# MrTornado24/IDE-3D

Hardware: AMD Instinct MI355X
Metric: 512x512 RGB+seg frames/s @96 depth samples (whole job) (higher is better)
Workload: dtype f32 (3x3 convs + MLPs: fp32 operands as 3 bf16 pieces, 6 products, f32 accumulate); 1 GPU; BASELINE config 2: random-init ide3d-ffhq-64-512, G.mapping + G.synthesis (64 render -> 512, 96 samples, RGB + 19-class seg) + uint8 frames, batch 4 seeds per GPU; global_batch=4, parallelism=dp1, conv_arithmetic=bf16x6, conv_arithmetic_is_library_default=True

## Files before the change

### ide-3d_amd/csrc/camera.hip

```cpp
#include "common.h"

namespace ide3d {

#pragma clang fp contract(off)

struct V3 { float x, y, z; };
__device__ __forceinline__ V3 normalized(V3 v) {
    const float n = sqrtf(v.x * v.x + v.y * v.y + v.z * v.z);
    return V3{v.x / n, v.y / n, v.z / n};
}
__device__ __forceinline__ V3 cross(V3 a, V3 b) { return V3{a.y * b.z - a.z * b.y, a.z * b.x - a.x * b.z, a.x * b.y - a.y * b.x}; }

__global__ void __launch_bounds__(64)
sphere_points_kernel(const float* __restrict__ theta, const float* __restrict__ pitch, int n, float r, int pitch_is_v,
                     float* __restrict__ pos, float* __restrict__ phi_out) {
    const int i = blockIdx.x * 64 + threadIdx.x;
    if (i >= n) return;
    const float kPi = 3.14159265358979323846f;
    float p = fminf(fmaxf(pitch[i], 1e-5f), (float)(3.14159265358979323846 - 1e-5));
    if (pitch[i] != pitch[i]) p = pitch[i];
    if (pitch_is_v) p = acosf(1.f - 2.f * (p * (1.f / kPi)));
    const float t = theta[i], sp = r * sinf(p);
    pos[3 * i + 0] = sp * cosf(t);
    pos[3 * i + 2] = sp * sinf(t);
    pos[3 * i + 1] = r * cosf(p);
    if (phi_out) phi_out[i] = p;
}

__global__ void __launch_bounds__(64)
cam2world_kernel(const float* __restrict__ forward, const float* __restrict__ origin, const float* __restrict__ lookat, int lookat_stride,
                 int n, float* __restrict__ out) {
    const int i = blockIdx.x * 64 + threadIdx.x;
    if (i >= n) return;
    const V3 o{origin[3 * i], origin[3 * i + 1], origin[3 * i + 2]};
    V3 f;
    if (lookat) {
        const float* l = lookat + (int64_t)i * lookat_stride;
        f = normalized(V3{l[0] - o.x, l[1] - o.y, l[2] - o.z});
    } else {
        f = V3{forward[3 * i], forward[3 * i + 1], forward[3 * i + 2]};
    }
    f = normalized(f);
    const V3 left = normalized(cross(V3{0.f, 1.f, 0.f}, f));
    const V3 up = normalized(cross(f, left));
    float* m = out + (int64_t)i * 16;
    m[0] = -left.x; m[1] = up.x; m[2]  = -f.x; m[3]  = o.x;
    m[4] = -left.y; m[5] = up.y; m[6]  = -f.y; m[7]  = o.y;
    m[8] = -left.z; m[9] = up.z; m[10] = -f.z; m[11] = o.z;
    m[12] = 0.f;    m[13] = 0.f; m[14] = 0.f;  m[15] = 1.f;
}

}

extern "C" int ide3d_sphere_points(const float* theta, const float* pitch, int32_t n, float r, int32_t pitch_is_v,
                                   float* pos, float* phi_out, void* stream) {
    using namespace ide3d;
    IDE3D_CHECK_ARG(theta && pitch && pos, "sphere_points: null pointer");
    IDE3D_CHECK_ARG(n > 0, "sphere_points: bad shape");
    hipLaunchKernelGGL(sphere_points_kernel, dim3(cdiv(n, 64)), dim3(64), 0, (hipStream_t)stream, theta, pitch, n, r, pitch_is_v, pos, phi_out);
    IDE3D_CHECK_LAUNCH("sphere_points");
    return IDE3D_OK;
}

extern "C" int ide3d_cam2world(const float* forward, const float* origin, const float* lookat, int32_t lookat_stride, int32_t n,
                               float* out, void* stream) {
    using namespace ide3d;
    IDE3D_CHECK_ARG(origin && out && (forward || lookat), "cam2world: null pointer");
    IDE3D_CHECK_ARG(n > 0 && (lookat_stride == 0 || lookat_stride == 3), "cam2world: bad shape");
    hipLaunchKernelGGL(cam2world_kernel, dim3(cdiv(n, 64)), dim3(64), 0, (hipStream_t)stream, forward, origin, lookat, lookat_stride, n, out);
    IDE3D_CHECK_LAUNCH("cam2world");
    return IDE3D_OK;
}
```

### ide-3d_amd/csrc/common.h

```cpp
#pragma once

#include <hip/hip_runtime.h>
#include <hip/hip_fp16.h>
#include <hip/hip_bf16.h>
#include <stdint.h>
#include <stdarg.h>
#include <stdio.h>

#include "../../include/ide3d_hip.h"

namespace ide3d {

constexpr int kWave = 64;
constexpr int kNumCU = 256;
constexpr int kNumXCD = 8;


void set_error(const char* fmt, ...);

const char* modconv_build_flags();
const char* triplane_tile_build_flags();
const char* raymarch_build_flags();

void note_exclusive_violation(const char* kernel, int blocks_per_cu);
// ... 10 lines not shown
}
#define IDE3D_EXCL_LAUNCH(KERNEL, GRID, THREADS, DYN_LDS, ST, ...) \
    do { if (ide3d::exclusive_on_this_device(KERNEL, (THREADS), (DYN_LDS), #KERNEL)) hipLaunchKernelGGL(KERNEL, GRID, dim3(THREADS), DYN_LDS, ST, __VA_ARGS__); } while (0)
#define IDE3D_STR_(x) #x
#define IDE3D_STR(x) IDE3D_STR_(x)

#define IDE3D_CHECK_ARG(cond, ...)                                   \
    do { if (!(cond)) { ide3d::set_error(__VA_ARGS__); return IDE3D_EINVAL; } } while (0)

#define IDE3D_CHECK_LAUNCH(what)                                     \
    do { hipError_t e_ = hipGetLastError();                          \
         if (e_ != hipSuccess) { ide3d::set_error("%s: %s", what, hipGetErrorString(e_)); \
                                 return IDE3D_ELAUNCH; }                \
         if (ide3d::take_refused()) return IDE3D_ELAUNCH; } while (0)


template <class T> struct Elem;
template <> struct Elem<float> {
    using math_t = float;
    static __device__ __forceinline__ float  ld(const float* p) { return *p; }
    static __device__ __forceinline__ void   st(float* p, float v) { *p = v; }
};
template <> struct Elem<double> {
    using math_t = double;
    static __device__ __forceinline__ double ld(const double* p) { return *p; }
    static __device__ __forceinline__ void   st(double* p, double v) { *p = v; }
};
template <> struct Elem<__half> {
    using math_t = float;
    static __device__ __forceinline__ float  ld(const __half* p) { return __half2float(*p); }
    static __device__ __forceinline__ void   st(__half* p, float v) { *p = __float2half(v); }
};
template <> struct Elem<__hip_bfloat16> {
    using math_t = float;
    static __device__ __forceinline__ float  ld(const __hip_bfloat16* p) { return __bfloat162float(*p); }
    static __device__ __forceinline__ void   st(__hip_bfloat16* p, float v) { *p = __float2bfloat16(v); }
};


__device__ __forceinline__ int lane_id() { return threadIdx.x & (kWave - 1); }

__host__ __device__ __forceinline__ int floordiv(int a, int b) {
    int q = a / b;
    return (a % b != 0 && ((a < 0) != (b < 0))) ? q - 1 : q;
}

__device__ __forceinline__ void amax_raise(float* amax, int n, float v) {
    unsigned* const slot = reinterpret_cast<unsigned*>(amax) + (size_t)n * IDE3D_AMAX_FLOATS + (blockIdx.x % IDE3D_AMAX_SLOTS) * IDE3D_AMAX_STRIDE;
    __hip_atomic_fetch_max(slot, __float_as_uint(v), __ATOMIC_RELAXED, __HIP_MEMORY_SCOPE_AGENT);
}
__device__ __forceinline__ void amax_raise_block(float* amax, int n, float v, float* scratch) {
#pragma unroll
    for (int off = 32; off > 0; off >>= 1) v = fmaxf(v, __shfl_xor(v, off));
    __syncthreads();
    if ((threadIdx.x & 63) == 0) scratch[threadIdx.x >> 6] = v;
    __syncthreads();
    if (threadIdx.x == 0) {
        float m = scratch[0];
        for (int i = 1; i < (int)(blockDim.x >> 6); ++i) m = fmaxf(m, scratch[i]);
        if (m > 0.f) amax_raise(amax, n, m);
    }
}
__device__ __forceinline__ void amax_lds_flush(unsigned* s_am, int n, float v) { if (v > 0.f) atomicMax(&s_am[n & 63], __float_as_uint(v)); }
__device__ __forceinline__ void amax_lds_commit(float* amax, const unsigned* s_am, int p_n) {
    __syncthreads();
    if ((int)threadIdx.x < p_n && threadIdx.x < 64 && s_am[threadIdx.x] != 0u) amax_raise(amax, (int)threadIdx.x, __uint_as_float(s_am[threadIdx.x]));
}

__host__ __device__ __forceinline__ int64_t cdiv64(int64_t a, int64_t b) { return (a + b - 1) / b; }
__host__ __device__ __forceinline__ int     cdiv(int a, int b) { return (a + b - 1) / b; }

__device__ __forceinline__ bool pool_gt(float v, float m) { return v > m || v != v; }

inline bool ptr_aligned(const void* p, uintptr_t bytes) { return (reinterpret_cast<uintptr_t>(p) & (bytes - 1)) == 0; }

inline int stream_grid(int64_t work_items, int per_block) {
    int64_t g = cdiv64(work_items, per_block);
    const int64_t cap = (int64_t)kNumCU * 8;
    if (g > cap) g = cap;
    if (g < 1) g = 1;
    return (int)g;
}

__device__ __forceinline__ int xcd_remap(int bid, int nblocks) {
    const int xcd = bid % kNumXCD;
    const int idx = bid / kNumXCD;
    const int q = nblocks / kNumXCD, r = nblocks % kNumXCD;
    const int base = (xcd < r) ? xcd * (q + 1) : r * (q + 1) + (xcd - r) * q;
    return base + idx;
}

}
```

### ide-3d_amd/csrc/core.hip

```cpp
#include "common.h"
#include <string.h>
#include <stdio.h>
#include <map>
#include <mutex>
#include <tuple>

namespace ide3d {

static thread_local char g_err[512] = "";

void set_error(const char* fmt, ...) {
    va_list ap;
    va_start(ap, fmt);
    vsnprintf(g_err, sizeof(g_err), fmt, ap);
    va_end(ap);
}

static int g_excl_violations = 0;
static char g_excl_text[384] = "";
void note_exclusive_violation(const char* kernel, int blocks_per_cu) {
    ++g_excl_violations;
    snprintf(g_excl_text, sizeof(g_excl_text), "%d workgroups of %.200s fit one CU of this device: exclusive residency (DESIGN.md 4.2) does not hold", blocks_per_cu, kernel);
    fprintf(stderr, "[libide3d_hip] %s; the launch is refused (select IDE3D_CONV_ARITH=fp32)\n", g_excl_text);
}
int exclusive_violations() { return g_excl_violations; }
static thread_local bool g_refused = false;
void refuse_launch(const char* kernel) {
    g_refused = true;
    set_error("%.200s: more than one workgroup fits a CU of this device, exclusive residency (DESIGN.md 4.2) does not hold; launch refused "
              "(IDE3D_CONV_ARITH=fp32 selects the arithmetic that needs none)", kernel);
}
bool take_refused() { const bool r = g_refused; g_refused = false; return r; }

bool exclusive_checked(const void* kernel, int threads, size_t dyn_lds, const char* name) {
    static std::mutex mu;
    static std::map<std::tuple<const void*, int, int, size_t>, int> table;
    int dev = 0;
    if (hipGetDevice(&dev) != hipSuccess) return true;
    int occ;
    {
        std::lock_guard<std::mutex> lock(mu);
        const auto key = std::make_tuple(kernel, dev, threads, dyn_lds);
        auto it = table.find(key);
        if (it == table.end()) {
            int n = 0;
            occ = (hipOccupancyMaxActiveBlocksPerMultiprocessor(&n, kernel, threads, dyn_lds) == hipSuccess && n > 0) ? n : -1;
            table.emplace(key, occ);
            if (occ > 1) note_exclusive_violation(name, occ);
        } else occ = it->second;
    }
    if (occ > 1) refuse_launch(name);
    return occ <= 1;
}

}

extern "C" int ide3d_exclusive_violations(void) { return ide3d::g_excl_violations; }
extern "C" const char* ide3d_exclusive_violation_text(void) { return ide3d::g_excl_text; }
extern "C" const char* ide3d_last_error(void) { return ide3d::g_err; }
extern "C" int ide3d_abi_version(void) { return 8; }
extern "C" const char* ide3d_build_arch(void) { return "gfx950"; }
extern "C" const char* ide3d_build_flags(void) {
    static char buf[512] = "";
    static bool done = false;
    if (!done) {
        snprintf(buf, sizeof(buf), "%s%s%s", ide3d::modconv_build_flags(), ide3d::triplane_tile_build_flags(), ide3d::raymarch_build_flags());
        const size_t n = strlen(buf);
        if (n && buf[n - 1] == ' ') buf[n - 1] = 0;
        done = true;
    }
    return buf;
}
```

### ide-3d_amd/csrc/modconv.hip

```cpp
#include "common.h"
#include "knobs.h"
#include <stdlib.h>
#include <string.h>
#include <type_traits>

namespace ide3d {

typedef float f32x16 __attribute__((ext_vector_type(16)));

#ifdef IDE3D_MC_TRACE
__device__ unsigned long long g_mc_dbg[256];
#define IDE3D_MC_TS(k) { const unsigned long long now_ = __builtin_readcyclecounter(); mc_acc[k] += now_ - mc_last; mc_last = now_; }
#else
#define IDE3D_MC_TS(k)
#endif

enum { MODE_CONV3 = 0, MODE_CONV1 = 1, MODE_TCONV3 = 2, MODE_TCONV3A = 3, MODE_CONV3S2 = 4 };

template <int MODE> struct ModeCfg;
template <> struct ModeCfg<MODE_CONV3>  { static constexpr int KC = 4, WTAPS = 9, MAXT = 9; };
template <> struct ModeCfg<MODE_CONV1>  { static constexpr int KC = 16, WTAPS = 1, MAXT = 1; };
template <> struct ModeCfg<MODE_CONV3S2> { static constexpr int KC = 4, WTAPS = 9, MAXT = 9; };
template <> struct ModeCfg<MODE_TCONV3> { static constexpr int KC = 4, WTAPS = 9, MAXT = 4; };
template <> struct ModeCfg<MODE_TCONV3A> { static constexpr int KC = 4, WTAPS = 9, MAXT = 9; };
// ... 495 lines not shown
    for (int q = 0; q < PARTS; ++q) {
        const unsigned pk = pk_bf16(a, b);
        out[q] = pk;
        if (q + 1 < PARTS) { a -= __uint_as_float(pk << 16); b -= __uint_as_float(pk & 0xffff0000u); }
    }
    }
}
template <int F16>
__device__ __forceinline__ f32x16 sp_mfma(const u32x4& a, const u32x4& b, const f32x16& c) {
    if constexpr (F16) return __builtin_amdgcn_mfma_f32_32x32x16_f16(__builtin_bit_cast(f16x8, a), __builtin_bit_cast(f16x8, b), c, 0, 0, 0);
    else return __builtin_amdgcn_mfma_f32_32x32x16_bf16(__builtin_bit_cast(bf16x8, a), __builtin_bit_cast(bf16x8, b), c, 0, 0, 0);
}
__device__ __forceinline__ void f16_scale(float bound, float& scale, float& unscale) {
    scale = 1.f; unscale = 1.f;
    if (bound > 0.f && bound < __builtin_inff()) {
        int e;
        frexpf(bound, &e);
        e = min(max(15 - e, -126), 126);
        scale = ldexpf(1.f, e); unscale = ldexpf(1.f, -e);
    }
}

__global__ void __launch_bounds__(256)
modconv_row_scale_kernel(const float* __restrict__ w, int cout, int rowlen, int rows_padded, float* __restrict__ scale, float* __restrict__ unscale) {
    const int row = blockIdx.x * 4 + (threadIdx.x >> 6), lane = threadIdx.x & 63;
    if (row >= rows_padded) return;
    float m = 0.f;
    if (row < cout) for (int i = lane; i < rowlen; i += 64) m = fmaxf(m, fabsf(w[(int64_t)row * rowlen + i]));
#pragma unroll
    for (int off = 32; off > 0; off >>= 1) m = fmaxf(m, __shfl_xor(m, off));
    if (lane == 0) { float sc, us; f16_scale(m, sc, us); scale[row] = sc; unscale[row] = us; }
}

template <int PARTS, int F16 = 0>
__global__ void __launch_bounds__(256)
modconv_pack_split_kernel(const float* __restrict__ w, int cout, int cin, int bm, int mblocks, int cchunks, u32x4* __restrict__ out,
                          const float* __restrict__ row_scale = nullptr) {
    const int64_t total = (int64_t)mblocks * cchunks * 9 * 2 * bm;
    const int64_t stride = (int64_t)gridDim.x * blockDim.x;
    for (int64_t i = (int64_t)blockIdx.x * blockDim.x + threadIdx.x; i < total; i += stride) {
        int64_t r = i;
        const int co_l = (int)(r % bm); r /= bm;
        const int kg = (int)(r % 2); r /= 2;
        const int tap = (int)(r % 9); r /= 9;
        const int cc = (int)(r % cchunks); r /= cchunks;
        const int mb = (int)r;
        const int co = mb * bm + co_l;
        const float rs = F16 ? row_scale[co] : 1.f;
        unsigned pk[4][PARTS];
#pragma unroll
        for (int e = 0; e < 4; ++e) {
            const int ci = cc * 16 + kg * 8 + e * 2;
            const float a = (co < cout && ci < cin) ? w[((int64_t)co * cin + ci) * 9 + tap] * rs : 0.f;
            const float b = (co < cout && ci + 1 < cin) ? w[((int64_t)co * cin + ci + 1) * 9 + tap] * rs : 0.f;
            split_pair<PARTS, F16>(a, b, pk[e]);
        }
        const int64_t base = (((int64_t)(mb * cchunks + cc) * 9 + tap) * PARTS * 2 + kg) * bm + co_l;
#pragma unroll
        for (int q = 0; q < PARTS; ++q) {
            const u32x4 v = {pk[0][q], pk[1][q], pk[2][q], pk[3][q]};
            out[base + (int64_t)q * 2 * bm] = v;
        }
    }
}

template <int OFF_BYTES>
__device__ __forceinline__ u32x4 lds_read128_async(unsigned addr) {
    u32x4 v;
    asm volatile("ds_read_b128 %0, %1 offset:%2" : "=v"(v) : "v"(addr), "n"(OFF_BYTES));
    return v;
}
template <int PENDING>
__device__ __forceinline__ void lds_wait128(u32x4& first) { asm volatile("s_waitcnt lgkmcnt(%1)" : "+v"(first) : "n"(PENDING)); }
__device__ __forceinline__ void lds_pin128(u32x4& v) { asm volatile("" : "+v"(v)); }

struct HeadEpi {
    const u32x4* w;
    const float* bias;
    float* y;
    int rows;
    float clamp;
    int store_x;
    int bias_first;
};
template <int PH, int PW, int NWV, int MTW, int NTW, int BM, int MT, int PARTS, int SCRATCH>
__device__ __forceinline__ void split_heads_finish(const ide3d_modconv_params& p, const HeadEpi& he, f32x16 (&acc)[1][MTW][NTW], float* smem,
                                                   int n0, int y0, int x0, int wm, int wn, int lp) {
    constexpr int NT = 64 * NWV, BN = PH * PW, TP = BN + 4, ROWS = MT * 32, CCH = BM / 16, A_UNITS = PARTS * 2 * ROWS;
    static_assert(BM * TP + 2 * BM + ROWS <= SCRATCH, "activation tile + coefficients must fit the loop's LDS");
    const int tid = threadIdx.x, lane = tid & 63, half = lane >> 5, l32 = lane & 31;
    const int wid = __builtin_amdgcn_readfirstlane(tid >> 6);
    const int hw = p.h * p.w_;
    float* const s_t = smem;
    float* const s_dm = smem + BM * TP;
    float* const s_bi = s_dm + BM;
    float* const s_hb = s_bi + BM;
    for (int e = tid; e < BM; e += NT) {
        s_dm[e] = (p.dcoefs && e < p.cout) ? p.dcoefs[(int64_t)n0 * p.cout + e] : 1.f;
        s_bi[e] = (p.bias && e < p.cout) ? p.bias[e] : 0.f;
    }
    for (int e = tid; e < ROWS; e += NT) s_hb[e] = (he.bias && e < he.rows) ? he.bias[e] : 0.f;
    __syncthreads();
    const float e_alpha = (p.act == 3) ? p.alpha : 1.f, e_gain = p.gain;
    const float e_clamp = (p.clamp >= 0.f) ? p.clamp : __builtin_inff();
    const float e_nstr = p.noise ? p.noise_strength : 0.f;
    auto finish = [&](float v, float d, float nz, float bb) {
        v *= d; v += nz; v += bb;
        v = (v > 0.f) ? v : v * e_alpha;
        v *= e_gain;
        return fminf(fmaxf(v, -e_clamp), e_clamp);
    };
#pragma unroll
    for (int j = 0; j < NTW; ++j) {
        const int pix = (wn * NTW + j) * 32 + lp;
        const int gy = y0 + pix / PW, gx = x0 + pix % PW;
        const float nz = (e_nstr != 0.f) ? p.noise[gy * p.w_ + gx] * e_nstr : 0.f;
#pragma unroll
        for (int i = 0; i < MTW; ++i)
#pragma unroll
            for (int r = 0; r < 16; ++r) {
                const int rl = (wm * MTW + i) * 32 + (r & 3) + 8 * (r >> 2) + 4 * half;
                s_t[rl * TP + pix] = finish(acc[0][i][j][r], s_dm[rl], nz, s_bi[rl]);
            }
    }
    __syncthreads();
    typedef float f32x4a __attribute__((ext_vector_type(4)));
    typedef float f32x4u __attribute__((ext_vector_type(4), aligned(4)));
    if (he.store_x) {
        float* const yimg = p.y + (int64_t)n0 * p.cout * hw;
#pragma unroll 4
        for (int e = tid; e < BM * BN / 4; e += NT) {
            const int rl = e / (BN / 4), pix = (e % (BN / 4)) * 4;
            const int gy = y0 + pix / PW, gx = x0 + pix % PW;
            *reinterpret_cast<f32x4u*>(yimg + (int64_t)rl * hw + gy * p.w_ + gx) = *reinterpret_cast<const f32x4a*>(s_t + rl * TP + pix);
        }
    }
    constexpr int NPT = BN / 32;
    constexpr int RG = (MT % 2 == 0 && NPT / NWV < 2) ? 2 : 1, MTH = MT / RG, PG = NWV / RG, NTH = NPT / PG;
    static_assert(MTH * RG == MT && NTH * PG == NPT && NTH >= 1, "head work must split evenly over the waves");
    const int rg = wid / PG, pg = wid % PG;
    const u32x4* __restrict__ wsrc = he.w + (int64_t)n0 * CCH * A_UNITS + half * ROWS + rg * MTH * 32 + l32;
    f32x16 hacc[MTH][NTH];
#pragma unroll
    for (int m = 0; m < MTH; ++m)
#pragma unroll
        for (int g = 0; g < 4; ++g) {
            const f32x4a b4 = *reinterpret_cast<const f32x4a*>(s_hb + (rg * MTH + m) * 32 + 8 * g + 4 * half);
#pragma unroll
            for (int t = 0; t < NTH; ++t)
#pragma unroll
                for (int k = 0; k < 4; ++k) hacc[m][t][4 * g + k] = he.bias_first ? b4[k] : 0.f;
        }
    u32x4 af[2][MTH][PARTS];
    auto fetch_a = [&](int c, int buf) {
#pragma unroll
        for (int m = 0; m < MTH; ++m)
#pragma unroll
            for (int q = 0; q < PARTS; ++q) af[buf][m][q] = wsrc[(int64_t)c * A_UNITS + q * 2 * ROWS + m * 32];
    };
    fetch_a(0, 0);
#pragma unroll
    for (int c = 0; c < CCH; ++c) {
        const int ab = c & 1;
        if (c + 1 < CCH) fetch_a(c + 1, ab ^ 1);
#pragma unroll
        for (int t = 0; t < NTH; ++t) {
// ... 661 lines not shown
                for (int j = 0; j < STRIP_CO; ++j) acc[j] = fmaf(va, w1[j], acc[j]);
            } else {
                const float vb = ok_b ? xb[k] * scv[k] : 0.f;
                const float4 a0 = wv[0], a1 = wv[1], c0v = wv[4], c1v = wv[5];
                const float w0[STRIP_CO] = {a0.x, a0.y, a0.z, a0.w, a1.x, a1.y, a1.z, a1.w};
                const float w2[STRIP_CO] = {c0v.x, c0v.y, c0v.z, c0v.w, c1v.x, c1v.y, c1v.z, c1v.w};
#pragma unroll
                for (int j = 0; j < STRIP_CO; ++j) { acc[j] = fmaf(va, w0[j], acc[j]); acc[j] = fmaf(vb, w2[j], acc[j]); }
            }
        }
    }
#pragma unroll
    for (int j = 0; j < STRIP_CO; ++j) s_red[q][j][lane] = acc[j];
    __syncthreads();
    float am = 0.f;
    {
        static_assert(STRIP_CO <= STRIP_WAVES, "wave q < STRIP_CO finishes output channel co0 + q");
        float v = 0.f;
        const int qc = min(q, STRIP_CO - 1);
#pragma unroll
        for (int k = 0; k < STRIP_WAVES; ++k) v += s_red[k][qc][lane];
        const int co = co0 + q;
        if (live && q < STRIP_CO && co < p.cout) {
            v *= p.dcoefs ? p.dcoefs[(int64_t)n * p.cout + co] : 1.f;
            const int oy = is_row ? oh - 1 : t, ox = is_row ? t : ow - 1;
            p.y[((int64_t)n * p.cout + co) * ((int64_t)oh * pitch) + (int64_t)oy * pitch + ox] = v;
            amax_acc(am, v);
        }
    }
    if (p.y_amax) amax_raise_block(p.y_amax, n, am, s_am);
}

struct BlockId { int mb, tile, grp, split; };
__device__ __forceinline__ BlockId decode_block(const ConvGeom& g) {
    int bid = xcd_remap(blockIdx.x, gridDim.x);
    BlockId b;
    b.mb = bid % g.mblocks; bid /= g.mblocks;
    b.tile = bid % g.tile_base[4]; bid /= g.tile_base[4];
    b.grp = bid % g.img_groups; bid /= g.img_groups;
    b.split = bid;
    return b;
}

template <int MODE, int BIG, int TI, int PH, int PW>
__global__ void __launch_bounds__(256, (McCfg<MODE, BIG, TI, PH, PW>::NCLS * McCfg<MODE, BIG, TI, PH, PW>::MTW * McCfg<MODE, BIG, TI, PH, PW>::NTW > 8) ? 1
                                       : (TI * PH * PW <= 128 && MODE != MODE_CONV3S2) ? 3 : 2)
modconv_kernel(ide3d_modconv_params p, const float* __restrict__ wp, float* __restrict__ partial, ConvGeom g) {
    using K = McCfg<MODE, BIG, TI, PH, PW>;
    __shared__ __attribute__((aligned(16))) float s_w[2 * K::LDS_W];
    __shared__ __attribute__((aligned(16))) float s_x[2 * K::LDS_X];
    const BlockId b = decode_block(g);
    int cls = 0;
    if (MODE == MODE_TCONV3) { cls = (b.tile >= g.tile_base[1]) + (b.tile >= g.tile_base[2]) + (b.tile >= g.tile_base[3]); }
    modconv_tile<MODE, BIG, TI, PH, PW>(p, wp, partial, g, s_w, s_x, b.mb, b.tile - g.tile_base[cls], b.grp, b.split, cls, g.tiles_x[cls]);
}


#ifdef IDE3D_SP_SHARED_SIMD
constexpr bool kSpExclusive = false;
#else
constexpr bool kSpExclusive = true;
#endif
template <int MODE, int BIG, int PH, int PARTS, int WBUF, int NWV>
constexpr int sp_waves_per_simd() {
    using K = SpCfg<MODE, BIG, PH, PARTS, WBUF, NWV>;
    return (NWV == 8) ? 2 : (!kSpExclusive && K::LDS_BYTES <= 80 * 1024 && (WBUF == 1 || K::NCLS * K::MTW * K::NTW <= 8)) ? 2 : 1;
}
template <int MODE, int BIG, int PH, int PARTS, int WBUF = 2, int NWV = 4, int F16 = 0>
__global__ void __launch_bounds__(64 * NWV, (sp_waves_per_simd<MODE, BIG, PH, PARTS, WBUF, NWV>()))
modconv_split_kernel(ide3d_modconv_params p, const u32x4* __restrict__ wp, float* __restrict__ partial, ConvGeom g, const float* __restrict__ row_unscale) {
    using K = SpCfg<MODE, BIG, PH, PARTS, WBUF, NWV>;
    if constexpr (kSpExclusive) { if constexpr (NWV == 8) asm volatile("" ::: "v255"); else asm volatile("" ::: "v255", "a255"); }
    __shared__ __attribute__((aligned(16))) unsigned char sp_smem[K::LDS_BYTES];
    const BlockId b = decode_block(g);
    modconv_split_tile<MODE, BIG, PH, PARTS, WBUF, NWV, F16>(p, wp, partial, g, sp_smem, b.mb, b.tile, b.grp, b.split, g.tiles_x[0], row_unscale);
}

template <int BIG, int PH, int HEAD_MT>
__global__ void __launch_bounds__(512, 2)
modconv_split_heads_kernel(ide3d_modconv_params p, const u32x4* __restrict__ wp, ConvGeom g, HeadEpi he) {
    using K = SpCfg<MODE_CONV3, BIG, PH, 3, 2, 8>;
    if constexpr (kSpExclusive) asm volatile("" ::: "v255");
    __shared__ __attribute__((aligned(16))) unsigned char sp_smem[K::LDS_BYTES];
    const BlockId b = decode_block(g);
    modconv_split_tile<MODE_CONV3, BIG, PH, 3, 2, 8, 0, 1, -1, HEAD_MT>(p, wp, nullptr, g, sp_smem, b.mb, b.tile, b.grp, b.split, g.tiles_x[0], nullptr, nullptr, &he);
}

template <int BIG, int PH, int PARTS, int F16 = 0>
__global__ void __launch_bounds__(512, 2)
modconv_split_pair_kernel(ide3d_modconv_params p, const u32x4* __restrict__ wp, float* __restrict__ partial, ConvGeom g, const float* __restrict__ row_unscale) {
    using K = SpCfg<MODE_TCONV3A, BIG, PH, PARTS, 2, 8, 1>;
    if constexpr (kSpExclusive) asm volatile("" ::: "v255");
    __shared__ __attribute__((aligned(16))) unsigned char sp_smem[K::LDS_BYTES];
    const int half_grid = (int)(gridDim.x >> 1);
    const int par = __builtin_amdgcn_readfirstlane((int)blockIdx.x >= half_grid ? 1 : 0);
    int bid = xcd_remap((int)blockIdx.x - par * half_grid, half_grid);
    BlockId b;
    b.mb = bid % g.mblocks; bid /= g.mblocks;
    b.tile = bid % g.tile_base[4]; bid /= g.tile_base[4];
    b.grp = bid % g.img_groups; bid /= g.img_groups;
    b.split = bid;
    if (par == 0) modconv_split_tile<MODE_TCONV3A, BIG, PH, PARTS, 2, 8, F16, 1, 0>(p, wp, partial, g, sp_smem, b.mb, b.tile, b.grp, b.split, g.tiles_x[0], row_unscale);
    else          modconv_split_tile<MODE_TCONV3A, BIG, PH, PARTS, 2, 8, F16, 1, 1>(p, wp, partial, g, sp_smem, b.mb, b.tile, b.grp, b.split, g.tiles_x[0], row_unscale);
}

template <int MODE, int BIG, int PH, int PARTS, int WBUF, int F16>
__global__ void __launch_bounds__(512, 2)
modconv_split_teams_kernel(ide3d_modconv_params p, const u32x4* __restrict__ wp, float* __restrict__ partial, ConvGeom g, const float* __restrict__ row_unscale) {
    using K = SpCfg<MODE, BIG, PH, PARTS, WBUF, 4>;
    static_assert(2 * K::LDS_BYTES <= 160 * 1024, "both teams' LDS must fit");
    asm volatile("" ::: "v255");
    __shared__ __attribute__((aligned(16))) unsigned char sp_smem[2 * K::LDS_BYTES];
    const int team = (int)(threadIdx.x >> 8);
    int bid = xcd_remap(blockIdx.x, gridDim.x);
    const int mpairs = g.mblocks >> 1;
    BlockId b;
    b.mb = 2 * (bid % mpairs) + team; bid /= mpairs;
    b.tile = bid % g.tile_base[4]; bid /= g.tile_base[4];
    b.grp = bid % g.img_groups; bid /= g.img_groups;
    b.split = bid;
    modconv_split_tile<MODE, BIG, PH, PARTS, WBUF, 4, F16, 2>(p, wp, partial, g, sp_smem + team * K::LDS_BYTES, b.mb, b.tile, b.grp, b.split, g.tiles_x[0], row_unscale,
                                                              reinterpret_cast<float*>(sp_smem));
}

__global__ void __launch_bounds__(256)
modconv_epilogue_kernel(ide3d_modconv_params p, const float* __restrict__ partial, int split_k, int oh, int ow) {
    const int64_t per = (int64_t)p.n * p.cout * oh * ow;
    const int64_t stride = (int64_t)gridDim.x * blockDim.x;
    int am_n = -1; float am = 0.f;
    __shared__ unsigned s_am[64];
    const bool am_lds = p.y_amax && p.n <= 64;
    if (p.y_amax) { if (threadIdx.x < 64) s_am[threadIdx.x] = 0u; __syncthreads(); }
    const int hw = oh * ow;
    if (p.y_pitch <= 0 && (hw & 3) == 0) {
        typedef float f32x4v __attribute__((ext_vector_type(4)));
        const int64_t per4 = per >> 2;
        for (int64_t q = (int64_t)blockIdx.x * blockDim.x + threadIdx.x; q < per4; q += stride) {
            const int64_t i = q << 2;
            f32x4v v = {0.f, 0.f, 0.f, 0.f};
            int s = 0;
            for (; s + 4 <= split_k; s += 4) {
                f32x4v t[4];
#pragma unroll
                for (int k = 0; k < 4; ++k) t[k] = *reinterpret_cast<const f32x4v*>(partial + (int64_t)(s + k) * per + i);
#pragma unroll
                for (int k = 0; k < 4; ++k) v += t[k];
            }
            for (; s < split_k; ++s) v += *reinterpret_cast<const f32x4v*>(partial + (int64_t)s * per + i);
            const int pix = (int)(i % hw);
            const int co = (int)((i / hw) % p.cout);
            const int n = (int)(i / ((int64_t)hw * p.cout));
            const float d = p.dcoefs ? p.dcoefs[(int64_t)n * p.cout + co] : 1.f, bb = p.bias ? p.bias[co] : 0.f;
#pragma unroll
            for (int e = 0; e < 4; ++e) {
                float x = v[e];
                if (p.dcoefs) x *= d;
                if (p.noise) x += p.noise[pix + e] * p.noise_strength;
                if (p.bias) x += bb;
                if (p.act == 3) x = (x > 0.f) ? x : x * p.alpha;
                x *= p.gain;
                if (p.clamp >= 0.f) x = fminf(fmaxf(x, -p.clamp), p.clamp);
                v[e] = x;
            }
            *reinterpret_cast<f32x4v*>(p.y + i) = v;
            if (p.y_amax) {
                if (n != am_n) { if (am_n >= 0) { if (am_lds) amax_lds_flush(s_am, am_n, am); else amax_commit(p.y_amax, am_n, am, false); } am_n = n; am = 0.f; }
                amax_acc(am, v[0]); amax_acc(am, v[1]); amax_acc(am, v[2]); amax_acc(am, v[3]);
// ... 363 lines not shown
    IDE3D_CHECK_ARG(p.y_pitch == 0 || (p.mode == 2 && p.y_pitch >= 2 * p.w_ + 1), "modconv2d: y_pitch is the row pitch of a transposed convolution's output (>= 2 w + 1), or 0");
    hipStream_t st_head = (hipStream_t)stream;
    {
        const int64_t hw = (int64_t)p.h * p.w_;
        if (head_small_applies(p)) {
            if (hw <= 64) hipLaunchKernelGGL((head_small_kernel<64, 32>), dim3(cdiv(p.cout, HS_RB), 1, p.n), dim3(HS_THREADS), 0, st_head, p, (int)hw);
            else          hipLaunchKernelGGL((head_small_kernel<256, 8>), dim3(cdiv(p.cout, HS_RB), cdiv((int)hw, 256), p.n), dim3(HS_THREADS), 0, st_head, p, (int)hw);
            IDE3D_CHECK_LAUNCH("modconv2d (small-map heads)");
            return IDE3D_OK;
        }
    }
    if (head_split_applies(p, resolve_arith(p.arith))) {
        const int parts = resolve_arith(p.arith) == 3 ? 2 : 3, mt = p.cout <= 32 ? 1 : 6, cchunks = cdiv(p.cin, 16);
        IDE3D_CHECK_ARG(p.workspace_bytes >= head_packed_units(p.n, cchunks, parts, mt) * 16, "modconv2d: workspace too small for the packed head weights");
        u32x4* wu = reinterpret_cast<u32x4*>(p.workspace);
        const int64_t items = (int64_t)p.n * cchunks * 2 * mt * 32;
        const int tiles = cdiv(p.h * p.w_, 32 * head_waves(mt));
        const int hw_h = p.h * p.w_, wgs_img = kNumCU / p.n, tiles32 = hw_h / 32;
        const bool resident = head_resident_applies(p);
#define IDE3D_HEAD_RES(P, M, C) IDE3D_EXCL_LAUNCH((head_resident_kernel<P, M, C>), dim3(p.n * wgs_img), 512, 0, st_head, p, wu, wgs_img, tiles32)
#define IDE3D_HEAD(P, M) do { \
            hipLaunchKernelGGL(head_pack_split_kernel<P>, dim3(stream_grid(items, 256)), dim3(256), 0, st_head, p.w, p.w_batch_stride, p.n, p.cout, p.cin, M * 32, cchunks, wu); \
            if (resident) { if (M == 6) IDE3D_HEAD_RES(P, 6, 8); else if (cchunks == 4) IDE3D_HEAD_RES(P, 1, 4); else IDE3D_HEAD_RES(P, 1, 8); } \
            else IDE3D_EXCL_LAUNCH((head_split_kernel<P, M>), dim3(p.n * tiles), 64 * head_waves(M), 0, st_head, p, wu, cchunks, tiles); } while (0)
        if (parts == 2) { if (mt == 1) IDE3D_HEAD(2, 1); else IDE3D_HEAD(2, 6); }
        else            { if (mt == 1) IDE3D_HEAD(3, 1); else IDE3D_HEAD(3, 6); }
#undef IDE3D_HEAD
#undef IDE3D_HEAD_RES
        IDE3D_CHECK_LAUNCH("modconv2d (split-bf16 heads)");
        return IDE3D_OK;
    }
    int arith_eff = resolve_arith(p.arith);
    if (arith_eff == 16 && !p.x_amax) arith_eff = 6;
    ConvPlan pl; plan_conv(p, pl, arith_eff);
    IDE3D_CHECK_ARG(p.workspace_bytes >= (pl.packed_floats + pl.aux_floats + pl.partial_floats) * (int64_t)sizeof(float),
                    "modconv2d: workspace too small (need %lld bytes)", (long long)((pl.packed_floats + pl.aux_floats + pl.partial_floats) * sizeof(float)));
    hipStream_t st = (hipStream_t)stream;
    float* wp = p.workspace;
    float* partial = p.workspace + pl.packed_floats + pl.aux_floats;
    if (pl.parts) {
        if (!p.weights_packed) pack_split_weights(p, pl, wp, st);
#define IDE3D_SP_DISPATCH(M) \
        do { if (pl.big == 1) { if (pl.f16) launch_split<M, 1, 2, 1>(p, pl, wp, partial, st); else if (pl.parts == 2) launch_split<M, 1, 2>(p, pl, wp, partial, st); else launch_split<M, 1, 3>(p, pl, wp, partial, st); } \
             else             { if (pl.f16) launch_split<M, 2, 2, 1>(p, pl, wp, partial, st); else if (pl.parts == 2) launch_split<M, 2, 2>(p, pl, wp, partial, st); else launch_split<M, 2, 3>(p, pl, wp, partial, st); } } while (0)
        if (pl.mode == MODE_CONV3) IDE3D_SP_DISPATCH(MODE_CONV3); else IDE3D_SP_DISPATCH(MODE_TCONV3A);
#undef IDE3D_SP_DISPATCH
    } else {
    if (!p.weights_packed) {
        hipLaunchKernelGGL(modconv_pack_kernel, dim3(stream_grid(pl.packed_floats, 256)), dim3(256), 0, st,
                           p.w, p.w_batch_stride, p.w_batch_stride ? p.n : 1, p.cout, p.cin, pl.taps, pl.bm, pl.kc, pl.mblocks, pl.cchunks, wp);
    }
#define IDE3D_MC_DISPATCH(M) \
    do { if (pl.big == 1) launch_tiles<M, 1>(p, pl, wp, partial, st); else if (pl.big == 2) launch_tiles<M, 2>(p, pl, wp, partial, st); \
         else launch_tiles<M, 0>(p, pl, wp, partial, st); } while (0)
    if (pl.mode == MODE_CONV3)       IDE3D_MC_DISPATCH(MODE_CONV3);
    else if (pl.mode == MODE_CONV1)  IDE3D_MC_DISPATCH(MODE_CONV1);
    else if (pl.mode == MODE_CONV3S2) IDE3D_MC_DISPATCH(MODE_CONV3S2);
    else if (pl.mode == MODE_TCONV3A) IDE3D_MC_DISPATCH(MODE_TCONV3A);
    else                             IDE3D_MC_DISPATCH(MODE_TCONV3);
#undef IDE3D_MC_DISPATCH
    }
    if (pl.g.split_k > 1) {
        const int64_t per = (int64_t)p.n * p.cout * pl.oh * pl.ow;
        hipLaunchKernelGGL(modconv_epilogue_kernel, dim3(stream_grid((p.y_pitch <= 0 && ((pl.oh * pl.ow) & 3) == 0) ? per / 4 : per, 256)), dim3(256), 0, st, p, partial, pl.g.split_k, pl.oh, pl.ow);
    }
    if (pl.mode == MODE_TCONV3A && !p.weights_packed) {
        hipLaunchKernelGGL(tconv_strip_pack_kernel, dim3(stream_grid(pl.strip_floats, 256)), dim3(256), 0, st, p.w, p.cout, p.cin, cdiv(p.cout, STRIP_CO) * STRIP_CO,
                           wp + pl.packed_floats + pl.strip_off);
    }
    if (pl.strip) {
        const int cout_pad = cdiv(p.cout, STRIP_CO) * STRIP_CO;
        float* const wstrip = wp + pl.packed_floats + pl.strip_off;
        const int nb_re = cdiv(p.w_ + 1, 64), nb_ro = cdiv(p.w_, 64), nb_ce = cdiv(p.h, 64), nb_co = cdiv(p.h, 64);
        float* const xs = wstrip + pl.strip_floats;
        hipLaunchKernelGGL(tconv_strip_gather_kernel, dim3(stream_grid((int64_t)p.n * p.cin * (p.h + p.w_), 256)), dim3(256), 0, st, p.x, p.n * p.cin, p.h, p.w_, xs);
        hipLaunchKernelGGL(tconv_strip_kernel, dim3(nb_re + nb_ro + nb_ce + nb_co, cout_pad / STRIP_CO, p.n), dim3(64 * STRIP_WAVES), 0, st, p, wstrip, xs, cout_pad,
                           pl.oh, pl.ow, (int64_t)(p.y_pitch > 0 ? p.y_pitch : pl.ow), nb_re, nb_ro, nb_ce);
    }
    IDE3D_CHECK_LAUNCH("modconv2d");
    return IDE3D_OK;
}

extern "C" int ide3d_modconv2d_heads(const ide3d_modconv_params* pp, const ide3d_modconv_head_epilogue* hp, void* stream) {
    using namespace ide3d;
    IDE3D_CHECK_ARG(pp != nullptr && hp != nullptr, "modconv2d_heads: null params");
    const ide3d_modconv_params& p = *pp;
    const ide3d_modconv_head_epilogue& h = *hp;
    IDE3D_CHECK_ARG(p.x && p.w && p.workspace && (p.y || h.no_activation_output) && h.w && h.y && h.workspace, "modconv2d_heads: null tensor / workspace pointer");
    int rc = check_modconv(p);
    if (rc) return rc;
    IDE3D_CHECK_ARG(p.act == 1 || p.act == 3, "modconv2d_heads: act must be linear (1) or lrelu (3)");
    IDE3D_CHECK_ARG(h.rows > 0, "modconv2d_heads: bad head rows");
    auto no_kernel = [](const char* why) { set_error("modconv2d_heads: %s", why); return IDE3D_ENOKERNEL; };
    if (knob_live("IDE3D_MODCONV_NO_HEAD_FUSION")) return no_kernel("IDE3D_MODCONV_NO_HEAD_FUSION is set");
    if (p.k != 3 || p.mode != 0 || p.w_batch_stride != 0 || p.y_amax || p.y_pitch != 0) return no_kernel("not a shared-weight 3x3 layer without side outputs");
    int arith = resolve_arith(p.arith);
    if (arith == 16 && !p.x_amax) arith = 6;
    if (arith != 6) return no_kernel("the fused form exists for bf16x6 only");
    ConvPlan pl; plan_conv(p, pl, arith);
    if (pl.parts != 3 || pl.f16 || pl.mode != MODE_CONV3 || pl.pair || pl.g.split_k != 1 || pl.g.mblocks != 1 || pl.bm != p.cout || kTiles[pl.tile].images != 1)
        return no_kernel("the layer's plan does not hold all channels of a tile in one workgroup");
    const bool tile16 = pl.big == 1 && p.cout == 128 && pl.tile == T16x16 && sp_form(pl).waves == 8;
    const bool tile32 = pl.big == 2 && p.cout == 64 && pl.tile == T32x16;
    const int ph = tile32 ? 32 : 16;
    if (!(tile16 || tile32) || p.h % ph != 0 || p.w_ % 16 != 0) return no_kernel("no fused instance for this tile");
    ide3d_modconv_params q{};
    q.x = p.y; q.w = h.w; q.bias = h.bias; q.y = h.y;
    q.n = p.n; q.cin = p.cout; q.cout = h.rows; q.h = p.h; q.w_ = p.w_; q.k = 1; q.mode = 0;
    q.act = 1; q.alpha = 0.f; q.gain = 1.f; q.clamp = h.clamp; q.w_batch_stride = (int64_t)h.rows * p.cout; q.arith = p.arith;
    const int mt = h.rows <= 32 ? 1 : 6, hcc = p.cout / 16;
    if (head_small_applies(q) || !head_split_applies(q, resolve_arith(q.arith)) || resolve_arith(q.arith) == 3 || (mt == 6 && !tile16))
        return no_kernel("the heads do not take the split-bf16 path");
    IDE3D_CHECK_ARG(p.workspace_bytes >= (pl.packed_floats + pl.aux_floats) * (int64_t)sizeof(float), "modconv2d_heads: workspace too small");
    IDE3D_CHECK_ARG(h.workspace_bytes >= head_packed_units(p.n, hcc, 3, mt) * 16, "modconv2d_heads: head workspace too small");
    hipStream_t st = (hipStream_t)stream;
    if (!p.weights_packed) pack_split_weights(p, pl, p.workspace, st);
    u32x4* const hw_packed = reinterpret_cast<u32x4*>(h.workspace);
    const int64_t items = (int64_t)p.n * hcc * 2 * mt * 32;
    hipLaunchKernelGGL(head_pack_split_kernel<3>, dim3(stream_grid(items, 256)), dim3(256), 0, st, h.w, q.w_batch_stride, p.n, h.rows, p.cout, mt * 32, hcc, hw_packed);
    HeadEpi e;
    e.w = hw_packed; e.bias = h.bias; e.y = h.y; e.rows = h.rows; e.clamp = h.clamp; e.store_x = !h.no_activation_output;
    e.bias_first = head_resident_applies(q) ? 1 : 0;
    const ConvGeom& g = pl.g;
    const unsigned nblocks = (unsigned)((int64_t)g.mblocks * g.tile_base[4] * g.img_groups * g.split_k);
    const u32x4* wu = reinterpret_cast<const u32x4*>(p.workspace);
    if (tile32) IDE3D_EXCL_LAUNCH((modconv_split_heads_kernel<2, 32, 1>), dim3(nblocks), 512, 0, st, p, wu, g, e);
    else if (mt == 1) IDE3D_EXCL_LAUNCH((modconv_split_heads_kernel<1, 16, 1>), dim3(nblocks), 512, 0, st, p, wu, g, e);
    else IDE3D_EXCL_LAUNCH((modconv_split_heads_kernel<1, 16, 6>), dim3(nblocks), 512, 0, st, p, wu, g, e);
    IDE3D_CHECK_LAUNCH("modconv2d_heads");
    return IDE3D_OK;
}

extern "C" int ide3d_modconv_plan(const ide3d_modconv_params* pp, ide3d_modconv_plan_info* out) {
    using namespace ide3d;
    IDE3D_CHECK_ARG(pp != nullptr && out != nullptr, "modconv_plan: null argument");
    const ide3d_modconv_params p = flatten_pointwise(*pp);
    int rc = check_modconv(p);
    if (rc) return rc;
    *out = ide3d_modconv_plan_info{};
    const int arith = resolve_arith(p.arith);
    if (head_small_applies(p)) {
        const int hw = p.h * p.w_;
        out->kind = IDE3D_PLAN_HEAD_SMALL; out->tile_h = 1; out->tile_w = hw <= 64 ? 64 : 256; out->rows = HS_RB; out->waves = HS_THREADS / 64; out->split_k = 1;
        out->workgroups = (int64_t)cdiv(p.cout, HS_RB) * (hw <= 64 ? 1 : cdiv(hw, 256)) * p.n;
        return IDE3D_OK;
    }
    if (head_split_applies(p, arith)) {
        const int mt = p.cout <= 32 ? 1 : 6;
        out->rows = mt * 32; out->parts = arith == 3 ? 2 : 3; out->split_k = 1; out->tile_h = 1;
        if (head_resident_applies(p)) { out->kind = IDE3D_PLAN_HEAD_RESIDENT; out->tile_w = 32; out->waves = 8; out->workgroups = (int64_t)p.n * (kNumCU / p.n); }
        else { out->kind = IDE3D_PLAN_HEAD_SPLIT; out->waves = head_waves(mt); out->tile_w = 32 * out->waves; out->workgroups = (int64_t)p.n * cdiv(p.h * p.w_, out->tile_w); }
        return IDE3D_OK;
    }
    int arith_eff = arith;
    if (arith_eff == 16 && !p.x_amax) arith_eff = 6;
    ConvPlan pl; plan_conv(p, pl, arith_eff);
    const int64_t blocks = (int64_t)pl.g.mblocks * pl.g.tile_base[4] * pl.g.img_groups * pl.g.split_k * (pl.pair ? 2 : 1);
    out->tile_h = kTiles[pl.tile].rows; out->tile_w = kTiles[pl.tile].cols; out->images_per_tile = kTiles[pl.tile].images;
    out->rows = pl.bm; out->parts = pl.parts; out->f16 = pl.f16; out->split_k = pl.g.split_k; out->strip = pl.strip;
    out->transposed_all_class = (pl.mode == MODE_TCONV3A);
    if (pl.parts) {
        const SpForm f = sp_form(pl);
        out->kind = f.teams ? IDE3D_PLAN_SPLIT_TEAMS : IDE3D_PLAN_SPLIT; out->waves = f.teams ? 8 : f.waves; out->workgroups = f.teams ? blocks / 2 : blocks;
    } else {
        out->kind = IDE3D_PLAN_FP32; out->waves = 4; out->workgroups = blocks;
    }
    return IDE3D_OK;
}

extern "C" int ide3d_set_conv_arithmetic(int32_t arith) {
    IDE3D_CHECK_ARG(arith == 0 || arith == 1 || arith == 3 || arith == 6 || arith == 16,
                    "set_conv_arithmetic: 0 (environment default), 1 (fp32), 3 (bf16x3), 6 (bf16x6) or 16 (f16x3)");
    ide3d::g_conv_arith = arith;
    return IDE3D_OK;
}
extern "C" int32_t ide3d_get_conv_arithmetic(void) { return ide3d::conv_arith_default(); }

#ifdef IDE3D_MC_TRACE
extern "C" int ide3d_debug_mc(unsigned long long* host) {
    return (int)hipMemcpyFromSymbol(host, HIP_SYMBOL(ide3d::g_mc_dbg), sizeof(unsigned long long) * 256);
}
#endif

namespace ide3d {
const char* modconv_build_flags() {
    return ""
#ifdef IDE3D_SP_SHARED_SIMD
        "!IDE3D_SP_SHARED_SIMD "
#endif
#ifdef IDE3D_MC_TRACE
        "IDE3D_MC_TRACE "
#endif
        ;
}
}
```

### ide-3d_amd/csrc/resample.hip

```cpp
#include "common.h"

namespace ide3d {
namespace {

constexpr int SK_ROWS = 8, SK_COLS = 32, SK_CH = 32;
constexpr int SK_LR = SK_ROWS / 2 + 2, SK_LC = SK_COLS / 2 + 2;
constexpr int SK_TP = SK_CH + 1;

struct SkipArgs {
    const float* lo; const float* add; float* out;
    int64_t lo_s[4], add_s[4];
    int n, c, h, w;
    int tiles_x, tiles_y, cgroups;
};

__global__ void __launch_bounds__(256)
skip_upsample_add_cl_kernel(const SkipArgs p) {
    __shared__ float s_lo[SK_CH][SK_LR][SK_LC + 1];
    __shared__ float s_t[SK_ROWS * SK_COLS][SK_TP];
    const int tid = threadIdx.x;
    int b = xcd_remap(blockIdx.x, gridDim.x);
    const int cg = b % p.cgroups; b /= p.cgroups;
    const int tx = b % p.tiles_x; b /= p.tiles_x;
    const int ty = b % p.tiles_y; b /= p.tiles_y;
    const int n = b;
    const int c0 = cg * SK_CH, Y0 = ty * SK_ROWS, X0 = tx * SK_COLS;
    const int H = 2 * p.h, W = 2 * p.w;
    const int m0 = Y0 / 2 - 1, q0 = X0 / 2 - 1;
    constexpr int NLO = (SK_CH * SK_LR * SK_LC + 255) / 256;
    float lo_v[NLO];
#pragma unroll
    for (int i = 0; i < NLO; ++i) {
        const int e = tid + i * 256;
        const int c = e / (SK_LR * SK_LC), r = e % (SK_LR * SK_LC), ry = r / SK_LC, rx = r % SK_LC;
        const int yy = m0 + ry, xx = q0 + rx;
        const bool ok = e < SK_CH * SK_LR * SK_LC && c0 + c < p.c && yy >= 0 && yy < p.h && xx >= 0 && xx < p.w;
        const int64_t off = n * p.lo_s[0] + (int64_t)min(c0 + c, p.c - 1) * p.lo_s[1] + (int64_t)min(max(yy, 0), p.h - 1) * p.lo_s[2]
                          + (int64_t)min(max(xx, 0), p.w - 1) * p.lo_s[3];
        const float v = p.lo[off];
        lo_v[i] = ok ? v : 0.f;
    }
    const int row = tid >> 5, x = tid & 31;
    const int Y = Y0 + row, X = X0 + x;
    const bool ok = Y < H && X < W;
    float add_v[SK_CH];
    {
        const float* ap = p.add + n * p.add_s[0] + (int64_t)min(Y, H - 1) * p.add_s[2] + (int64_t)min(X, W - 1) * p.add_s[3];
#pragma unroll
        for (int c = 0; c < SK_CH; ++c) add_v[c] = ap[(int64_t)min(c0 + c, p.c - 1) * p.add_s[1]];
    }
#pragma unroll
    for (int i = 0; i < NLO; ++i) {
        const int e = tid + i * 256;
        if (e < SK_CH * SK_LR * SK_LC) {
            const int c = e / (SK_LR * SK_LC), r = e % (SK_LR * SK_LC);
            s_lo[c][r / SK_LC][r % SK_LC] = lo_v[i];
        }
    }
    __syncthreads();
    {
        const int ly = (Y >> 1) - m0 - 1 + (Y & 1), lx = (X >> 1) - q0 - 1 + (X & 1);
        const float wy0 = (Y & 1) ? 0.75f : 0.25f, wy1 = 1.0f - wy0;
        const float wx0 = (X & 1) ? 0.75f : 0.25f, wx1 = 1.0f - wx0;
#pragma unroll
        for (int c = 0; c < SK_CH; ++c) {
            const float a = s_lo[c][ly][lx], bq = s_lo[c][ly][lx + 1], cq = s_lo[c][ly + 1][lx], d = s_lo[c][ly + 1][lx + 1];
            float v = wy0 * (wx0 * a + wx1 * bq) + wy1 * (wx0 * cq + wx1 * d);
            if (ok && c0 + c < p.c) v += add_v[c];
            s_t[tid][c] = v;
        }
    }
    __syncthreads();
    {
        const int j = tid & 7;
#pragma unroll
        for (int k = 0; k < 8; ++k) {
            const int px = (tid >> 3) + 32 * k, row = px >> 5, x = px & 31;
            const int Y = Y0 + row, X = X0 + x;
            if (Y >= H || X >= W) continue;
            float* o = p.out + (((int64_t)n * H + Y) * W + X) * p.c + c0 + 4 * j;
            const float* t = &s_t[px][4 * j];
            if (c0 + 4 * j + 3 < p.c) {
                typedef float f32x4_t __attribute__((ext_vector_type(4)));
                const f32x4_t v = {t[0], t[1], t[2], t[3]};
                __builtin_nontemporal_store(v, reinterpret_cast<f32x4_t*>(o));
            } else {
                for (int e = 0; e < 4; ++e) if (c0 + 4 * j + e < p.c) o[e] = t[e];
            }
        }
    }
}

struct BilinArgs {
    const float* x; int n, c, h, w;
    float* dst[3]; int c_begin[3], c_count[3];
    int64_t bs[3];
};

__global__ void __launch_bounds__(256)
bilinear_up2_split_kernel(const BilinArgs p) {
    const int H = 2 * p.h, W = 2 * p.w, W4 = W / 4;
    const int ctot = p.c_count[0] + p.c_count[1] + p.c_count[2];
    const int64_t total = (int64_t)p.n * ctot * H * W4;
    const int64_t stride = (int64_t)gridDim.x * blockDim.x;
    for (int64_t i = (int64_t)blockIdx.x * blockDim.x + threadIdx.x; i < total; i += stride) {
        int64_t r = i;
        const int X = (int)(r % W4) * 4; r /= W4;
        const int Y = (int)(r % H); r /= H;
        int cc = (int)(r % ctot);
        const int n = (int)(r / ctot);
        int k = 0;
        if (cc >= p.c_count[0]) { cc -= p.c_count[0]; k = 1; if (cc >= p.c_count[1]) { cc -= p.c_count[1]; k = 2; } }
        const int ci = p.c_begin[k] + cc;
        const float sy = fmaxf(0.5f * ((float)Y + 0.5f) - 0.5f, 0.f);
        const int y0 = (int)sy, y1 = y0 + (y0 < p.h - 1);
        const float ly1 = sy - (float)y0, ly0 = 1.f - ly1;
        const float* r0 = p.x + ((int64_t)n * p.c + ci) * ((int64_t)p.h * p.w) + (int64_t)y0 * p.w;
        const float* r1 = r0 + (int64_t)(y1 - y0) * p.w;
        float o[4];
#pragma unroll
        for (int e = 0; e < 4; ++e) {
            const float sx = fmaxf(0.5f * ((float)(X + e) + 0.5f) - 0.5f, 0.f);
            const int x0 = (int)sx, x1 = x0 + (x0 < p.w - 1);
            const float lx1 = sx - (float)x0, lx0 = 1.f - lx1;
            o[e] = ly0 * (lx0 * r0[x0] + lx1 * r0[x1]) + ly1 * (lx0 * r1[x0] + lx1 * r1[x1]);
        }
        *reinterpret_cast<float4*>(p.dst[k] + (int64_t)n * p.bs[k] + ((int64_t)cc * H + Y) * W + X) = make_float4(o[0], o[1], o[2], o[3]);
    }
}

}
}

extern "C" int ide3d_skip_upsample_add_cl(const float* lo, const int64_t lo_stride[4], const float* add, const int64_t add_stride[4],
                                          int32_t n, int32_t c, int32_t h, int32_t w, float* out, void* stream) {
    using namespace ide3d;
    IDE3D_CHECK_ARG(lo && add && out && lo_stride && add_stride, "skip_upsample_add_cl: null pointer");
    IDE3D_CHECK_ARG(n > 0 && c > 0 && h > 0 && w > 0, "skip_upsample_add_cl: bad shape");
    IDE3D_CHECK_ARG(c % 4 == 0 && (reinterpret_cast<uintptr_t>(out) & 15) == 0, "skip_upsample_add_cl: channels must be a multiple of 4 and out 16-byte aligned");
    SkipArgs a;
    a.lo = lo; a.add = add; a.out = out;
    for (int i = 0; i < 4; ++i) { a.lo_s[i] = lo_stride[i]; a.add_s[i] = add_stride[i]; }
    a.n = n; a.c = c; a.h = h; a.w = w;
    a.tiles_x = cdiv(2 * w, SK_COLS); a.tiles_y = cdiv(2 * h, SK_ROWS); a.cgroups = cdiv(c, SK_CH);
    const int64_t blocks = (int64_t)n * a.tiles_x * a.tiles_y * a.cgroups;
    IDE3D_CHECK_ARG(blocks < 0x7fffffffLL, "skip_upsample_add_cl: too many tiles");
    hipLaunchKernelGGL(skip_upsample_add_cl_kernel, dim3((unsigned)blocks), dim3(256), 0, (hipStream_t)stream, a);
    IDE3D_CHECK_LAUNCH("skip_upsample_add_cl");
    return IDE3D_OK;
}

extern "C" int ide3d_bilinear_up2_split(const float* x, int32_t n, int32_t c, int32_t h, int32_t w,
                                        float* const dst[3], const int32_t c_begin[3], const int32_t c_count[3], const int64_t* dst_batch_floats, void* stream) {
    using namespace ide3d;
    IDE3D_CHECK_ARG(x && dst && c_begin && c_count, "bilinear_up2_split: null pointer");
    IDE3D_CHECK_ARG(n > 0 && c > 0 && h > 0 && w > 0, "bilinear_up2_split: bad shape");
    IDE3D_CHECK_ARG(w % 2 == 0, "bilinear_up2_split: input width must be even (16-byte output stores)");
    BilinArgs a;
    a.x = x; a.n = n; a.c = c; a.h = h; a.w = w;
    int64_t total = 0;
    for (int k = 0; k < 3; ++k) {
        a.dst[k] = dst[k]; a.c_begin[k] = c_begin[k]; a.c_count[k] = c_count[k];
        const int64_t dense = (int64_t)c_count[k] * 4 * h * w;
        a.bs[k] = (dst_batch_floats && dst_batch_floats[k]) ? dst_batch_floats[k] : dense;
        IDE3D_CHECK_ARG(a.bs[k] >= dense && a.bs[k] % 4 == 0, "bilinear_up2_split: batch stride of output %d is smaller than an image or not a multiple of 4 floats", k);
        IDE3D_CHECK_ARG(c_count[k] >= 0 && c_begin[k] >= 0 && c_begin[k] + c_count[k] <= c && (c_count[k] == 0 || dst[k]),
                        "bilinear_up2_split: channel range %d outside the input", k);
        IDE3D_CHECK_ARG(c_count[k] == 0 || (reinterpret_cast<uintptr_t>(dst[k]) & 15) == 0, "bilinear_up2_split: output %d is not 16-byte aligned", k);
        total += (int64_t)n * c_count[k] * 2 * h * (w / 2);
    }
    if (total == 0) return IDE3D_OK;
    hipLaunchKernelGGL(bilinear_up2_split_kernel, dim3(stream_grid(total, 256)), dim3(256), 0, (hipStream_t)stream, a);
    IDE3D_CHECK_LAUNCH("bilinear_up2_split");
    return IDE3D_OK;
}
```

### ide-3d_amd/torch_utils/hip_plugin.py

```python

import ctypes
import math
import os
import threading
import weakref

import torch

_LIB_ENV = 'IDE3D_HIP_LIB'
_ABI_VERSION = 8
AMAX_SLOTS, AMAX_STRIDE = 32, 64
AMAX_FLOATS = AMAX_SLOTS * AMAX_STRIDE

_DTYPE_CODE = {torch.float32: 0, torch.float16: 1, torch.bfloat16: 2, torch.float64: 3}

_lock = threading.Lock()
_lib = None

CALLS = {}


def lib_path():
    env = os.environ.get(_LIB_ENV)
    if env:
# ... 270 lines not shown
                    paths.add(line.split()[-1])
    except OSError:
        pass
    return paths


def load():
    global _lib
    if _lib is not None:
        return _lib
    with _lock:
        if _lib is not None:
            return _lib
        path = lib_path()
        if not os.path.isfile(path):
            raise RuntimeError(
                f'libide3d_hip.so not found at {path}. Build it with `python -c "import __graft_entry__ as g; g.build()"` '
                f'or `make -C ide-3d_amd/csrc`, or point ${_LIB_ENV} at it. There is no CPU/eager fallback for CUDA tensors.')
        torch.cuda.is_available()
        try:
            lib = ctypes.CDLL(path, mode=ctypes.RTLD_LOCAL)
        except OSError as e:
            raise RuntimeError(f'failed to load {path}: {e}') from e
        rts = _hip_runtimes_mapped()
        if len(rts) > 1:
            raise RuntimeError(f'two HIP runtimes mapped in one process ({sorted(rts)}); import torch before loading the plugin')
        vp, i32, i64, f32 = ctypes.c_void_p, ctypes.c_int32, ctypes.c_int64, ctypes.c_float
        lib.ide3d_last_error.restype = ctypes.c_char_p
        lib.ide3d_last_error.argtypes = []
        lib.ide3d_abi_version.restype = ctypes.c_int
        lib.ide3d_build_arch.restype = ctypes.c_char_p
        if lib.ide3d_abi_version() != _ABI_VERSION:
            raise RuntimeError(f'{path}: ABI version {lib.ide3d_abi_version()} != expected {_ABI_VERSION}; rebuild')
        lib.ide3d_build_flags.restype = ctypes.c_char_p
        lib.ide3d_build_flags.argtypes = []
        flags = lib.ide3d_build_flags().decode('ascii', 'replace').split()
        unsafe = [f for f in flags if f.startswith('!')]
        if unsafe and os.environ.get('IDE3D_ALLOW_EXPERIMENT_BUILD') != '1':
            raise RuntimeError(f'{path} was built with experiment knobs that change results or drop a safety property ({" ".join(unsafe)}); '
                               'rebuild without EXTRA=..., or set IDE3D_ALLOW_EXPERIMENT_BUILD=1 for timing experiments')
        protos = {
            'ide3d_bias_act': [vp, vp, vp, vp, vp, vp, ctypes.c_int, ctypes.c_int, ctypes.c_int, f32, f32, f32, i64, i64, i64, vp],
            'ide3d_upfirdn2d': [ctypes.POINTER(_UpfirdnParams), vp],
            'ide3d_upfirdn2d_ex': [ctypes.POINTER(_UpfirdnParams), ctypes.POINTER(_UpfirdnEpilogue), vp],
            'ide3d_upfirdn2d_plan': [ctypes.POINTER(_UpfirdnParams), ctypes.POINTER(_UpfirdnEpilogue), ctypes.POINTER(_UpfirdnPlanInfo)],
            'ide3d_filtered_lrelu': [ctypes.POINTER(_FlreluParams), vp],
            'ide3d_filtered_lrelu_act': [vp, vp, ctypes.c_int, i32, i32, i32, i32, ctypes.POINTER(i64 * 4),
                                         i32, i32, i32, i32, f32, f32, f32, ctypes.c_int, vp],
            'ide3d_triplane_sample': [vp, ctypes.POINTER(i64 * 4), i32, i32, i32, i32, vp, i64, vp, vp],
            'ide3d_triplane_sample_rays': [vp, ctypes.POINTER(i64 * 4), i32, i32, i32, i32, vp, i64, vp, i32, i32, i32, vp],
            'ide3d_triplane_taps': [i32, i32, vp, i64, vp, vp],
            'ide3d_triplane_tile_masks': [i32, i32, vp, i32, i32, i32, i32, vp, vp],
            'ide3d_triplane_sample_backward': [vp, vp, ctypes.POINTER(i64 * 4), i32, i32, i32, i32, vp, i64,
                                               vp, ctypes.POINTER(i64 * 4), vp, vp],
            'ide3d_composite': [vp, vp, vp, vp, i64, i32, i32, ctypes.c_int, ctypes.c_int, ctypes.c_int, f32,
                                ctypes.c_int, vp, vp, vp, vp],
            'ide3d_composite_plan': [vp, i64, i32, i32, ctypes.POINTER(_CompositePlanInfo)],
            'ide3d_sample_pdf': [vp, vp, vp, i64, i64, i32, i32, f32, vp, vp],
            'ide3d_render_rays': [ctypes.POINTER(_RenderParams), vp],
            'ide3d_render_ray_weights': [ctypes.POINTER(_RenderParams), vp, vp, vp, vp, vp],
            'ide3d_merge_depths': [vp, vp, i64, i32, i32, vp, vp, vp],
            'ide3d_render_rays_merged': [ctypes.POINTER(_RenderParams), vp, vp, vp, i32, vp],
            'ide3d_render_rays_backward': [ctypes.POINTER(_RenderParams), ctypes.POINTER(_RenderGrads), vp],
            'ide3d_render_param_grad_workspace_bytes': [ctypes.POINTER(_RenderParams)],
            'ide3d_render_rays_backward_params': [ctypes.POINTER(_RenderParams), ctypes.POINTER(_RenderGrads), ctypes.POINTER(_RenderParamGrads), vp],
            'ide3d_render_camera_grad_workspace_bytes': [ctypes.POINTER(_RenderParams)],
            'ide3d_render_rays_backward_camera': [ctypes.POINTER(_RenderParams), ctypes.POINTER(_RenderGrads), ctypes.POINTER(_RenderParamGrads),
                                                  ctypes.POINTER(_RenderCameraGrads), vp],
            'ide3d_render_merged_param_grad_workspace_bytes': [ctypes.POINTER(_RenderParams)],
            'ide3d_render_rays_merged_backward': [ctypes.POINTER(_RenderParams), vp, vp, vp, i32, ctypes.POINTER(_RenderGrads),
                                                  ctypes.POINTER(_RenderParamGrads), vp],
            'ide3d_sample_voxel': [ctypes.POINTER(_RenderParams), vp, i64, vp, vp, ctypes.c_int, vp],
            'ide3d_lattice_points': [ctypes.POINTER(_Lattice), i64, i64, vp, vp],
            'ide3d_density_lattice': [ctypes.POINTER(_RenderParams), ctypes.POINTER(_Lattice), i64, i64, vp, vp],
            'ide3d_mesh_workspace_bytes': [i32, i32, i32],
            'ide3d_mesh_count': [vp, i32, i32, i32, f32, vp, vp, i64, vp],
            'ide3d_mesh_emit': [vp, i32, i32, i32, f32, vp, ctypes.POINTER(_Lattice), i32, vp, i64, i64, i64, vp, vp, vp, vp],
            'ide3d_raster_workspace_bytes': [i32, i64, i32, i32],
            'ide3d_raster_project': [vp, i64, vp, i32, i32, i32, f32, f32, f32, f32, f32, f32, f32, vp, i64, vp],
            'ide3d_raster_depth': [vp, i64, i64, i32, i32, i32, i32, i32, vp, i64, vp],
            'ide3d_raster_shade': [vp, vp, i64, i32, i32, i32, vp, vp, vp, vp, i32, f32, f32, ctypes.POINTER(ctypes.c_float * 3), f32, vp, i64, vp, vp, vp, vp, vp],
            'ide3d_modconv2d': [ctypes.POINTER(_ModconvParams), vp],
            'ide3d_modconv2d_heads': [ctypes.POINTER(_ModconvParams), ctypes.POINTER(_ModconvHeadEpilogue), vp],
            'ide3d_modconv_plan': [ctypes.POINTER(_ModconvParams), ctypes.POINTER(_ModconvPlanInfo)],
            'ide3d_modconv_workspace_bytes': [i32, i32, i32, i32, i32, i32, i32, i32],
            'ide3d_act_bwd_workspace_bytes': [i32, i32, i32, i32],
            'ide3d_modconv_act_backward': [ctypes.POINTER(_ActBwdParams), vp],
            'ide3d_modconv_scale_dot': [vp, vp, vp, vp, vp, i32, i32, i32, i32, vp, i64, vp],
            'ide3d_head_wgrad_workspace_bytes': [i32, i32, i32, i32, i32],
            'ide3d_head_weight_grad': [vp, vp, vp, i32, i32, i32, i32, i32, vp, i64, vp],
            'ide3d_wgrad_workspace_bytes': [i32, i32, i32, i32, i32],
            'ide3d_modconv_weight_grad': [ctypes.POINTER(_WgradParams), vp],
            'ide3d_bias_noise_workspace_bytes': [i32, i32, i32, i32],
            'ide3d_bias_noise_grad': [vp, vp, vp, i32, i32, i32, i32, vp, i64, vp],
            'ide3d_noise_reg_workspace_bytes': [ctypes.POINTER(i32), i32],
            'ide3d_noise_reg_levels': [ctypes.POINTER(i32), i32],
            'ide3d_noise_reg': [vp, ctypes.POINTER(i32), i32, vp, i64, vp, vp, vp],
            'ide3d_noise_reg_backward': [vp, ctypes.POINTER(i32), i32, vp, i64, vp, vp, vp, vp],
            'ide3d_noise_normalize_workspace_bytes': [ctypes.POINTER(i32), i32],
            'ide3d_noise_normalize': [vp, ctypes.POINTER(i32), i32, vp, i64, vp],
            'ide3d_lpips_prep': [vp, vp, vp, vp, i32, i32, i32, i32, f32, f32, vp],
            'ide3d_lpips_prep_backward': [vp, vp, vp, i32, i32, i32, i32, f32, vp],
            'ide3d_maxpool2': [vp, vp, i64, i32, i32, vp],
            'ide3d_lpips_stage_backward': [vp, vp, vp, vp, i64, i32, i32, vp],
            'ide3d_lpips_head_workspace_bytes': [ctypes.POINTER(_LpipsTap), i32, i32],
            'ide3d_lpips_head': [ctypes.POINTER(_LpipsTap), i32, i32, vp, i64, vp, vp],
            'ide3d_lpips_head_backward': [ctypes.POINTER(_LpipsTap), i32, i32, vp, vp],
            'ide3d_unfold2d': [vp, vp, i32, i32, i32, i32, i32, i32, i32, vp],
            'ide3d_fold2d': [vp, vp, i32, i32, i32, i32, i32, i32, i32, vp],
            'ide3d_maxpool3s2p0': [vp, vp, vp, i64, i32, i32, vp],
            'ide3d_lpips_tap_backward': [vp, vp, vp, vp, vp, i64, i32, i32, i32, vp],
            'ide3d_feat_l1_workspace_bytes': [ctypes.POINTER(_FeatL1Tap), i32, i32],
            'ide3d_feat_l1': [ctypes.POINTER(_FeatL1Tap), i32, i32, vp, i64, vp, vp],
            'ide3d_feat_l1_tap_backward': [vp, vp, vp, vp, vp, f32, i64, i32, i32, i64, vp],
            'ide3d_maxpool2_relu_backward': [vp, vp, vp, i64, i32, i32, vp],
            'ide3d_resize_bilinear': [vp, vp, i64, i32, i32, i32, i32, vp],
            'ide3d_resize_bilinear_backward': [vp, vp, i64, i32, i32, i32, i32, vp],
            'ide3d_parse_ce_workspace_bytes': [i32, i32, i32, i32, i32, i32],
            'ide3d_parse_ce': [vp, vp, i32, i32, i32, i32, i32, i32, vp, vp, i64, vp, vp],
            'ide3d_parse_ce_backward': [vp, vp, vp, vp, vp, i32, i32, i32, i32, i32, i32, vp],
            'ide3d_maxpool3s2': [vp, vp, vp, i64, i32, i32, vp],
            'ide3d_maxpool3s2_backward': [vp, vp, vp, vp, i64, i32, i32, vp],
            'ide3d_parse_join': [ctypes.POINTER(_ParseJoinParams), vp],
            'ide3d_plane_sums': [vp, vp, vp, i64, i64, f32, vp],
            'ide3d_parse_stem_backward': [vp, vp, vp, i32, i32, i32, i32, vp],
            'ide3d_id_prep': [vp, vp, i32, i32, vp],
            'ide3d_id_prep_backward': [vp, vp, i32, i32, vp],
            'ide3d_prelu': [vp, vp, vp, i32, i32, i32, i32, vp],
            'ide3d_prelu_backward': [vp, i64, i64, i32, vp, vp, vp, i32, i32, i32, i32, vp],
            'ide3d_se_gate': [vp, vp, vp, vp, i32, i32, i32, vp],
            'ide3d_se_gate_backward': [vp, vp, vp, vp, vp, vp, i32, i32, i32, vp],
            'ide3d_linear_workspace_bytes': [i32, i32, i32],
            'ide3d_linear_backward_input_workspace_bytes': [i32, i32, i32],
            'ide3d_linear': [vp, vp, vp, vp, i32, i32, i32, vp, i64, vp],
            'ide3d_linear_backward_input': [vp, vp, vp, i32, i32, i32, vp, i64, vp],
            'ide3d_linear_weight_grad': [vp, vp, vp, i32, i32, i32, vp],
            'ide3d_residual_join': [vp, vp, vp, i64, f32, vp],
            'ide3d_id_head': [vp, vp, vp, vp, vp, i32, i32, vp],
            'ide3d_id_head_backward': [vp, vp, vp, vp, vp, i32, i32, vp],
            'ide3d_set_conv_arithmetic': [i32],
            'ide3d_get_conv_arithmetic': [],
            'ide3d_frame_u8': [vp, vp, vp, i32, i32, i32, i32, vp, vp],
            'ide3d_sphere_points': [vp, vp, i32, ctypes.c_float, i32, vp, vp, vp],
            'ide3d_cam2world': [vp, vp, vp, i32, i32, vp, vp],
            'ide3d_style_demod': [vp, i64, vp, vp, vp, i32, i32, i32, i32, f32, f32, vp, vp, vp],
            'ide3d_fold_heads': [vp, i64, i32, i32, i32, f32, vp, vp, vp, i32, f32, vp, vp, vp, i32, f32, vp, vp],
            'ide3d_style_demod_batch': [ctypes.POINTER(_StyleJob), i32, i32, i32, vp],
            'ide3d_fold_heads_batch': [ctypes.POINTER(_FoldJob), i32, i32, i32, vp],
            'ide3d_mapping': [ctypes.POINTER(_MappingParams), vp],
            'ide3d_mapping_workspace_bytes': [],
            'ide3d_mapping_supported': [],
            'ide3d_skip_upsample_add_cl': [vp, ctypes.POINTER(i64 * 4), vp, ctypes.POINTER(i64 * 4), i32, i32, i32, i32, vp, vp],
            'ide3d_bilinear_up2_split': [vp, i32, i32, i32, i32, ctypes.POINTER(vp * 3), ctypes.POINTER(i32 * 3), ctypes.POINTER(i32 * 3), ctypes.POINTER(ctypes.c_int64 * 3), vp],
            'ide3d_lowres_layers_supported': [i32, i32, i32, ctypes.POINTER(i32), i32, i32],
            'ide3d_lowres_workspace_bytes': [ctypes.POINTER(_LowresParams)],
            'ide3d_lowres_group': [ctypes.POINTER(_LowresParams), vp],
        }
        for name, argtypes in protos.items():
            fn = getattr(lib, name)
            fn.restype = ctypes.c_int64 if name.endswith('_bytes') else ctypes.c_int
            fn.argtypes = argtypes
        _lib = lib
        return _lib


EXPORTED_SYMBOLS = (
    'ide3d_last_error', 'ide3d_abi_version', 'ide3d_build_arch', 'ide3d_build_flags', 'ide3d_exclusive_violations', 'ide3d_exclusive_violation_text', 'ide3d_bias_act', 'ide3d_upfirdn2d', 'ide3d_upfirdn2d_ex', 'ide3d_upfirdn2d_plan',
    'ide3d_filtered_lrelu', 'ide3d_filtered_lrelu_act', 'ide3d_triplane_sample', 'ide3d_triplane_sample_rays', 'ide3d_triplane_taps', 'ide3d_triplane_tile_masks',
    'ide3d_triplane_sample_backward', 'ide3d_composite', 'ide3d_composite_plan', 'ide3d_sample_pdf', 'ide3d_render_rays', 'ide3d_render_rays_backward', 'ide3d_sample_voxel',
    'ide3d_lattice_points', 'ide3d_density_lattice',
    'ide3d_modconv2d', 'ide3d_modconv2d_heads', 'ide3d_modconv_workspace_bytes', 'ide3d_modconv_plan', 'ide3d_set_conv_arithmetic', 'ide3d_get_conv_arithmetic', 'ide3d_frame_u8', 'ide3d_sphere_points', 'ide3d_cam2world', 'ide3d_style_demod', 'ide3d_fold_heads',
    'ide3d_style_demod_batch', 'ide3d_fold_heads_batch',
    'ide3d_skip_upsample_add_cl', 'ide3d_bilinear_up2_split', 'ide3d_mapping', 'ide3d_mapping_workspace_bytes', 'ide3d_mapping_supported',
    'ide3d_lowres_layers_supported', 'ide3d_lowres_phase_r_plan', 'ide3d_lowres_workspace_bytes', 'ide3d_lowres_group',
    'ide3d_act_bwd_workspace_bytes', 'ide3d_modconv_act_backward', 'ide3d_modconv_scale_dot', 'ide3d_head_wgrad_workspace_bytes',
    'ide3d_head_weight_grad', 'ide3d_wgrad_workspace_bytes', 'ide3d_modconv_weight_grad', 'ide3d_bias_noise_workspace_bytes',
    'ide3d_bias_noise_grad', 'ide3d_render_param_grad_workspace_bytes', 'ide3d_render_rays_backward_params',
    'ide3d_noise_reg_workspace_bytes', 'ide3d_noise_reg_levels', 'ide3d_noise_reg', 'ide3d_noise_reg_backward',
    'ide3d_noise_normalize_workspace_bytes', 'ide3d_noise_normalize',
    'ide3d_render_camera_grad_workspace_bytes', 'ide3d_render_rays_backward_camera',
    'ide3d_lpips_prep', 'ide3d_lpips_prep_backward', 'ide3d_maxpool2', 'ide3d_lpips_stage_backward', 'ide3d_lpips_head_workspace_bytes',
    'ide3d_lpips_head', 'ide3d_lpips_head_backward',
    'ide3d_unfold2d', 'ide3d_fold2d', 'ide3d_maxpool3s2p0', 'ide3d_lpips_tap_backward',
    'ide3d_feat_l1_workspace_bytes', 'ide3d_feat_l1', 'ide3d_feat_l1_tap_backward', 'ide3d_maxpool2_relu_backward',
    'ide3d_resize_bilinear', 'ide3d_resize_bilinear_backward', 'ide3d_parse_ce_workspace_bytes', 'ide3d_parse_ce', 'ide3d_parse_ce_backward',
    'ide3d_maxpool3s2', 'ide3d_maxpool3s2_backward', 'ide3d_parse_join', 'ide3d_plane_sums', 'ide3d_parse_stem_backward',
    'ide3d_id_prep', 'ide3d_id_prep_backward', 'ide3d_prelu', 'ide3d_prelu_backward', 'ide3d_se_gate', 'ide3d_se_gate_backward',
    'ide3d_linear_workspace_bytes', 'ide3d_linear_backward_input_workspace_bytes', 'ide3d_linear', 'ide3d_linear_backward_input',
    'ide3d_linear_weight_grad', 'ide3d_residual_join', 'ide3d_id_head', 'ide3d_id_head_backward',
    'ide3d_mesh_workspace_bytes', 'ide3d_mesh_count', 'ide3d_mesh_emit',
    'ide3d_render_ray_weights', 'ide3d_merge_depths', 'ide3d_render_rays_merged',
    'ide3d_render_merged_param_grad_workspace_bytes', 'ide3d_render_rays_merged_backward',
    'ide3d_raster_workspace_bytes', 'ide3d_raster_project', 'ide3d_raster_depth', 'ide3d_raster_shade',
)


def exclusive_violations():
    lib = load()
    lib.ide3d_exclusive_violations.restype = ctypes.c_int
    lib.ide3d_exclusive_violation_text.restype = ctypes.c_char_p
    return int(lib.ide3d_exclusive_violations()), lib.ide3d_exclusive_violation_text().decode('utf-8', 'replace')


def _check(rc, what):
    if rc == 0:
        CALLS[what] = CALLS.get(what, 0) + 1
    if rc != 0:
        msg = load().ide3d_last_error().decode('utf-8', 'replace')
        raise RuntimeError(f'{what} failed (code {rc}): {msg}')


_raw_stream = getattr(torch._C, '_cuda_getCurrentRawStream', None)


def _stream_handle(device):
    if _raw_stream is not None:
        return _raw_stream(device.index if device.index is not None else torch.cuda.current_device())
    return torch.cuda.current_stream(device).cuda_stream


def _stream(t):
    return ctypes.c_void_p(_stream_handle(t.device))


_private_streams = {}


def _hip_runtime():
    paths = _hip_runtimes_mapped()
    if len(paths) != 1:
        raise RuntimeError(f'expected exactly one HIP runtime mapped in this process, found {sorted(paths)}')
    rt = ctypes.CDLL(next(iter(paths)))
    rt.hipStreamCreateWithFlags.argtypes = [ctypes.POINTER(ctypes.c_void_p), ctypes.c_uint]
    rt.hipStreamCreateWithFlags.restype = ctypes.c_int
    return rt


def private_stream(device, purpose):
    device = torch.device(device)
    idx = device.index if device.index is not None else torch.cuda.current_device()
    key = (idx, purpose)
    st = _private_streams.get(key)
    if st is None:
        with _lock:
            st = _private_streams.get(key)
            if st is None:
                torch.cuda.init()
                h = ctypes.c_void_p()
                with torch.cuda.device(idx):
                    rc = _hip_runtime().hipStreamCreateWithFlags(ctypes.byref(h), 1)
                if rc != 0 or not h.value:
                    raise RuntimeError(f'hipStreamCreateWithFlags failed ({rc})')
                st = _private_streams[key] = torch.cuda.ExternalStream(h.value, device=torch.device('cuda', idx))
    return st


capture_lock = threading.RLock()


class _NoGuard:
    def __enter__(self):
        return self

    def __exit__(self, *exc):
        return False


_NO_GUARD = _NoGuard()


def _dev_guard(device):
    if device is None:
        return _NO_GUARD
    idx = device.index if isinstance(device, torch.device) else device
    if idx is None or idx == torch.cuda.current_device():
        return _NO_GUARD
# ... 679 lines not shown
        sig = torch.empty([p.n * int(count)], dtype=torch.float32, device=tex_planes.device)
        if count:
            with _dev_guard(tex_planes.device):
                rc = load().ide3d_density_lattice(ctypes.byref(p), ctypes.byref(lat), int(first), int(count), _ptr(sig), _stream(tex_planes))
            if rc == -2:
                return None
            _check(rc, 'density_lattice')
        return sig


class ModconvPlugin:
    _ws = _Workspaces(limit=1024)
    _heads_declined = set()

    @staticmethod
    def _workspace(lib, x, w, n, cin, cout, h, wd, k, mode, per_image, arith):
        key = (0 if per_image else w.data_ptr(), tuple(w.shape), n, h, wd, mode, x.device.index, _ws_domain(x.device), arith)
        def alloc():
            nbytes = lib.ide3d_modconv_workspace_bytes(n, cin, cout, h, wd, k, mode, int(per_image))
            _require(nbytes >= 0, 'modconv2d: unsupported configuration')
            return torch.empty([max(nbytes // 4, 1)], dtype=torch.float32, device=x.device)
        return ModconvPlugin._ws.entry(key, alloc)

    @staticmethod
    def _params(lib, x, w, y, styles, dcoefs, noise, noise_strength, bias, act, alpha, gain, clamp, mode, arith, x_amax, y_amax):
        n, cin, h, wd = x.shape
        per_image = (w.ndim == 5)
        cout, _, k, _ = w.shape[-4:]
        ent = ModconvPlugin._workspace(lib, x, w, n, cin, cout, h, wd, k, mode, per_image, arith)
        p = _ModconvParams()
        p.x, p.w, p.y = x.data_ptr(), w.data_ptr(), (y.data_ptr() if y is not None else None)
        keep = []
        for name, t in (('styles', styles), ('dcoefs', dcoefs), ('noise', noise), ('bias', bias)):
            if t is not None:
                t = t.contiguous(); keep.append(t)
                _require(t.is_cuda and t.dtype == torch.float32, f'modconv2d: {name} must be float32 on GPU')
                _require(t.device == x.device, f'modconv2d: {name} must reside on the same device as x')
                setattr(p, name, t.data_ptr())
        p.n, p.cin, p.cout, p.h, p.w_, p.k = n, cin, cout, h, wd, k
        p.noise_strength = float(noise_strength)
        p.act, p.alpha, p.gain, p.clamp = int(act), float(alpha), float(gain), float(clamp)
        p.mode = mode
        p.weights_packed = int((not per_image) and ModconvPlugin._ws.packed(ent, (w,))[0])
        p.w_batch_stride = (cout * cin * k * k) if per_image else 0
        p.arith = arith
        for name, t in (('x_amax', x_amax), ('y_amax', y_amax)):
            if t is not None:
                _require(t.is_cuda and t.device == x.device and t.dtype == torch.float32 and tuple(t.shape) == (n, AMAX_FLOATS) and t.is_contiguous(),
                         f'modconv2d: {name} must be a contiguous float32 [n, AMAX_FLOATS] tensor on the device of x')
                setattr(p, name, t.data_ptr())
        p.workspace, p.workspace_bytes = ent[0].data_ptr(), ent[0].numel() * 4
        return p, ent, keep

    @staticmethod
    def modconv2d(x, w, styles, dcoefs, noise, noise_strength, bias, act, alpha, gain, clamp, mode=0, arith=0, x_amax=None, y_amax=None, pad_rows=False):
        for t in (x, w):
            _require(t.is_cuda and t.dtype == torch.float32 and t.is_contiguous(), 'modconv2d: contiguous float32 CUDA tensors required')
        _require(w.device == x.device, 'modconv2d: w must reside on the same device as x')
        n, cin, h, wd = x.shape
        per_image = (w.ndim == 5)
        if per_image:
            _require(w.shape[0] == n and styles is None, 'modconv2d: per-image weights need w.shape[0] == batch and styles=None')
        cout, cin2, k, k2 = w.shape[-4:]
        _require(cin == cin2 and k == k2 and k in (1, 3), 'modconv2d: weight must be [cout, cin, k, k] with k in {1, 3}')
        _require(mode in (0, 1, 2), 'modconv2d: mode must be 0, 1 or 2')
        _require(mode != 1 or (k == 3 and h >= 3 and wd >= 3), 'modconv2d: mode 1 is a 3x3 stride-2 convolution on an input of at least 3x3')
        oh, ow = (2 * h + 1, 2 * wd + 1) if mode == 2 else (((h - 3) // 2 + 1, (wd - 3) // 2 + 1) if mode == 1 else (h, wd))
        pitch = (ow + 3) // 4 * 4 if (pad_rows and mode == 2) else ow
        y = torch.empty([n, cout, oh, pitch], dtype=torch.float32, device=x.device)
        lib = load()
        arith = int(arith) or int(lib.ide3d_get_conv_arithmetic())
        if arith == 16 and x_amax is None:
            arith = 6
        p, ent, keep = ModconvPlugin._params(lib, x, w, y, styles, dcoefs, noise, noise_strength, bias, act, alpha, gain, clamp, mode, arith, x_amax, y_amax)
        p.y_pitch = pitch if pitch != ow else 0
        with _dev_guard(x.device):
            rc = lib.ide3d_modconv2d(ctypes.byref(p), _stream(x))
        _check(rc, 'modconv2d')
        ModconvPlugin._ws.mark_packed(ent, () if per_image else (w,))
        return y if pitch == ow else y[..., :ow]

    @staticmethod
    def modconv2d_heads(x, w, styles, dcoefs, noise, noise_strength, bias, act, alpha, gain, clamp, head_w, head_bias, head_clamp,
                        want_x=True, arith=0):
        for t in (x, w, head_w):
            _require(t.is_cuda and t.dtype == torch.float32 and t.is_contiguous(), 'modconv2d_heads: contiguous float32 CUDA tensors required')
        n, cin, h, wd = x.shape
        cout = w.shape[0]
        _require(w.ndim == 4 and tuple(w.shape[1:]) == (cin, 3, 3), 'modconv2d_heads: w must be [cout, cin, 3, 3]')
        _require(head_w.ndim == 5 and head_w.shape[0] == n and head_w.shape[2] == cout and tuple(head_w.shape[3:]) == (1, 1),
                 'modconv2d_heads: head_w must be [n, rows, cout, 1, 1]')
        lib = load()
        arith = int(arith) or int(lib.ide3d_get_conv_arithmetic())
        if arith == 16:
            arith = 6
        rows = head_w.shape[1]
        shape_key = (n, cin, cout, h, wd, rows, arith)
        knob_off = 'IDE3D_MODCONV_NO_HEAD_FUSION' in os.environ
        if knob_off or shape_key in ModconvPlugin._heads_declined:
            return None
        y = torch.empty([n, cout, h, wd], dtype=torch.float32, device=x.device) if want_x else None
        heads = torch.empty([n, rows, h, wd], dtype=torch.float32, device=x.device)
        p, ent, keep = ModconvPlugin._params(lib, x, w, y, styles, dcoefs, noise, noise_strength, bias, act, alpha, gain, clamp, 0, arith, None, None)
        hent = ModconvPlugin._workspace(lib, heads, head_w, n, cout, rows, h, wd, 1, 0, True, arith)
        e = _ModconvHeadEpilogue()
        e.w, e.y, e.rows, e.clamp, e.no_activation_output = head_w.data_ptr(), heads.data_ptr(), rows, float(head_clamp), int(not want_x)
        if head_bias is not None:
            head_bias = head_bias.contiguous()
            _require(head_bias.is_cuda and head_bias.dtype == torch.float32 and head_bias.numel() == rows, 'modconv2d_heads: head_bias must be float32 [rows] on GPU')
            e.bias = head_bias.data_ptr()
        e.workspace, e.workspace_bytes = hent[0].data_ptr(), hent[0].numel() * 4
        with _dev_guard(x.device):
            rc = lib.ide3d_modconv2d_heads(ctypes.byref(p), ctypes.byref(e), _stream(x))
        if rc == -2:
            ModconvPlugin._heads_declined.add(shape_key)
            return None
        _check(rc, 'modconv2d_heads')
        ModconvPlugin._ws.mark_packed(ent, (w,))
        return y, heads


class ModconvGradPlugin:

    @staticmethod
    def _f32(t, name, dev, shape=None):
        _require(t.is_cuda and t.dtype == torch.float32 and t.device == dev, f'{name} must be float32 on the device of the gradient')
        if shape is not None:
            _require(tuple(t.shape) == tuple(shape), f'{name} must be {list(shape)}, got {list(t.shape)}')
        return t

    @staticmethod
    def act_backward(dy, y, act, alpha, gain, clamp, noise=None, noise_strength=1.0, bias=None, dcoefs=None):
        dev = dy.device
        ModconvGradPlugin._f32(dy, 'dy', dev)
        _require(dy.ndim == 4 and dy.is_contiguous(), 'act_backward: dy must be a contiguous [n, c, h, w] tensor')
        n, c, h, w = dy.shape
        ModconvGradPlugin._f32(y, 'y', dev, dy.shape)
        _require(y.stride(3) == 1 and y.stride(2) >= w and y.stride(1) == h * y.stride(2) and y.stride(0) == c * y.stride(1),
                 'act_backward: y must be dense apart from padded rows')
        _require(act in (0, 1, 3), 'act_backward: act must be 0 (dot only), 1 (linear) or 3 (lrelu)')
        _require(act != 0 or dcoefs is not None, 'act_backward: the dot-only form needs dcoefs')
        lib = load()
        p = _ActBwdParams()
        keep = []
        p.dy, p.y = dy.data_ptr(), y.data_ptr()
        p.y_pitch = y.stride(2) if y.stride(2) != w else 0
        dz = torch.empty_like(dy) if act != 0 else None
        if dz is not None:
            p.dz = dz.data_ptr()
        if noise is not None:
            noise = ModconvGradPlugin._f32(noise, 'noise', dev).contiguous(); keep.append(noise)
            _require(noise.numel() == h * w, 'act_backward: noise must be [h, w]')
            p.noise = noise.data_ptr()
        p.noise_strength = float(noise_strength)
        if bias is not None:
            bias = ModconvGradPlugin._f32(bias, 'bias', dev, (c,)).contiguous(); keep.append(bias)
            p.bias = bias.data_ptr()
        dd = ws = None
        if dcoefs is not None:
            dcoefs = ModconvGradPlugin._f32(dcoefs, 'dcoefs', dev, (n, c)).contiguous(); keep.append(dcoefs)
            dd = torch.empty([n, c], dtype=torch.float32, device=dev)
            nbytes = lib.ide3d_act_bwd_workspace_bytes(n, c, h, w)
            _require(nbytes > 0, 'act_backward: unsupported shape')
            ws = torch.empty([nbytes // 4], dtype=torch.float32, device=dev)
            p.dcoefs, p.ddcoefs, p.workspace, p.workspace_bytes = dcoefs.data_ptr(), dd.data_ptr(), ws.data_ptr(), nbytes
        p.n, p.c, p.h, p.w = n, c, h, w
        p.act, p.alpha, p.gain, p.clamp = int(act), float(alpha), float(gain), float(clamp)
        with _dev_guard(dev):
            rc = lib.ide3d_modconv_act_backward(ctypes.byref(p), _stream(dy))
        _check(rc, 'modconv_act_backward')
        return dz, dd

    @staticmethod
    def scale_dot(x, t, styles):
        dev = t.device
        ModconvGradPlugin._f32(t, 't', dev)
        _require(t.ndim == 4 and t.is_contiguous(), 'scale_dot: t must be a contiguous [n, c, h, w] tensor')
        n, c, h, w = t.shape
        x = ModconvGradPlugin._f32(x, 'x', dev, t.shape).contiguous()
        styles = ModconvGradPlugin._f32(styles, 'styles', dev, (n, c)).contiguous()
        lib = load()
        dx = torch.empty_like(t)
        ds = torch.empty([n, c], dtype=torch.float32, device=dev)
        nbytes = lib.ide3d_act_bwd_workspace_bytes(n, c, h, w)
        _require(nbytes > 0, 'scale_dot: unsupported shape')
        ws = torch.empty([nbytes // 4], dtype=torch.float32, device=dev)
        with _dev_guard(dev):
            rc = lib.ide3d_modconv_scale_dot(_ptr(x), _ptr(t), _ptr(styles), _ptr(dx), _ptr(ds), n, c, h, w, _ptr(ws), nbytes, _stream(t))
        _check(rc, 'modconv_scale_dot')
        return dx, ds

    @staticmethod
    def head_weight_grad(dy, x):
        dev = dy.device
        ModconvGradPlugin._f32(dy, 'dy', dev)
        _require(dy.ndim == 4 and x.ndim == 4 and x.shape[0] == dy.shape[0] and x.shape[2:] == dy.shape[2:], 'head_weight_grad: dy [n, rows, h, w], x [n, cin, h, w]')
# ... 1116 lines not shown
    def cam2world(forward, origin, lookat=None):
        _require(origin.is_cuda and origin.dtype == torch.float32 and origin.ndim == 2 and origin.shape[1] == 3, 'cam2world: origin must be float32 [n, 3] on a CUDA device')
        origin = origin.contiguous()
        n = origin.shape[0]
        stride = 0
        if lookat is not None:
            _require(lookat.dtype == torch.float32 and lookat.device == origin.device and lookat.numel() in (3, 3 * n), 'cam2world: lookat must hold 3 or 3 n float32 values on the same device')
            lookat = lookat.contiguous()
            stride = 3 if (lookat.numel() == 3 * n and n > 1) else 0
        else:
            _require(forward is not None and forward.dtype == torch.float32 and forward.device == origin.device and tuple(forward.shape) == (n, 3),
                     'cam2world: forward must be float32 [n, 3] on the same device')
            forward = forward.contiguous()
        out = torch.empty([n, 4, 4], dtype=torch.float32, device=origin.device)
        with _dev_guard(origin.device):
            rc = load().ide3d_cam2world(_ptr(forward if lookat is None else None), _ptr(origin), _ptr(lookat), stride, n, _ptr(out), _stream(origin))
        _check(rc, 'cam2world')
        return out


class MappingPlugin:
    MAX_N, MAX_WIDTH, MAX_LAYERS = 8, 1024, 16
    _ws = _Workspaces()

    @staticmethod
    def supports(n, z_dim, embed, widths, device=None):
        k0 = z_dim + embed
        if not (1 <= n <= MappingPlugin.MAX_N and 0 < k0 <= MappingPlugin.MAX_WIDTH and k0 % 4 == 0 and 1 <= len(widths) <= MappingPlugin.MAX_LAYERS
                and all(0 < w <= MappingPlugin.MAX_WIDTH and w % 4 == 0 for w in widths)):
            return False
        with _dev_guard(device):
            return bool(load().ide3d_mapping_supported())

    @staticmethod
    def mapping(z, c, embed_w, embed_b, embed_wgain, embed_bgain, fc_ws, fc_bs, lr_multiplier, alpha, act_gain, num_ws, w_avg, psi, cutoff, trusted=False):
        dev = z.device
        if trusted:
            _require(z.is_cuda and z.dtype == torch.float32 and z.is_contiguous() and (c is None or (c.device == dev and c.dtype == torch.float32 and c.is_contiguous()
                                                                                                 and tuple(c.shape) == (z.shape[0], embed_w.shape[1]))),
                     'mapping: z / c must be contiguous float32 tensors on one CUDA device, c [n, c_dim]')
            return MappingPlugin._launch(z, c, embed_w, embed_b, embed_wgain, embed_bgain, fc_ws, fc_bs, lr_multiplier, alpha, act_gain, num_ws, w_avg, psi, cutoff)
        f32c = lambda t: t is None or (t.is_cuda and t.device == dev and t.dtype == torch.float32 and t.is_contiguous())
        _require(all(f32c(t) for t in (z, c, embed_w, embed_b, w_avg, *fc_ws, *fc_bs)), 'mapping: contiguous float32 tensors on one CUDA device required')
        n, z_dim = z.shape
        embed = 0 if embed_w is None else embed_w.shape[0]
        _require(MappingPlugin.supports(n, z_dim, embed, [w.shape[0] for w in fc_ws], device=dev), 'mapping: unsupported shape')
        _require((embed_w is None) or (c is not None and embed_w.ndim == 2 and tuple(c.shape) == (n, embed_w.shape[1])),
                 f'mapping: c must be [{n}, {None if embed_w is None else embed_w.shape[1]}] (got {None if c is None else tuple(c.shape)})')
        _require(embed_b is None or (embed_w is not None and tuple(embed_b.shape) == (embed,)), 'mapping: embed bias must be [embed]')
        _require(w_avg is None or w_avg.numel() == fc_ws[-1].shape[0], 'mapping: w_avg must have w_dim elements')
        _require(num_ws >= 1, 'mapping: num_ws must be positive')
        k = z_dim + embed
        for w, b in zip(fc_ws, fc_bs):
            _require(w.ndim == 2 and w.shape[1] == k and (b is None or tuple(b.shape) == (w.shape[0],)), 'mapping: layer widths do not chain')
            k = w.shape[0]
        return MappingPlugin._launch(z, c, embed_w, embed_b, embed_wgain, embed_bgain, fc_ws, fc_bs, lr_multiplier, alpha, act_gain, num_ws, w_avg, psi, cutoff)

    @staticmethod
    def _launch(z, c, embed_w, embed_b, embed_wgain, embed_bgain, fc_ws, fc_bs, lr_multiplier, alpha, act_gain, num_ws, w_avg, psi, cutoff):
        dev = z.device
        n, z_dim = z.shape
        embed = 0 if embed_w is None else embed_w.shape[0]
        k = fc_ws[-1].shape[0]
        lib = load()
        wsp = MappingPlugin._ws.entry((dev.index, _ws_domain(dev)), lambda: torch.zeros([lib.ide3d_mapping_workspace_bytes() // 4 + 4], dtype=torch.float32, device=dev))[0]
        out = torch.empty([n, num_ws, k], dtype=torch.float32, device=dev)
        p = _MappingParams()
        p.z, p.c = z.data_ptr(), (c.data_ptr() if c is not None else 0)
        p.embed_w, p.embed_b = (embed_w.data_ptr() if embed_w is not None else 0), (embed_b.data_ptr() if embed_b is not None else 0)
        for i, (w, b) in enumerate(zip(fc_ws, fc_bs)):
            p.fc_w[i], p.fc_b[i], p.fc_out[i] = w.data_ptr(), (b.data_ptr() if b is not None else 0), w.shape[0]
        p.w_avg = w_avg.data_ptr() if w_avg is not None else 0
        p.ws, p.workspace, p.workspace_bytes = out.data_ptr(), wsp.data_ptr(), wsp.numel() * 4
        p.n, p.z_dim, p.c_dim, p.embed, p.layers, p.num_ws = n, z_dim, (c.shape[1] if c is not None else 0), embed, len(fc_ws), num_ws
        p.embed_weight_gain, p.embed_bias_gain, p.lr_multiplier = float(embed_wgain), float(embed_bgain), float(lr_multiplier)
        p.alpha, p.act_gain, p.truncation_psi = float(alpha), float(act_gain), float(psi)
        p.truncation_cutoff = -1 if cutoff is None else int(cutoff)
        with _dev_guard(dev):
            rc = lib.ide3d_mapping(ctypes.byref(p), _stream(z))
        _check(rc, 'mapping')
        return out


class ResamplePlugin:
    @staticmethod
    def skip_upsample_add_cl(lo, add):
        _require(lo.is_cuda and lo.dtype == torch.float32 and add.dtype == torch.float32 and add.device == lo.device,
                 'skip_upsample_add_cl: float32 CUDA tensors on one device required')
        n, c, h, w = lo.shape
        _require(tuple(add.shape) == (n, c, 2 * h, 2 * w), 'skip_upsample_add_cl: add must be [n, c, 2h, 2w]')
        _require(c % 4 == 0, 'skip_upsample_add_cl: channel count must be a multiple of 4')
        out = torch.empty([n, c, 2 * h, 2 * w], dtype=torch.float32, device=lo.device, memory_format=torch.channels_last)
        with _dev_guard(lo.device):
            rc = load().ide3d_skip_upsample_add_cl(_ptr(lo), ctypes.byref(_i64x4(lo.stride())), _ptr(add), ctypes.byref(_i64x4(add.stride())),
                                                   n, c, h, w, _ptr(out), _stream(lo))
        _check(rc, 'skip_upsample_add_cl')
        return out

    @staticmethod
    def bilinear_up2_split(x, ranges, adjacent=None):
        _require(x.is_cuda and x.dtype == torch.float32, 'bilinear_up2_split: float32 CUDA tensor required')
        _require(1 <= len(ranges) <= 3, 'bilinear_up2_split: one to three channel ranges')
        x = x.contiguous()
        n, c, h, w = x.shape
        outs = [None if (adjacent and k in adjacent) else torch.empty([n, cnt, 2 * h, 2 * w], dtype=torch.float32, device=x.device) for k, (_b, cnt) in enumerate(ranges)]
        bs = [0, 0, 0]
        if adjacent:
            i, j = adjacent
            _require(j == i + 1 and 0 <= i and j < len(ranges), 'bilinear_up2_split: adjacent outputs must be consecutive')
            ci, cj = ranges[i][1], ranges[j][1]
            both = torch.empty([n, ci + cj, 2 * h, 2 * w], dtype=torch.float32, device=x.device)
            outs[i], outs[j] = both[:, :ci], both[:, ci:]
            bs[i] = bs[j] = (ci + cj) * 4 * h * w
        dst = (ctypes.c_void_p * 3)(*([o.data_ptr() for o in outs] + [0] * (3 - len(outs))))
        bsa = (ctypes.c_int64 * 3)(*bs)
        beg = (ctypes.c_int32 * 3)(*([int(b) for b, _c in ranges] + [0] * (3 - len(outs))))
        cnt = (ctypes.c_int32 * 3)(*([int(c_) for _b, c_ in ranges] + [0] * (3 - len(outs))))
        with _dev_guard(x.device):
            rc = load().ide3d_bilinear_up2_split(_ptr(x), n, c, h, w, ctypes.byref(dst), ctypes.byref(beg), ctypes.byref(cnt), ctypes.byref(bsa), _stream(x))
        _check(rc, 'bilinear_up2_split')
        return outs


class LowresPlugin:
    _ws = _Workspaces(limit=64)

    @staticmethod
    def layers_supported(n, C, res0, ups, arith=0):
        arr = (ctypes.c_int32 * len(ups))(*[int(u) for u in ups])
        return int(load().ide3d_lowres_layers_supported(int(n), int(C), int(res0), arr, len(ups), int(arith)))

    @staticmethod
    def phase_r_plan(n, C, res0, ups, arith=0):
        arr = (ctypes.c_int32 * len(ups))(*[int(u) for u in ups])
        bands, scratch = (ctypes.c_int32 * len(ups))(), (ctypes.c_int64 * len(ups))()
        fit = int(load().ide3d_lowres_phase_r_plan(int(n), int(C), int(res0), arr, len(ups), int(arith), bands, scratch))
        return [(int(bands[l]), int(scratch[l])) for l in range(fit)]

    @staticmethod
    def group(x0, layers, heads, fir, arith=0):
        lib = load()
        n, C = layers[0]['styles'].shape
        dev = x0.device
        _require(1 <= len(layers) <= LOWRES_MAX_LAYERS and len(heads) <= LOWRES_MAX_HEADS, 'lowres_group: too many layers / heads')
        _require(x0.is_cuda and x0.dtype == torch.float32 and x0.is_contiguous() and x0.shape[-3] == C and x0.shape[-1] == x0.shape[-2], 'lowres_group: x0 must be contiguous float32 [C, r, r] or [n, C, r, r]')
        _require(fir.is_cuda and fir.dtype == torch.float32 and fir.is_contiguous() and tuple(fir.shape) == (4, 4) and fir.device == dev, 'lowres_group: fir must be a float32 [4, 4] filter on the device of x0')
        arith = int(arith) or int(lib.ide3d_get_conv_arithmetic())
        p = _LowresParams()
        p.x0, p.x0_batch_stride = x0.data_ptr(), (x0.stride(0) if x0.ndim == 4 else 0)
        p.fir = fir.data_ptr()
        p.n, p.C, p.res0, p.nlayers, p.nheads, p.arith = n, C, x0.shape[-1], len(layers), len(heads), arith
        keep, res, head_res = [], x0.shape[-1], {}
        for l, L in enumerate(layers):
            q = p.layers[l]
            w = L['weight']
            _require(w.is_cuda and w.dtype == torch.float32 and w.is_contiguous() and tuple(w.shape) == (C, C, 3, 3) and w.device == dev, f'lowres_group: layer {l}: weight must be contiguous float32 [C, C, 3, 3]')
            q.weight = w.data_ptr()
            res = res * 2 if int(L['up']) == 2 else res
            for name, shape in (('styles', (n, C)), ('dcoefs', (n, C)), ('noise', (res, res)), ('bias', (C,))):
                t = L.get(name)
                if t is None:
                    _require(name in ('noise', 'bias'), f'lowres_group: layer {l}: {name} is required')
                    continue
                t = t.contiguous(); keep.append(t)
                _require(t.is_cuda and t.dtype == torch.float32 and tuple(t.shape) == shape and t.device == dev, f'lowres_group: layer {l}: {name} must be float32 {shape} on the device of x0')
                setattr(q, name, t.data_ptr())
            q.act_gain, q.clamp, q.up, q.head = float(L['act_gain']), float(L['clamp']), int(L['up']), int(L.get('head', -1))
            if q.head >= 0:
                head_res[q.head] = res
        key = (tuple(L['weight'].data_ptr() for L in layers), n, C, x0.shape[-1], tuple(int(L['up']) for L in layers), dev.index, _ws_domain(dev), arith)
        def alloc():
            nbytes = lib.ide3d_lowres_workspace_bytes(ctypes.byref(p))
            _require(nbytes > 0, 'lowres_group: unsupported configuration')
            return torch.zeros([nbytes // 4 + 1], dtype=torch.float32, device=dev)
        ent = LowresPlugin._ws.entry(key, alloc)
        weights = [L['weight'] for L in layers]
        for l, packed in enumerate(LowresPlugin._ws.packed(ent, weights)):
            p.layers[l].weights_packed = int(packed)
# ... 50 lines not shown
```

### ide-3d_amd/training/graph_cache.py

```python

import collections
import contextlib
import os
import threading
import warnings
import weakref

import torch

_tls = threading.local()
_caches = weakref.WeakKeyDictionary()
_pools = {}

STATS = collections.Counter()


_PASS_ENV = ('IDE3D_NO_SKIP_MERGE', 'IDE3D_NO_STYLE_PREFETCH', 'IDE3D_NO_STYLE_BATCH', 'IDE3D_NO_LOWRES_GROUP')


def _env_int(name, default):
    try:
        return int(os.environ.get(name, default))
    except ValueError:
        return default


def enabled():
    return os.environ.get('IDE3D_AUTO_GRAPH', '1') != '0' and not getattr(_tls, 'off', 0)


@contextlib.contextmanager
def disabled():
    _tls.off = getattr(_tls, 'off', 0) + 1
    try:
        yield
    finally:
        _tls.off -= 1


def reset(module=None):
    if module is None:
        for c in list(_caches.values()):
            c.clear()
    elif module in _caches:
        _caches[module].clear()


def stats(module):
    c = _caches.get(module)
    return {'graphs': 0 if c is None else len(c.entries), 'seen': 0 if c is None else len(c.seen)}


def tree_stamp(root):
    acc = []
    push = acc.append
    requires_grad = False
    hooked = False
    stack = [root]
    while stack:
        m = stack.pop()
        if m._forward_hooks or m._forward_pre_hooks:
            hooked = True
        for p in m._parameters.values():
            if p is not None:
                push(p._version); push(p.data_ptr())
                if p.requires_grad:
                    requires_grad = True
        for b in m._buffers.values():
            if b is not None:
                push(b._version); push(b.data_ptr())
        for sub in m._modules.values():
            if sub is not None:
                stack.append(sub)
    return hash(tuple(acc)), requires_grad, hooked


def _global_hooks():
    mod = torch.nn.modules.module
    return bool(getattr(mod, '_global_forward_hooks', None)) or bool(getattr(mod, '_global_forward_pre_hooks', None))


class _Captured:
    __slots__ = ('graph', 'ws', 'c', 'jitter', 'jitter_given', 'out', 'planes', 'tensors', 'aliases', 'versions', '__weakref__')

    def untouched(self):
        v = 0
        for t in self.tensors:
            v += t._version
        return v == self.versions


class _ModuleGraphs:
    def __init__(self):
        self.entries = collections.OrderedDict()
        self.seen = {}
        self.stamp = None
        self.evictions = 0
        self.lock = threading.RLock()

    def clear(self):
# ... 224 lines not shown
```

### ide-3d_amd/training/networks.py

```python

import math

import numpy as np
import torch

from dnnlib import util
from torch_utils import custom_ops
from torch_utils import misc
from torch_utils import persistence
from torch_utils.ops import bias_act
from torch_utils.ops import conv2d_resample
from torch_utils.ops import fma
from torch_utils.ops import upfirdn2d

_modconv_plugin = None

use_hip_modconv = True


def _upfirdn_plugin():
    upfirdn2d._init()
    return upfirdn2d._plugin


# ... 448 lines not shown
    if not (lay.weight.shape[2:] == (3, 3) and lay.padding == 1 and lay.up in (1, 2) and lay.activation in ('linear', 'lrelu') and x.ndim == 4
            and styles.shape[0] == x.shape[0]):
        return None
    oh, ow = lay.up * x.shape[2], lay.up * x.shape[3]
    noise_const = getattr(lay, 'noise_const', None)
    map_grad = noise_const is not None and noise_const.requires_grad
    map_used = map_grad and noise is not None and noise.ndim == 2 and tuple(noise_const.shape) == (oh, ow)
    if (map_grad and not (hip_noise_grad and map_used)) or not _conv_grad_ok(x, styles, *_layer_params(lay), noise_map=(noise_const if map_used else None)):
        return None
    gh, gw = (oh + 1, ow + 1) if lay.up == 2 else (oh, ow)
    if x.shape[0] * lay.weight.shape[0] * gh * gw >= 2 ** 31 or x.numel() >= 2 ** 31:
        return None
    if noise is not None and not (noise.ndim == 2 and tuple(noise.shape) == (oh, ow) and (hip_param_grad or map_used or not noise.requires_grad)):
        return None
    if lay.resample_filter.requires_grad:
        return None
    if dcoefs is None:
        dcoefs = _demod_coefs(lay.weight, styles)
    bias = lay.bias.to(x.dtype)
    if lay.up == 1:
        return _ModconvActGrad.apply(x, styles, dcoefs, lay.weight, noise, bias, lay.activation, act_gain, act_clamp)
    return _ModconvUpGrad.apply(x, styles, dcoefs, lay.weight, lay.resample_filter, noise, bias, lay.activation, act_gain, act_clamp)


def _folded_head_weights(torgb, toseg, w):
    if not (w.ndim == 2 and w.stride(1) == 1 and torgb.weight.shape[2] == 1
            and _inference_on_gpu(w, torgb.weight, toseg.weight, torgb.affine.weight, torgb.affine.bias, toseg.affine.weight, toseg.affine.bias)
            and _style_init()):
        return None
    return _style_plugin.fold_heads(w, torgb.affine.weight_gain,
                                    torgb.affine.weight, torgb.affine.bias, torgb.weight.reshape(torgb.weight.shape[0], -1), torgb.weight_gain,
                                    toseg.affine.weight, toseg.affine.bias, toseg.weight.reshape(toseg.weight.shape[0], -1), toseg.weight_gain)


def _adjacent_views(a, b):
    if a is None or b is None or a._base is None or a._base is not b._base:
        return None
    t = a._base
    if (t.ndim != 4 or a.ndim != 4 or b.ndim != 4 or not t.is_contiguous() or t.shape[1] != a.shape[1] + b.shape[1]
            or a.shape[0] != t.shape[0] or a.shape[2:] != t.shape[2:] or b.shape[0] != t.shape[0] or b.shape[2:] != t.shape[2:]
            or a.stride() != t.stride() or b.stride() != t.stride()
            or a.data_ptr() != t.data_ptr() or b.data_ptr() != t.data_ptr() + a.shape[1] * t.stride(1) * t.element_size()):
        return None
    return t


def _dual_head_weights(torgb, toseg, w):
    wcat = _take_prefetched(torgb, w) if _prefetch_table() else None
    if wcat is None:
        wcat = _folded_head_weights(torgb, toseg, w)
    if wcat is None:
        s_rgb = torgb.affine(w) * torgb.weight_gain
        s_seg = toseg.affine(w) * toseg.weight_gain
        wr = torgb.weight[None, :, :, 0, 0] * s_rgb[:, None, :]
        ws = toseg.weight[None, :, :, 0, 0] * s_seg[:, None, :]
        wcat = torch.cat([wr, ws], dim=1)[:, :, :, None, None].contiguous()
    return wcat


def _dual_head(x, torgb, toseg, w, wcat=None):
    if (hip_conv_grad and torch.is_grad_enabled() and torgb.weight.shape[2] == 1 and torgb.conv_clamp == toseg.conv_clamp and x.ndim == 4
            and w.ndim == 2 and w.shape[0] == x.shape[0] and x.numel() < 2 ** 31
            and x.shape[0] * (torgb.weight.shape[0] + toseg.weight.shape[0]) * x.shape[2] * x.shape[3] < 2 ** 31
            and _conv_grad_ok(x, w, *_head_params(torgb, toseg))):
        y = _DualHeadGrad.apply(x, _dual_head_weights(torgb, toseg, w), _cat_cached(torgb.bias, toseg.bias),
                                -1.0 if torgb.conv_clamp is None else torgb.conv_clamp)
        co = torgb.weight.shape[0]
        return y[:, :co], y[:, co:]
    if not (use_hip_modconv and torgb.weight.shape[2] == 1 and torgb.conv_clamp == toseg.conv_clamp
            and _inference_on_gpu(x, w, *_head_params(torgb, toseg)) and _modconv_init()):
        return None
    n = x.shape[0]
    if w.shape[0] != n:
        return None
    if wcat is None:
        wcat = _dual_head_weights(torgb, toseg, w)
    bias = _cat_cached(torgb.bias, toseg.bias)
    clamp = -1.0 if torgb.conv_clamp is None else torgb.conv_clamp
    y = _modconv_plugin.modconv2d(x.contiguous(), wcat, None, None, None, 0.0, bias, 1, 0.0, 1.0, clamp)
    co = torgb.weight.shape[0]
    return y[:, :co], y[:, co:]


def _conv1_dual_head(block, x, w1, w_shared, want_x, noise_mode='random', gain=1, input_noise=None, **unused):
    c1, tr, ts = block.conv1, block.torgb, block.toseg
    if not (use_hip_modconv and type(c1) is SynthesisLayer and c1.up == 1 and c1.padding == 1 and c1.weight.shape[2:] == (3, 3)
            and c1.activation in ('linear', 'lrelu') and tr.weight.shape[2] == 1 and tr.conv_clamp == ts.conv_clamp
            and x.ndim == 4 and x.shape[0] == w1.shape[0] == w_shared.shape[0]
            and _inference_on_gpu(x, w1, w_shared, *_layer_params(c1), *_head_params(tr, ts))
            and not _hooked(block, c1, tr, ts) and _modconv_init()):
        return None
    from torch_utils import hip_plugin
    if hip_plugin.conv_arithmetic() != 'bf16x6':
        return None
    noise = None
    if c1.use_noise and noise_mode != 'none':
        if input_noise is not None or noise_mode != 'const' or tuple(c1.noise_const.shape) != tuple(x.shape[2:]):
            return None
        noise = _scaled_const_noise(c1.noise_const, c1.noise_strength)
    styles, dcoefs = _styles_and_dcoefs(c1.affine, w1, c1.weight, True)
    if dcoefs is None:
        dcoefs = _demod_coefs(c1.weight, styles)
    spec = bias_act.activation_funcs[c1.activation]
    act_gain = c1.act_gain * gain
    act_clamp = c1.conv_clamp * gain if c1.conv_clamp is not None else None
    bias = c1.bias.to(x.dtype)
    wcat = _dual_head_weights(tr, ts, w_shared)
    hbias = _cat_cached(tr.bias, ts.bias)
    hclamp = -1.0 if tr.conv_clamp is None else tr.conv_clamp
    xc = x.contiguous()
    out = _modconv_plugin.modconv2d_heads(xc, c1.weight.contiguous(), styles.contiguous(), dcoefs, noise, 1.0, bias,
                                          spec.cuda_idx, spec.def_alpha, act_gain, -1.0 if act_clamp is None else act_clamp,
                                          wcat, hbias, hclamp, want_x=want_x)
    if out is None:
        x = _modconv_bias_act(x, c1.weight, styles, True, noise, 1.0, bias, c1.activation, act_gain, act_clamp, dcoefs=dcoefs)
        return x, _dual_head(x, tr, ts, w_shared, wcat=wcat)
    x, y = out
    co = tr.weight.shape[0]
    return x, (y[:, :co], y[:, co:])


_lowres_plugin = None


def _lowres_init():
    global _lowres_plugin
    if _lowres_plugin is None:
        _lowres_plugin = custom_ops.get_plugin(module_name='lowres_plugin', sources=['lowres.hip'])
    return True


def _hooked(*modules):
    from torch.nn.modules import module as _m
    if _m._global_forward_hooks or _m._global_forward_pre_hooks:
        return True
    return any(m._forward_hooks or m._forward_pre_hooks for m in modules)


def lowres_group_forward(blocks, ws_per_block, noise_mode='const', force_fp32=False, **other_kwargs):
    if os.environ.get('IDE3D_NO_LOWRES_GROUP') or not use_hip_modconv or other_kwargs or noise_mode not in ('const', 'none'):
        return None
    if not blocks or len(blocks) != len(ws_per_block):
        return None
    b0 = blocks[0]
    ws0 = ws_per_block[0]
    if not (torch.is_tensor(ws0) and ws0.is_cuda and ws0.dtype == torch.float32) or (torch.is_grad_enabled() and ws0.requires_grad):
        return None
    if b0.in_channels != 0 or b0.use_single_layer or not hasattr(b0, 'const') or not _inference_on_gpu(b0.const, b0.conv1.weight):
        return None
    from torch_utils import hip_plugin
    if hip_plugin.conv_arithmetic() not in ('bf16x6', 'bf16x3'):
        return None
    C, n = b0.out_channels, ws0.shape[0]
    if C % 32 != 0 or n > 8:
        return None
    cand = []
    for bi, blk in enumerate(blocks):
        ok = (blk.architecture == 'skip' and not blk.use_single_layer and blk.out_channels == C and (bi == 0 or blk.in_channels == C)
              and not (blk.use_fp16 and not force_fp32) and not getattr(blk, 'skip_channels_last', False)
              and blk.torgb.conv_clamp == blk.toseg.conv_clamp and blk.torgb.weight.shape[2] == 1 and blk._filter_is_1331()
              and blk.resolution == b0.resolution << bi
              and not _hooked(blk, blk.conv1, blk.torgb, blk.toseg, *([blk.conv0] if bi else [])))
        if ok and torch.is_grad_enabled():
            ok = _inference_on_gpu(ws_per_block[bi], *([blk.const] if bi == 0 else _layer_params(blk.conv0)), *_layer_params(blk.conv1),
                                   *_head_params(blk.torgb, blk.toseg))
        if not ok:
            break
        for name in (('conv1',) if bi == 0 else ('conv0', 'conv1')):
            lay = getattr(blk, name)
            if not (lay.activation == 'lrelu' and lay.weight.shape == (C, C, 3, 3) and lay.padding == 1 and lay.up == (2 if name == 'conv0' else 1)
                    and _inference_on_gpu(ws0, lay.weight, lay.bias) and lay.weight.is_contiguous()
                    and (not lay.use_noise or noise_mode == 'none' or lay.noise_const.shape[-1] == blk.resolution)):
                ok = False
                break
            cand.append((bi, name, lay))
        if not ok:
            cand = [c for c in cand if c[0] < bi]
            break
    if not cand or not _lowres_init():
        return None
    ups = [lay.up for _, _, lay in cand]
    fit = _lowres_plugin.layers_supported(n, C, b0.resolution, ups)
    if fit < 1:
        return None
    cand = cand[:fit]
    last_bi, last_name, _ = cand[-1]
    resume = last_name == 'conv0'
    nheads = last_bi if resume else last_bi + 1
    if nheads > hip_plugin.LOWRES_MAX_HEADS or (nheads == 0):
        return None
    layers, heads = [], []
    for bi, name, lay in cand:
        blk, wsb = blocks[bi], ws_per_block[bi]
        w = wsb[:, (0 if (bi == 0 or name == 'conv0') else 1)]
        styles, dcoefs = _styles_and_dcoefs(lay.affine, w, lay.weight, True)
        noise = None
# ... 383 lines not shown
        if self.up == 1:
            if noise is None or (const_noise and input_noise is None and noise.shape == x.shape[2:]):
                y = _modconv_bias_act(x, self.weight, styles, True, noise, 1.0,
                                      self.bias.to(x.dtype), self.activation, act_gain, act_clamp, dcoefs=dcoefs_pre)
                if y is not None:
                    return y
        x = modulated_conv2d(x=x, weight=self.weight, styles=styles, noise=noise, up=self.up, padding=self.padding,
                             resample_filter=(self.resample_filter if self.up > 1 else None), flip_weight=(self.up == 1),
                             fused_modconv=(fused_modconv and not _inference_on_gpu(x, self.weight, styles)))
        return bias_act.bias_act(x, self.bias.to(x.dtype), act=self.activation, gain=act_gain, clamp=act_clamp)


@persistence.persistent_class
class ToRGBLayer(torch.nn.Module):

    def __init__(self, in_channels, out_channels, w_dim, kernel_size=1, conv_clamp=None, channels_last=False, **unused):
        super().__init__()
        self.conv_clamp = conv_clamp
        self.affine = FullyConnectedLayer(w_dim, in_channels, bias_init=1)
        memory_format = torch.channels_last if channels_last else torch.contiguous_format
        self.weight = torch.nn.Parameter(torch.randn([out_channels, in_channels, kernel_size, kernel_size]).to(memory_format=memory_format))
        self.bias = torch.nn.Parameter(torch.zeros([out_channels]))
        self.weight_gain = 1 / np.sqrt(in_channels * (kernel_size ** 2))

    def forward(self, x, w, fused_modconv=True):
        styles = self.affine(w) * self.weight_gain
        if x.size(0) > styles.size(0):
            assert x.size(0) % styles.size(0) == 0
            styles = styles.repeat_interleave(x.size(0) // styles.size(0), dim=0)
        y = _modconv_bias_act(x, self.weight, styles, False, None, 0.0, self.bias.to(x.dtype), 'linear', 1.0, self.conv_clamp)
        if y is not None:
            return y
        x = modulated_conv2d(x=x, weight=self.weight, styles=styles, demodulate=False, fused_modconv=fused_modconv)
        return bias_act.bias_act(x, self.bias.to(x.dtype), clamp=self.conv_clamp)


@persistence.persistent_class
class SegSynthesisBlock(torch.nn.Module):

    def __init__(self, in_channels, out_channels, w_dim, resolution, img_channels, seg_channels, is_last,
                 architecture='skip', resample_filter=[1, 3, 3, 1], conv_clamp=None, use_fp16=False,
                 fp16_channels_last=False, use_single_layer=False, disable_upsample=False, **layer_kwargs):
        assert architecture in ['orig', 'skip']
        super().__init__()
        self.in_channels, self.out_channels = in_channels, out_channels
        self.w_dim, self.resolution = w_dim, resolution
        self.img_channels, self.seg_channels = img_channels, seg_channels
        self.is_last, self.architecture = is_last, architecture
        self.use_fp16 = use_fp16
        self.channels_last = (use_fp16 and fp16_channels_last)
        self.use_single_layer = use_single_layer
        self.register_buffer('resample_filter', upfirdn2d.setup_filter(resample_filter))
        self.num_conv = self.num_torgb = self.num_toseg = 0
        layer_name = layer_kwargs.pop('layer_name', 'training.networks.SynthesisLayer')

        if in_channels == 0:
            self.const = torch.nn.Parameter(torch.randn([out_channels, resolution, resolution]))
        else:
            self.conv0 = util.construct_class_by_name(
                class_name=layer_name, in_channels=in_channels, out_channels=out_channels, w_dim=w_dim,
                resolution=resolution, up=(1 if disable_upsample else 2), resample_filter=resample_filter,
                conv_clamp=conv_clamp, channels_last=self.channels_last, **layer_kwargs)
            self.num_conv += 1
        if not use_single_layer:
            self.conv1 = util.construct_class_by_name(
                class_name=layer_name, in_channels=out_channels, out_channels=out_channels, w_dim=w_dim,
                resolution=resolution, conv_clamp=conv_clamp, channels_last=self.channels_last, **layer_kwargs)
            self.num_conv += 1
        if is_last or architecture == 'skip':
            self.torgb = ToRGBLayer(out_channels, img_channels, w_dim=w_dim, conv_clamp=conv_clamp, channels_last=self.channels_last)
            self.num_torgb += 1
            self.toseg = ToRGBLayer(out_channels, seg_channels, w_dim=w_dim, conv_clamp=conv_clamp, channels_last=self.channels_last)
            self.num_toseg += 1

    def _merge_skip(self, skip, x):
        if skip is None:
            return None
        if skip.size(-1) * 2 == x.size(-1):
            return upfirdn2d.upsample2d(skip, self.resample_filter)
        if skip.size(-1) == x.size(-1):
            return skip
        raise NotImplementedError

    def _accumulate(self, lo, cur, y):
        if lo is not None:
            if (getattr(self, 'skip_channels_last', False) and lo.shape[1] % 4 == 0 and self.resample_filter.shape == (4, 4)
                    and _inference_on_gpu(lo, y) and self._filter_is_1331() and _resample_init()):
                return _resample_plugin.skip_upsample_add_cl(lo, y)
            f = self.resample_filter
            return _upfirdn_plugin().upfirdn2d_ex(lo, f, 2, 2, 1, 1, 2, 1, 2, 1, False, 4.0, add=y)
        return cur.add_(y) if cur is not None else y

    def _filter_is_1331(self):
        ok = getattr(self, '_f1331', None)
        if ok is None:
            ref = upfirdn2d.setup_filter([1, 3, 3, 1])
            ok = self._f1331 = bool(torch.equal(self.resample_filter.detach().cpu(), ref))
        return ok

    def forward(self, x, img, seg, ws, force_fp32=False, fused_modconv=None, block_noise=None, disable_rgb=False, **layer_kwargs):
        misc.assert_shape(ws, [None, self.num_conv + self.num_torgb, self.w_dim])
        resume_after_conv0 = bool(layer_kwargs.pop('_resume_after_conv0', False))
        x_unused = bool(layer_kwargs.pop('_x_unused', False))
        ws_list = ws.unbind(dim=1)
        w_iter = iter(ws_list)
        dtype = torch.float16 if self.use_fp16 and not force_fp32 else torch.float32
        memory_format = torch.channels_last if self.channels_last and not force_fp32 else torch.contiguous_format
        out_dtype = dtype
        if dtype == torch.float16 and ws.is_cuda and not torch.is_grad_enabled() and use_hip_modconv:
            dtype, memory_format = torch.float32, torch.contiguous_format
        if fused_modconv is None:
            with misc.suppress_tracer_warnings():
                fused_modconv = (not self.training) and (dtype == torch.float32 or int(ws.shape[0]) == 1)

        fused = fused_heads = None
        if self.in_channels == 0:
            x = self.const.to(dtype=dtype, memory_format=memory_format)
            x = x.unsqueeze(0).expand(ws.shape[0], *x.size())
            if not self.use_single_layer:
                layer_kwargs['input_noise'] = block_noise[:, 1:2] if block_noise is not None else None
                x = self.conv1(x, next(w_iter), fused_modconv=fused_modconv, **layer_kwargs)
        else:
            x = x.to(dtype=dtype, memory_format=memory_format)
            layer_kwargs['input_noise'] = block_noise[:, 0:1] if block_noise is not None else None
            if resume_after_conv0:
                next(w_iter)
            else:
                x = self.conv0(x, next(w_iter), fused_modconv=fused_modconv, **layer_kwargs)
            if not self.use_single_layer:
                layer_kwargs['input_noise'] = block_noise[:, 1:2] if block_noise is not None else None
                w1 = next(w_iter)
                if (self.is_last or self.architecture == 'skip') and not disable_rgb and dtype == torch.float32:
                    fused = _conv1_dual_head(self, x, w1, ws_list[self.num_conv], not x_unused, **layer_kwargs)
                if fused is not None:
                    x, fused_heads = fused
                else:
                    x = self.conv1(x, w1, fused_modconv=fused_modconv, **layer_kwargs)

        w_shared = next(w_iter) if (self.is_last or self.architecture == 'skip') else None
        ref = x if x is not None else fused_heads[0]
        img_lo = seg_lo = None
        heads_follow = (self.is_last or self.architecture == 'skip') and not disable_rgb
        if (heads_follow and _inference_on_gpu(ref, img, seg, w_shared, *_head_params(self.torgb, self.toseg)) and img is not None and seg is not None
                and img.size(-1) * 2 == ref.size(-1)):
            img_lo, seg_lo, img, seg = img, seg, None, None
        else:
            img = self._merge_skip(img, ref)
            seg = self._merge_skip(seg, ref)
        if self.is_last or self.architecture == 'skip':
            if disable_rgb:
                img = seg = None
            else:
                heads = fused_heads if fused_heads is not None else _dual_head(x, self.torgb, self.toseg, w_shared)
                if heads is not None:
                    y, y_seg = heads
                else:
                    y = self.torgb(x, w_shared, fused_modconv=fused_modconv).to(dtype=torch.float32, memory_format=torch.contiguous_format)
                    y_seg = self.toseg(x, w_shared, fused_modconv=fused_modconv).to(dtype=torch.float32, memory_format=torch.contiguous_format)
                lo_both, y_both = _adjacent_views(img_lo, seg_lo), _adjacent_views(y, y_seg)
                if (lo_both is not None and y_both is not None and img is None and seg is None and not getattr(self, 'skip_channels_last', False)
                        and not self.is_last and not os.environ.get('IDE3D_NO_SKIP_MERGE')):
                    both = self._accumulate(lo_both, None, y_both)
                    img, seg = both[:, :y.shape[1]], both[:, y.shape[1]:]
                else:
                    img = self._accumulate(img_lo, img, y)
                    seg = self._accumulate(seg_lo, seg, y_seg)
        assert x is None or x.dtype == dtype
        if x is not None and out_dtype != dtype:
            x = x.to(out_dtype)
        assert img is None or img.dtype == torch.float32
        assert seg is None or seg.dtype == torch.float32
        return x, img, seg
```

### ide-3d_amd/training/triplane.py

```python

import contextlib
import dataclasses
import math
import os
from typing import Dict, List, Optional

import numpy as np
import torch

from dnnlib import util
from torch_utils import misc
from torch_utils import persistence
from torch_utils.ops import bias_act
from training import graph_cache
from training import networks
from training import volumetric_rendering as vr

fused_render_grad = True

fused_render_param_grad = False

fused_render_camera_grad = False

fused_hierarchical = False
# ... 80 lines not shown
        for name, layer in (('geo_w0', self.geo0), ('geo_w1', self.geo1), ('tex_w0', self.tex0), ('tex_w1', self.tex1)):
            if layer.weight.is_cuda and layer.weight.dtype == torch.float32 and not (torch.is_grad_enabled() and layer.weight.requires_grad):
                w = networks._scaled_weight(layer.weight, layer.weight_gain)
                b = layer.bias if layer.bias_gain == 1 else networks._scaled_weight(layer.bias, layer.bias_gain)
            else:
                w, b = layer.effective(torch.float32)
            out[name] = w.contiguous()
            out[name.replace('_w', '_b')] = b.contiguous()
        return out


@persistence.persistent_class
class TriplaneRenderer(torch.nn.Module):

    def __init__(self, spec: GeneratorSpec):
        super().__init__()
        self.spec = spec
        self.decoder = TriplaneDecoder(spec.plane_channels, spec.decoder_hidden, spec.feature_channels, spec.seg_channels)

    def sample_voxel(self, img_v, seg_v, pts, sigma_only=False, ray_grid=None):
        if self._hip_ok(img_v, seg_v, pts):
            vr._init()
            tex, geo = _as_channels_last(img_v), _as_channels_last(seg_v)
            out = vr._plugin.sample_voxel(tex, geo, self.decoder.kernel_weights(), pts.float(), sigma_only=sigma_only)
            if out is not None:
                return out
        geo_feat = util.sample_from_triplane(pts, seg_v, ray_grid=ray_grid)
        tex_feat = util.sample_from_triplane(pts, img_v, ray_grid=ray_grid)
        out = self.decoder(tex_feat, geo_feat)
        return out[:, -1] if sigma_only else out

    def density_lattice(self, img_v, seg_v, n, voxel_size, corner, scale, first, count):
        if self._hip_ok(img_v, seg_v):
            vr._init()
            out = vr._plugin.density_lattice(_as_channels_last(img_v), _as_channels_last(seg_v), self.decoder.kernel_weights(),
                                             n, voxel_size, corner, scale, first, count)
            if out is not None:
                return out
        from training import shape_extraction
        pts = shape_extraction.lattice_points(n, voxel_size, corner, scale, first, count, img_v.device)
        return self.sample_voxel(img_v, seg_v, pts.unsqueeze(0).expand(img_v.shape[0], -1, -1), sigma_only=True)

    def _hip_ok(self, *tensors):
        if any(t.device.type != 'cuda' or t.dtype != torch.float32 for t in tensors):
            return False
        if not torch.is_grad_enabled():
            return True
        return not (any(t.requires_grad for t in tensors) or any(p.requires_grad for p in self.decoder.parameters()))

    def _fused_grad_ok(self, img_v, seg_v, cam2world, jitter, sigma_noise):
        if fused_render_param_grad:
            return self._fused_param_grad_ok(img_v, seg_v, cam2world, jitter, sigma_noise)
        cam_grad = fused_render_camera_grad and cam2world.requires_grad
        if not torch.is_grad_enabled() or not (img_v.requires_grad or seg_v.requires_grad or cam_grad):
            return False
        if any(t.device.type != 'cuda' or t.dtype != torch.float32 for t in (img_v, seg_v, cam2world)):
            return False
        if (cam2world.requires_grad and not cam_grad) or any(p.requires_grad for p in self.decoder.parameters()):
            return False
        return not any(t is not None and t.requires_grad for t in (jitter, sigma_noise))

    def _fused_param_grad_ok(self, img_v, seg_v, cam2world, jitter, sigma_noise):
        params = list(self.decoder.parameters())
        cam_grad = fused_render_camera_grad and cam2world.requires_grad
        if not torch.is_grad_enabled() or not (img_v.requires_grad or seg_v.requires_grad or cam_grad or any(p.requires_grad for p in params)):
            return False
        if any(t.device.type != 'cuda' or t.dtype != torch.float32 for t in (img_v, seg_v, cam2world, *params)):
            return False
        if cam2world.requires_grad and not cam_grad:
            return False
        return not any(t is not None and t.requires_grad for t in (jitter, sigma_noise))

    def _fused_hier_grad_ok(self, img_v, seg_v, cam2world, jitter, sigma_noise, importance_u):
        params = list(self.decoder.parameters())
        param_grad = any(p.requires_grad for p in params)
        if not torch.is_grad_enabled() or not (img_v.requires_grad or seg_v.requires_grad or (fused_render_param_grad and param_grad)):
            return False
        if not _all_fp32_cuda(img_v, seg_v, cam2world, *(params if fused_render_param_grad else ())):
            return False
        if param_grad and not fused_render_param_grad:
            return False
        return not any(t is not None and t.requires_grad for t in (cam2world, jitter, sigma_noise, importance_u))

    def forward(self, img_v, seg_v, cam2world, fov=None, num_steps=None, ray_start=None, ray_end=None, img_size=None,
                nerf_noise=0.0, jitter=None, sigma_noise=None, white_back=False, clamp_mode=None,
                hierarchical=None, importance_u=None, sigma_noise_fine=None, **unused):
        sp = self.spec
        fov = sp.fov if fov is None else fov
        steps = sp.num_steps if num_steps is None else num_steps
        t0 = sp.ray_start if ray_start is None else ray_start
        t1 = sp.ray_end if ray_end is None else ray_end
        size = sp.render_size if img_size is None else img_size
        clamp_mode = sp.clamp_mode if clamp_mode is None else clamp_mode
        n, device = img_v.shape[0], img_v.device
        rays = size * size
        if jitter is None:
            jitter = torch.rand([n, rays, steps], device=device)
        elif jitter is False:
            jitter = None
        if sigma_noise is None and nerf_noise:
            sigma_noise = torch.randn([n, rays, steps], device=device) * nerf_noise
        for name, t in (('jitter', jitter), ('sigma_noise', sigma_noise)):
            if t is not None and tuple(t.shape) != (n, rays, steps):
                raise ValueError(f'TriplaneRenderer: {name} must be [images, rays, steps] = [{n}, {rays}, {steps}] for this call, got {list(t.shape)}')

        hierarchical = sp.hierarchical if hierarchical is None else hierarchical
        if not hierarchical and self._hip_ok(img_v, seg_v, cam2world):
            res = vr.render_triplane_fused(_as_channels_last(img_v), _as_channels_last(seg_v), self.decoder.kernel_weights(),
                                           cam2world.float(), fov, (size, size), steps, t0, t1, jitter=jitter,
                                           sigma_noise=sigma_noise, clamp_mode=clamp_mode, white_back=white_back)
            if res is not None:
                return res
        elif not hierarchical and fused_render_grad and self._fused_grad_ok(img_v, seg_v, cam2world, jitter, sigma_noise):
            res = vr.render_triplane_fused(_as_channels_last(img_v), _as_channels_last(seg_v), self.decoder.kernel_weights(),
                                           cam2world.float(), fov, (size, size), steps, t0, t1, jitter=jitter,
                                           sigma_noise=sigma_noise, clamp_mode=clamp_mode, white_back=white_back)
            if res is not None:
                return res
        elif hierarchical and fused_hierarchical and sigma_noise_fine is None \
                and self._hip_ok(img_v, seg_v, cam2world, *(() if importance_u is None else (importance_u,))):
            res = vr.render_triplane_hierarchical(_as_channels_last(img_v), _as_channels_last(seg_v), self.decoder.kernel_weights(),
                                                  cam2world.float(), fov, (size, size), steps, t0, t1, jitter=jitter,
                                                  sigma_noise=sigma_noise, importance_u=importance_u, clamp_mode=clamp_mode,
                                                  white_back=white_back)
            if res is not None:
                return res
        elif hierarchical and fused_hierarchical_grad and sigma_noise_fine is None \
                and self._fused_hier_grad_ok(img_v, seg_v, cam2world, jitter, sigma_noise, importance_u):
            res = vr.render_triplane_hierarchical(_as_channels_last(img_v), _as_channels_last(seg_v), self.decoder.kernel_weights(),
                                                  cam2world.float(), fov, (size, size), steps, t0, t1, jitter=jitter,
                                                  sigma_noise=sigma_noise, importance_u=importance_u, clamp_mode=clamp_mode,
                                                  white_back=white_back)
            if res is not None:
                return res

        points, z_vals, rays_d_cam = vr.get_initial_rays_trig(n, steps, device, fov, (size, size), t0, t1)
        pts, z_vals, rays_d, rays_o, _p, _y = vr.transform_sampled_points(
            points, z_vals, rays_d_cam, device, h_stddev=0, v_stddev=0, camera=cam2world, mode=None,
            jitter=(jitter.unsqueeze(-1) if jitter is not None else torch.full_like(z_vals, 0.5)))
        out = self.sample_voxel(img_v, seg_v, pts.reshape(n, -1, 3), ray_grid=(size, size, steps)).reshape(n, rays, steps, -1)
        noise = sigma_noise.unsqueeze(-1) if sigma_noise is not None else None
        integrate = lambda o, z, nz: vr.fancy_integration(o, rays_d_cam, z, device, noise_std=(1.0 if nz is not None else 0.0),
                                                          white_back=white_back, clamp_mode=clamp_mode, noise=nz)
        if hierarchical:
            with torch.no_grad():
                _f, _d, w = integrate(out, z_vals, noise)
                w = w.reshape(n * rays, steps) + 1e-5
                z = z_vals.reshape(n * rays, steps)
                z_fine = vr.sample_pdf(0.5 * (z[:, :-1] + z[:, 1:]), w[:, 1:-1], steps, det=False, u=importance_u)
                z_fine = z_fine.reshape(n, rays, steps, 1)
                pts_fine = rays_o.unsqueeze(2) + rays_d.unsqueeze(2) * z_fine
            out_fine = self.sample_voxel(img_v, seg_v, pts_fine.reshape(n, -1, 3)).reshape(n, rays, steps, -1)
            z_vals = torch.cat([z_fine, z_vals], 2)
            z_vals, order = torch.sort(z_vals, dim=2)
            out = torch.gather(torch.cat([out_fine, out], 2), 2, order.expand(-1, -1, -1, out.shape[-1]))
            noise = sigma_noise_fine.unsqueeze(-1) if sigma_noise_fine is not None else None
        feat, depth, weights = integrate(out, z_vals, noise)
        feat = feat.permute(0, 2, 1).reshape(n, -1, size, size)
        depth = depth.permute(0, 2, 1).reshape(n, 1, size, size)
        wsum = weights.sum(2).permute(0, 2, 1).reshape(n, 1, size, size)
        return feat, depth, wsum


def _as_channels_last(t):
    return t if t.stride(1) == 1 else t.contiguous(memory_format=torch.channels_last)


def _all_fp32_cuda(*tensors):
    return all(t.device.type == 'cuda' and t.dtype == torch.float32 for t in tensors)


@persistence.persistent_class
class TriplaneSynthesisNetwork(torch.nn.Module):

    def __init__(self, spec: GeneratorSpec):
        super().__init__()
        self.spec = spec
        self.w_dim = spec.w_dim
        self.img_resolution = spec.img_resolution
        self.img_channels = spec.img_channels
        self.seg_channels = spec.seg_channels
        self.render_size = spec.render_size
        self.voxel_block_resolutions = spec.voxel_resolutions()
        self.block_resolutions = spec.sr_resolutions()
        plane_ch = 3 * spec.plane_channels
        layer_kwargs = dict(layer_name='training.networks.SynthesisLayer')
        conv_clamp = spec.conv_clamp if (spec.conv_clamp is not None or spec.num_fp16_res == 0) else 256
        fp16_from = (spec.plane_resolution >> max(spec.num_fp16_res - 1, 0)) if spec.num_fp16_res > 0 else None

        self.num_ws = 0
        for res in self.voxel_block_resolutions:
            cin = spec.voxel_width(res // 2) if res > 4 else 0
            block = VoxelBlock(cin, spec.voxel_width(res), w_dim=spec.w_dim, resolution=res, img_channels=plane_ch,
                               seg_channels=plane_ch, is_last=False, architecture='skip', conv_clamp=conv_clamp,
                               use_fp16=(fp16_from is not None and res >= max(fp16_from, 8)), **layer_kwargs)
            self.num_ws += block.num_conv
            setattr(self, f'vb{res}', block)

        getattr(self, f'vb{self.voxel_block_resolutions[-1]}').skip_channels_last = True
        self.renderer = TriplaneRenderer(spec)
        self.style_prefetch = True

        widths = spec.sr_widths()
        cin = spec.feature_channels
        for res in self.block_resolutions:
            is_last = (res == self.img_resolution)
            block = networks.SegSynthesisBlock(cin, widths[res], w_dim=spec.w_dim, resolution=res,
                                               img_channels=spec.img_channels, seg_channels=spec.seg_channels,
                                               is_last=is_last, architecture='skip', conv_clamp=conv_clamp,
                                               use_fp16=(spec.num_fp16_res > 0), **layer_kwargs)
            self.num_ws += block.num_conv
            if is_last:
                self.num_ws += block.num_torgb
            setattr(self, f'b{res}', block)
            cin = widths[res]

    def split_ws(self, ws):
        with torch.autograd.profiler.record_function('split_ws'):
            misc.assert_shape(ws, [None, self.num_ws, self.w_dim])
            ws = ws.to(torch.float32)
            voxel_ws, block_ws, w_idx = [], [], 0
            for res in self.voxel_block_resolutions:
                block = getattr(self, f'vb{res}')
                voxel_ws.append(ws.narrow(1, w_idx, block.num_conv + block.num_torgb))
                w_idx += block.num_conv
            for res in self.block_resolutions:
                block = getattr(self, f'b{res}')
                block_ws.append(ws.narrow(1, w_idx, block.num_conv + block.num_torgb))
                w_idx += block.num_conv
        return voxel_ws, block_ws

    def backbone(self, voxel_ws, **block_kwargs):
        x_v = img_v = seg_v = None
        blocks = [getattr(self, f'vb{res}') for res in self.voxel_block_resolutions]
        start, resume = 0, False
        grp = networks.lowres_group_forward(blocks, voxel_ws, **block_kwargs) if (voxel_ws and torch.is_tensor(voxel_ws[0]) and voxel_ws[0].is_cuda) else None
        if grp is not None:
            x_v, img_v, seg_v, start, resume = grp
        for i, (block, cur_ws) in enumerate(zip(blocks, voxel_ws)):
            if i < start:
                continue
            extra = dict(_resume_after_conv0=True) if (resume and i == start) else {}
            if i == len(blocks) - 1:
                extra['_x_unused'] = True
            x_v, img_v, seg_v = block(x_v, img_v, cur_ws, condition_img=seg_v, **block_kwargs, **extra)
        return img_v, seg_v

    @contextlib.contextmanager
    def _pass_scope(self, ws, voxel_and_sr):
        voxel, sr = voxel_and_sr
        prefetch = (getattr(self, 'style_prefetch', True) and ws.is_cuda and not torch.is_grad_enabled()
                    and torch.cuda.is_current_stream_capturing() and not os.environ.get('IDE3D_NO_STYLE_PREFETCH'))
        side = None
        arena = networks.amax_arena(ws.shape[0], ws.device)
        arena.__enter__()
        try:
            if prefetch:
                side = networks.side_stream(ws.device)
                todo = [(getattr(self, f'vb{r}'), w) for r, w in voxel] + [(getattr(self, f'b{r}'), w) for r, w in sr]
                networks.prefetch_styles(todo, side)
            yield
        finally:
            arena.__exit__(None, None, None)
            if side is not None:
                networks.finish_prefetch(side)

    def planes(self, ws, noise_mode='const', force_fp32=False):
        def impl(ws_, _c, _jitter, _planes):
            voxel_ws, _ = self.split_ws(ws_)
            with self._pass_scope(ws_, (list(zip(self.voxel_block_resolutions, voxel_ws)), [])):
                return self.backbone(voxel_ws, noise_mode=noise_mode, force_fp32=force_fp32)

        if torch.is_tensor(ws) and ws.is_cuda:
            return graph_cache.run(self, impl, ws, None, {}, noise_mode, (), force_fp32, False, None, {}, kind='backbone')
        return impl(ws, None, False, None)

    def superres(self, feat, block_ws, **block_kwargs):
        fc = self.spec.feature_channels
        size = self.block_resolutions[0] // 2
        if (size == 2 * feat.shape[-1] and size == 2 * feat.shape[-2] and feat.shape[-1] % 2 == 0 and networks._inference_on_gpu(feat)
                and networks._resample_init()):
            x, img, seg = networks._resample_plugin.bilinear_up2_split(
                feat, [(0, fc), (0, self.img_channels), (fc, feat.shape[1] - fc)], adjacent=(1, 2))
        else:
            up = lambda t: torch.nn.functional.interpolate(t, size=(size, size), mode='bilinear', align_corners=False)
            x = up(feat[:, :fc])
            img = up(feat[:, :self.img_channels])
            seg = up(feat[:, fc:])
        last = len(self.block_resolutions) - 1
        for i, (res, cur_ws) in enumerate(zip(self.block_resolutions, block_ws)):
            extra = dict(_x_unused=True) if i == last else {}
            x, img, seg = getattr(self, f'b{res}')(x, img, seg, cur_ws, **block_kwargs, **extra)
        return img, seg

    def forward(self, ws, c=None, render_params=None, noise_mode='const', return_seg=False, return_raw=False,
                return_dict=False, force_fp32=False, cond_img=None, ray_jitter=None, cached_planes=None, **unused):
        assert c is not None, 'synthesis needs the 25-D camera label c'
        render_params = dict(render_params or {})
        flags = (bool(return_seg), bool(return_raw), bool(return_dict))

        def impl(ws_, c_, jitter_, planes_):
            return self._forward_impl(ws_, c_, render_params, noise_mode, flags, force_fp32, jitter_, planes_)

        if torch.is_tensor(ws) and ws.is_cuda:
            return graph_cache.run(self, impl, ws, c, render_params, noise_mode, flags, force_fp32, ray_jitter, cached_planes, unused)
        return impl(ws, c, ray_jitter, cached_planes)

    def _forward_impl(self, ws, c, render_params, noise_mode, flags, force_fp32, ray_jitter, cached_planes):
        return_seg, return_raw, return_dict = flags
        voxel_ws, block_ws = self.split_ws(ws)
        block_kwargs = dict(noise_mode=noise_mode, force_fp32=force_fp32)
        with self._pass_scope(ws, ([] if cached_planes is not None else list(zip(self.voxel_block_resolutions, voxel_ws)), list(zip(self.block_resolutions, block_ws)))):
            if cached_planes is not None:
                img_v, seg_v = cached_planes
            else:
                img_v, seg_v = self.backbone(voxel_ws, **block_kwargs)
            cam2world = c[:, :16].reshape(-1, 4, 4).to(torch.float32)
            feat, depth, wsum = self.renderer(
                img_v, seg_v, cam2world, fov=render_params.get('fov'), num_steps=render_params.get('num_steps'),
                ray_start=render_params.get('ray_start'), ray_end=render_params.get('ray_end'),
                nerf_noise=render_params.get('nerf_noise', 0.0), jitter=ray_jitter,
                hierarchical=render_params.get('hierarchical'), importance_u=render_params.get('importance_u'))
            img, seg = self.superres(feat, block_ws, **block_kwargs)
        img_raw = feat[:, :self.img_channels]
        if return_dict:
            return dict(image=img, image_seg=seg, image_raw=img_raw, image_depth=depth, planes=(img_v, seg_v))
        if return_seg and return_raw:
            return img, seg, img_raw
        if return_seg:
            return img, seg
        if return_raw:
            return img, img_raw
        return img


@persistence.persistent_class
class TriPlaneGenerator(torch.nn.Module):

    def __init__(self, spec: Optional[GeneratorSpec] = None, **spec_overrides):
        super().__init__()
        if spec is None:
            spec = GeneratorSpec(**spec_overrides)
        elif spec_overrides:
            spec = dataclasses.replace(spec, **spec_overrides)
        self.spec = spec
        self.z_dim, self.c_dim, self.w_dim = spec.z_dim, spec.c_dim, spec.w_dim
        self.img_resolution, self.img_channels = spec.img_resolution, spec.img_channels
        self.synthesis = TriplaneSynthesisNetwork(spec)
        self.num_ws = self.synthesis.num_ws
        self.mapping = networks.MappingNetwork(z_dim=spec.z_dim, c_dim=spec.c_dim, w_dim=spec.w_dim, num_ws=self.num_ws,
                                               num_layers=spec.mapping_layers)

    def forward(self, z, c, truncation_psi=1, truncation_cutoff=None, **synthesis_kwargs):
        ws = self.mapping(z, c, truncation_psi=truncation_psi, truncation_cutoff=truncation_cutoff)
        return self.synthesis(ws, c=c, **synthesis_kwargs)



INTRINSICS = (4.2647, 0.0, 0.5, 0.0, 4.2647, 0.5, 0.0, 0.0, 1.0)


def conditioning_label(device='cpu'):
    pose = [1, 0, 0, 0, 0, 1, 0, 0, 0, 0, 1, 2.7, 0, 0, 0, 1]
    return vr.device_const(pose + list(INTRINSICS), torch.float32, device).reshape(1, -1).clone()


def camera_label(yaw, pitch=math.pi * 0.5, radius=2.7, device='cpu'):
    cam, _phi, _theta = vr.sample_camera_positions(device, n=1, r=radius, horizontal_mean=yaw + math.pi * 0.5,
                                                   vertical_mean=pitch, mode=None)
    c2w = vr.create_cam2world_matrix(-cam, cam, device=device).reshape(1, -1)
    return torch.cat((c2w, vr.device_const(INTRINSICS, torch.float32, device).reshape(1, -1)), -1)


class GraphedRenderer:

    def __init__(self, G, batch, device, truncation_psi=1.0, noise_mode='const', warmup=3, ray_jitter=None, conv_arithmetic=None,
                 static_labels=False):
        self.G = G
        self.psi, self.noise_mode = truncation_psi, noise_mode
        self.static_labels = bool(static_labels)
        self.z_copied = torch.cuda.Event() if torch.device(device).type == 'cuda' else None
        restore = None
        if conv_arithmetic is not None:
            from torch_utils import hip_plugin
            restore = hip_plugin.conv_arithmetic()
            hip_plugin.conv_arithmetic(conv_arithmetic)
        try:
            self._capture(G, batch, device, warmup, ray_jitter)
        finally:
            if restore is not None:
                hip_plugin.conv_arithmetic(restore)

    def _capture(self, G, batch, device, warmup, ray_jitter):
        self.z = torch.zeros([batch, G.z_dim], dtype=torch.float32, device=device)
        self.c_cond = conditioning_label(device).repeat(batch, 1)
        self.c_cam = conditioning_label(device).repeat(batch, 1)
        sp = G.synthesis.spec
        if ray_jitter is False:
            self.jitter = None
        else:
# ... 58 lines not shown
```

### include/ide3d_hip.h

```cpp
#ifndef IDE3D_HIP_H_
#define IDE3D_HIP_H_

#include <stdint.h>

#ifdef __cplusplus
extern "C" {
#endif


#define IDE3D_OK            0
#define IDE3D_EINVAL       (-1)
#define IDE3D_ENOKERNEL    (-2)
#define IDE3D_ELAUNCH      (-3)

#define IDE3D_F32  0
#define IDE3D_F16  1
#define IDE3D_BF16 2
#define IDE3D_F64  3

const char* ide3d_last_error(void);
int         ide3d_abi_version(void);
const char* ide3d_build_arch(void);
const char* ide3d_build_flags(void);
int         ide3d_exclusive_violations(void);
// ... 190 lines not shown

int ide3d_render_ray_weights(const ide3d_render_params* p, float* weights, float* z_vals, float* pdf_bins, float* pdf_weights,
                             void* stream);
int ide3d_merge_depths(const float* z_fine, const float* z_coarse, int64_t rays, int32_t steps_fine, int32_t steps_coarse,
                       float* z_all, int32_t* src, void* stream);
int ide3d_render_rays_merged(const ide3d_render_params* p, const float* z_all, const int32_t* src, const float* z_fine,
                             int32_t total_steps, void* stream);

int64_t ide3d_render_merged_param_grad_workspace_bytes(const ide3d_render_params* p);
int ide3d_render_rays_merged_backward(const ide3d_render_params* p, const float* z_all, const int32_t* src, const float* z_fine,
                                      int32_t total_steps, const ide3d_render_grads* g, const ide3d_render_param_grads* q, void* stream);

int ide3d_sample_voxel(const ide3d_render_params* p, const float* pts, int64_t m,
                       float* out, float* out_sigma, int sigma_only, void* stream);

typedef struct ide3d_lattice {
    int32_t n;
    float   voxel_size;
    float   corner[3];
    float   scale;
} ide3d_lattice;

int ide3d_lattice_points(const ide3d_lattice* lat, int64_t first, int64_t count, float* pts, void* stream);

int ide3d_density_lattice(const ide3d_render_params* p, const ide3d_lattice* lat, int64_t first, int64_t count,
                          float* out_sigma, void* stream);

int64_t ide3d_mesh_workspace_bytes(int32_t X, int32_t Y, int32_t Z);
int ide3d_mesh_count(const float* volume, int32_t X, int32_t Y, int32_t Z, float iso, const uint8_t* table,
                     void* workspace, int64_t workspace_bytes, void* stream);
int ide3d_mesh_emit(const float* volume, int32_t X, int32_t Y, int32_t Z, float iso, const uint8_t* table,
                    const ide3d_lattice* lat, int32_t flip, void* workspace, int64_t workspace_bytes,
                    int64_t num_vertices, int64_t num_triangles, float* vertices, int32_t* triangles, float* normals, void* stream);

#define IDE3D_RASTER_CULL_NONE  0
#define IDE3D_RASTER_CULL_BACK  1
#define IDE3D_RASTER_CULL_FRONT 2
#define IDE3D_RASTER_BEHIND     1
#define IDE3D_RASTER_OUTSIDE    2
#define IDE3D_RASTER_BAD_INDEX  1
#define IDE3D_RASTER_DROPPED    2
int64_t ide3d_raster_workspace_bytes(int32_t N, int64_t V, int32_t H, int32_t W);
int ide3d_raster_project(const float* vertices, int64_t V, const float* world2cam, int32_t N, int32_t H, int32_t W, float fx, float fy,
                         float sx, float ox, float sy, float oy, float near, void* workspace, int64_t workspace_bytes, void* stream);
int ide3d_raster_depth(const int32_t* triangles, int64_t T, int64_t V, int32_t N, int32_t H, int32_t W, int32_t cull,
                       int32_t large_min, void* workspace, int64_t workspace_bytes, void* stream);
int ide3d_raster_shade(const float* vertices, const int32_t* triangles, int64_t V, int32_t N, int32_t H, int32_t W,
                       const float* normals, const uint8_t* colors, const int32_t* labels, const float* light, int32_t two_sided,
                       float ambient, float diffuse, const float* base_color, float bg, const void* workspace, int64_t workspace_bytes,
                       float* depth, int32_t* triangle, float* image, int32_t* label, void* stream);

typedef struct ide3d_modconv_params {
    const float* x; const float* w; const float* styles; const float* dcoefs;
    const float* noise; const float* bias; float* y;
    int32_t n, cin, cout, h, w_, k;
    float noise_strength;
    int32_t act; float alpha, gain, clamp;
    int32_t mode;
    int32_t weights_packed;
    float*  workspace;
    int64_t workspace_bytes;
    int64_t w_batch_stride;
    int32_t arith;
    const float* x_amax;
    float*       y_amax;
    int32_t      y_pitch;
} ide3d_modconv_params;

int64_t ide3d_modconv_workspace_bytes(int32_t n, int32_t cin, int32_t cout, int32_t h, int32_t w, int32_t k, int32_t mode,
                                      int32_t per_image_weights);
int ide3d_modconv2d(const ide3d_modconv_params* p, void* stream);

typedef struct ide3d_modconv_head_epilogue {
    const float* w;
    const float* bias;
    float*       y;
    int32_t      rows;
    float        clamp;
    int32_t      no_activation_output;
    float*       workspace;
    int64_t      workspace_bytes;
} ide3d_modconv_head_epilogue;
int ide3d_modconv2d_heads(const ide3d_modconv_params* p, const ide3d_modconv_head_epilogue* heads, void* stream);

typedef struct ide3d_act_bwd_params {
    const float* dy;
    const float* y;
    float*       dz;
    const float* noise;
    float        noise_strength;
    const float* bias;
    const float* dcoefs;
    float*       ddcoefs;
    int32_t      n, c, h, w, y_pitch;
    int32_t      act;
    float        alpha, gain, clamp;
    float*       workspace;
    int64_t      workspace_bytes;
} ide3d_act_bwd_params;

int64_t ide3d_act_bwd_workspace_bytes(int32_t n, int32_t c, int32_t h, int32_t w);
int ide3d_modconv_act_backward(const ide3d_act_bwd_params* p, void* stream);

int ide3d_modconv_scale_dot(const float* x, const float* t, const float* styles, float* dx, float* dstyles,
                            int32_t n, int32_t c, int32_t h, int32_t w, float* workspace, int64_t workspace_bytes, void* stream);

int64_t ide3d_head_wgrad_workspace_bytes(int32_t n, int32_t rows, int32_t cin, int32_t h, int32_t w);
int ide3d_head_weight_grad(const float* dy, const float* x, float* dw, int32_t n, int32_t rows, int32_t cin, int32_t h, int32_t w,
                           float* workspace, int64_t workspace_bytes, void* stream);

typedef struct ide3d_wgrad_params {
    const float* g;
    const float* x;
    const float* styles;
    const float* dcoefs;
    float*       dw;
    int32_t      n, cin, cout, h, w;
    int32_t      mode;
    int32_t      arith;
    float*       workspace;
    int64_t      workspace_bytes;
} ide3d_wgrad_params;

int64_t ide3d_wgrad_workspace_bytes(int32_t n, int32_t cin, int32_t cout, int32_t h, int32_t w);
int ide3d_modconv_weight_grad(const ide3d_wgrad_params* p, void* stream);

int64_t ide3d_bias_noise_workspace_bytes(int32_t n, int32_t c, int32_t h, int32_t w);
int ide3d_bias_noise_grad(const float* dz, float* db, float* dnoise, int32_t n, int32_t c, int32_t h, int32_t w,
                          float* workspace, int64_t workspace_bytes, void* stream);

enum { IDE3D_PLAN_FP32 = 0,
       IDE3D_PLAN_SPLIT = 1,
       IDE3D_PLAN_SPLIT_TEAMS = 2,
       IDE3D_PLAN_HEAD_SPLIT = 3,
       IDE3D_PLAN_HEAD_RESIDENT = 4,
       IDE3D_PLAN_HEAD_SMALL = 5 };
typedef struct ide3d_modconv_plan_info {
    int32_t kind;
    int32_t tile_h, tile_w;
    int32_t images_per_tile;
    int32_t rows;
    int32_t waves;
    int32_t parts, f16;
    int32_t split_k;
    int32_t strip;
    int32_t transposed_all_class;
    int32_t reserved;
    int64_t workgroups;
} ide3d_modconv_plan_info;
int ide3d_modconv_plan(const ide3d_modconv_params* p, ide3d_modconv_plan_info* out);

int     ide3d_set_conv_arithmetic(int32_t arith);
int32_t ide3d_get_conv_arithmetic(void);

int ide3d_style_demod(const float* w, int64_t w_stride, const float* affine_w, const float* affine_b, const float* wsq_t,
                      int32_t n, int32_t cin, int32_t cout, int32_t wdim, float affine_gain, float bias_gain,
                      float* styles, float* dcoefs, void* stream);

int ide3d_fold_heads(const float* w, int64_t w_stride, int32_t n, int32_t cin, int32_t wdim, float affine_gain,
                     const float* a0, const float* b0, const float* w0, int32_t cout0, float gain0,
                     const float* a1, const float* b1, const float* w1, int32_t cout1, float gain1,
                     float* out, void* stream);

#define IDE3D_STYLE_BATCH_MAX 24
typedef struct ide3d_style_job {
    const float* w; int64_t w_stride;
    const float* affine_w; const float* affine_b;
    const float* wsq_t;
    int32_t cin, cout;
    float affine_gain, bias_gain;
    float* styles; float* dcoefs;
} ide3d_style_job;
typedef struct ide3d_fold_job {
    const float* w; int64_t w_stride;
    int32_t cin; float affine_gain;
    const float *a0, *b0, *w0; int32_t cout0; float gain0;
    const float *a1, *b1, *w1; int32_t cout1; float gain1;
    float* out;
} ide3d_fold_job;
int ide3d_style_demod_batch(const ide3d_style_job* jobs, int32_t njobs, int32_t n, int32_t wdim, void* stream);
int ide3d_fold_heads_batch(const ide3d_fold_job* jobs, int32_t njobs, int32_t n, int32_t wdim, void* stream);

#define IDE3D_LOWRES_MAX_LAYERS 8
#define IDE3D_LOWRES_MAX_HEADS 4
typedef struct ide3d_lowres_layer {
    const float* weight;
    const float* styles;
    const float* dcoefs;
    const float* noise;
    const float* bias;
    float act_gain, clamp;
    int32_t up;
    int32_t head;
    int32_t weights_packed;
    int32_t reserved;
} ide3d_lowres_layer;
typedef struct ide3d_lowres_head {
    const float* w;
    const float* bias;
    float* skip;
    float clamp;
    int32_t O;
} ide3d_lowres_head;
typedef struct ide3d_lowres_params {
    const float* x0; int64_t x0_batch_stride;
    const float* fir;
    float* x_out;
    void* workspace; int64_t workspace_bytes;
    int32_t n, C, res0, nlayers, nheads;
    int32_t arith;
    int32_t reserved0;
    int32_t reserved;
    ide3d_lowres_layer layers[IDE3D_LOWRES_MAX_LAYERS];
    ide3d_lowres_head heads[IDE3D_LOWRES_MAX_HEADS];
} ide3d_lowres_params;
int32_t ide3d_lowres_layers_supported(int32_t n, int32_t C, int32_t res0, const int32_t* ups, int32_t nlayers, int32_t arith);
int32_t ide3d_lowres_phase_r_plan(int32_t n, int32_t C, int32_t res0, const int32_t* ups, int32_t nlayers, int32_t arith,
                                  int32_t* bands, int64_t* scratch_bytes);
int64_t ide3d_lowres_workspace_bytes(const ide3d_lowres_params* p);
int ide3d_lowres_group(const ide3d_lowres_params* p, void* stream);

typedef struct ide3d_mapping_params {
    const float* z; const float* c;
    const float* embed_w; const float* embed_b;
    const float* fc_w[16]; const float* fc_b[16];
    int32_t fc_out[16];
    const float* w_avg;
    float* ws;
    void* workspace; int64_t workspace_bytes;
    int32_t n, z_dim, c_dim, embed, layers, num_ws;
    float embed_weight_gain, embed_bias_gain, lr_multiplier, alpha, act_gain, truncation_psi;
    int32_t truncation_cutoff;
} ide3d_mapping_params;

int ide3d_mapping_workspace_bytes(void);
int ide3d_mapping_supported(void);
int ide3d_mapping(const ide3d_mapping_params* p, void* stream);

int ide3d_skip_upsample_add_cl(const float* lo, const int64_t lo_stride[4], const float* add, const int64_t add_stride[4],
                               int32_t n, int32_t c, int32_t h, int32_t w, float* out, void* stream);

int ide3d_bilinear_up2_split(const float* x, int32_t n, int32_t c, int32_t h, int32_t w,
                             float* const dst[3], const int32_t c_begin[3], const int32_t c_count[3], const int64_t* dst_batch_floats, void* stream);

int ide3d_frame_u8(const float* img, const float* seg, const uint8_t* palette,
                   int32_t n, int32_t classes, int32_t H, int32_t W, uint8_t* out, void* stream);

int ide3d_sphere_points(const float* theta, const float* pitch, int32_t n, float r, int32_t pitch_is_v,
                        float* pos, float* phi_out, void* stream);
int ide3d_cam2world(const float* forward, const float* origin, const float* lookat, int32_t lookat_stride, int32_t n,
                    float* out, void* stream);

typedef struct ide3d_noise_map {
    float*  data;
    int32_t side;
    int32_t reserved;
} ide3d_noise_map;

int64_t ide3d_noise_reg_workspace_bytes(const int32_t* sides, int32_t k);
int ide3d_noise_reg_levels(const int32_t* sides, int32_t k);
int ide3d_noise_reg(const ide3d_noise_map* table, const int32_t* sides, int32_t k, float* workspace, int64_t workspace_bytes,
                    float* means, float* loss, void* stream);
int ide3d_noise_reg_backward(const ide3d_noise_map* table, const int32_t* sides, int32_t k, const float* workspace, int64_t workspace_bytes,
                             const float* means, const float* dloss, float* grad, void* stream);
int64_t ide3d_noise_normalize_workspace_bytes(const int32_t* sides, int32_t k);
int ide3d_noise_normalize(const ide3d_noise_map* table, const int32_t* sides, int32_t k, float* workspace, int64_t workspace_bytes,
                          void* stream);

#define IDE3D_LPIPS_MAX_TAPS 8
typedef struct ide3d_lpips_tap {
    const float* a;
    const float* t;
    const float* lin;
    float*       out;
    int32_t      c, h, w;
    int32_t      reserved;
} ide3d_lpips_tap;

int ide3d_lpips_prep(const float* x, float* y, const float* mean, const float* std_, int32_t n, int32_t H, int32_t W, int32_t f,
                     float in_scale, float in_shift, void* stream);
int ide3d_lpips_prep_backward(const float* dy, float* dx, const float* std_, int32_t n, int32_t H, int32_t W, int32_t f,
                              float in_scale, void* stream);
int ide3d_maxpool2(const float* x, float* y, int64_t planes, int32_t h, int32_t w, void* stream);
int ide3d_lpips_stage_backward(const float* y, const float* dpool, const float* dtap, float* dz, int64_t planes, int32_t h, int32_t w,
                               void* stream);
int64_t ide3d_lpips_head_workspace_bytes(const ide3d_lpips_tap* taps, int32_t k, int32_t n);
int ide3d_lpips_head(const ide3d_lpips_tap* taps, int32_t k, int32_t n, float* workspace, int64_t workspace_bytes, float* loss,
                     void* stream);
int ide3d_lpips_head_backward(const ide3d_lpips_tap* taps, int32_t k, int32_t n, const float* dloss, void* stream);

int ide3d_unfold2d(const float* x, float* col, int32_t n, int32_t c, int32_t h, int32_t w, int32_t k, int32_t stride, int32_t pad,
                   void* stream);
int ide3d_fold2d(const float* dcol, float* dx, int32_t n, int32_t c, int32_t h, int32_t w, int32_t k, int32_t stride, int32_t pad,
                 void* stream);
int ide3d_maxpool3s2p0(const float* x, float* y, uint8_t* idx, int64_t planes, int32_t h, int32_t w, void* stream);
int ide3d_lpips_tap_backward(const float* y, const float* g, const uint8_t* idx, const float* dtap, float* dz, int64_t planes, int32_t h,
                             int32_t w, int32_t pooled, void* stream);

#define IDE3D_PARSE_JOIN_TERMS 3
typedef struct ide3d_parse_term {
    const float* p;
    int64_t      batch_stride;
    int64_t      plane_stride;
    int32_t      row_pitch;
    int32_t      half;
} ide3d_parse_term;
typedef struct ide3d_parse_join_params {
    ide3d_parse_term term[IDE3D_PARSE_JOIN_TERMS];
    const float* scale;
    const float* bias;
    const float* y;
    float*       out;
    int32_t      n, c, h, w;
    int32_t      post;
    float        bias_gain;
} ide3d_parse_join_params;

int ide3d_resize_bilinear(const float* x, float* y, int64_t planes, int32_t h, int32_t w, int32_t H, int32_t W, void* stream);
int ide3d_resize_bilinear_backward(const float* dy, float* dx, int64_t planes, int32_t h, int32_t w, int32_t H, int32_t W, void* stream);
int64_t ide3d_parse_ce_workspace_bytes(int32_t n, int32_t C, int32_t h, int32_t w, int32_t H, int32_t W);
int ide3d_parse_ce(const float* logits, const int64_t* labels, int32_t n, int32_t C, int32_t h, int32_t w, int32_t H, int32_t W,
                   double* lse, float* workspace, int64_t workspace_bytes, float* loss, void* stream);
int ide3d_parse_ce_backward(const float* logits, const int64_t* labels, const double* lse, const float* dloss, float* dlogits,
// ... 47 lines not shown
```

Measured before the change: 941.6 frames/s.

## Gate last triplane block conv and skip-add to cells sampled by rays

Before the final tri-plane voxel block runs, a kernel marks which 4x4 cells of each plane the camera rays' samples (plus bilinear footprint) will touch. A compacted list of live tiles is then built. The fused conv+heads kernel and the skip upsample-add skip tiles no ray reads, launching only live tiles via the list. This avoids computing tri-plane features the renderer never samples, at the cost of extra setup kernels and leaving unsampled plane regions unwritten.

```diff
diff --git a/ide-3d_amd/csrc/camera.hip b/ide-3d_amd/csrc/camera.hip
--- a/ide-3d_amd/csrc/camera.hip
+++ b/ide-3d_amd/csrc/camera.hip
@@ -1,4 +1,5 @@
 #include "common.h"
+#include "raymarch_ray.h"
 
 namespace ide3d {
 
@@ -50,6 +51,109 @@
     m[12] = 0.f;    m[13] = 0.f; m[14] = 0.f;  m[15] = 1.f;
 }
 
+__global__ void __launch_bounds__(256)
+plane_cells_kernel(ide3d_render_params p, int cells_h, int cells_w, int lds_cells, uint8_t* __restrict__ cells) {
+    extern __shared__ __attribute__((aligned(16))) uint8_t s_cells[];
+    const int n = blockIdx.y, per_img = p.rays_per_img * p.steps;
+    const int i = (int)blockIdx.x * 256 + (int)threadIdx.x;
+    uint8_t* const img_cells = cells + (int64_t)n * 3 * cells_h * cells_w;
+    if (lds_cells) {
+        for (int k = threadIdx.x * 4; k < lds_cells; k += 1024) *reinterpret_cast<uint32_t*>(s_cells + k) = 0u;
+        __syncthreads();
+    }
+    if (i < per_img) {
+        const int s = i % p.steps, r = i / p.steps;
+        const float zstep = (p.steps > 1) ? (p.z_lin[1] - p.z_lin[0]) : 0.f;
+        const float zl = p.z_lin[s];
+        float ax, ay, az, bx, by, bz;
+        ray_world_point(p, n, r, zl, 0.f, zstep, ax, ay, az);
+        ray_world_point(p, n, r, zl, 1.f, zstep, bx, by, bz);
+        Tap2 ta[3], tb[3];
+        triplane_taps(ax, ay, az, p.W, p.H, ta);
+        triplane_taps(bx, by, bz, p.W, p.H, tb);
+        uint8_t* const dst = lds_cells ? s_cells : img_cells;
+#pragma unroll
+        for (int pl = 0; pl < 3; ++pl) {
+            const int x_lo = min(max(min(ta[pl].ix0, tb[pl].ix0) - 1, 0), p.W - 1), x_hi = min(max(max(ta[pl].ix0, tb[pl].ix0) + 2, 0), p.W - 1);
+            const int y_lo = min(max(min(ta[pl].iy0, tb[pl].iy0) - 1, 0), p.H - 1), y_hi = min(max(max(ta[pl].iy0, tb[pl].iy0) + 2, 0), p.H - 1);
+            uint8_t* const c = dst + pl * cells_h * cells_w;
+            for (int cy = y_lo >> 2; cy <= (y_hi >> 2); ++cy)
+                for (int cx = x_lo >> 2; cx <= (x_hi >> 2); ++cx) c[cy * cells_w + cx] = 1;
+        }
+    }
+    if (lds_cells) {
+        __syncthreads();
+        for (int k = threadIdx.x * 4; k < lds_cells; k += 1024) {
+            const uint32_t v = *reinterpret_cast<const uint32_t*>(s_cells + k);
+            if (v == 0u) continue;
+#pragma unroll
+            for (int e = 0; e < 4; ++e) if ((v >> (8 * e)) & 0xffu) img_cells[k + e] = 1;
+        }
+    }
+}
+
+__global__ void __launch_bounds__(1024)
+plane_tile_list_kernel(ide3d_plane_gate g, int n, int tiles_y, int tiles_x, int th, int tw, int32_t* __restrict__ list) {
+    __shared__ int s_wave[16];
+    const int tid = threadIdx.x, lane = tid & 63, wid = tid >> 6;
+    const int total = n * tiles_y * tiles_x;
+    int base = 0;
+    for (int t0 = 0; t0 < total; t0 += 1024) {
+        const int t = t0 + tid;
+        bool live = false;
+        if (t < total) {
+            const int tx = t % tiles_x, ty = (t / tiles_x) % tiles_y, img = t / (tiles_x * tiles_y);
+            const int cy0 = (ty * th) >> 2, cy1 = min((ty * th + th - 1) >> 2, g.cells_h - 1);
+            const int cx0 = (tx * tw) >> 2, cx1 = min((tx * tw + tw - 1) >> 2, g.cells_w - 1);
+            for (int pl = 0; pl < 3; ++pl)
+                for (int cy = cy0; cy <= cy1; ++cy)
+                    for (int cx = cx0; cx <= cx1; ++cx) live |= g.cells[(((int64_t)img * 3 + pl) * g.cells_h + cy) * g.cells_w + cx] != 0;
+        }
+        const unsigned long long bal = __builtin_amdgcn_ballot_w64(live);
+        if (lane == 0) s_wave[wid] = __popcll(bal);
+        __syncthreads();
+        int before = base;
+        for (int w = 0; w < wid; ++w) before += s_wave[w];
+        if (live) list[1 + before + __popcll(bal & ((1ull << lane) - 1ull))] = t;
+        for (int w = 0; w < 16; ++w) base += s_wave[w];
+        __syncthreads();
+    }
+    if (tid == 0) list[0] = base;
+}
+
+}
+
+extern "C" int ide3d_plane_cells(const float* rays_d_cam, const float* z_lin, const float* cam2world, int32_t n, int32_t rays_per_img,
+                                 int32_t steps, int32_t H, int32_t W, uint8_t* cells, void* stream) {
+    using namespace ide3d;
+    IDE3D_CHECK_ARG(rays_d_cam && z_lin && cam2world && cells, "plane_cells: null pointer");
+    IDE3D_CHECK_ARG(n > 0 && rays_per_img > 0 && steps > 0 && H > 0 && W > 0, "plane_cells: bad shape");
+    const int cells_h = cdiv(H, 4), cells_w = cdiv(W, 4);
+    const int64_t per_img = (int64_t)rays_per_img * steps, map_bytes = 3 * (int64_t)cells_h * cells_w;
+    IDE3D_CHECK_ARG(per_img < 0x7fffff00LL && n <= 65535 && n * map_bytes < 0x7fffffffLL, "plane_cells: too many samples, images or cells");
+    ide3d_render_params p{};
+    p.rays_d_cam = rays_d_cam; p.z_lin = z_lin; p.cam2world = cam2world;
+    p.jitter = z_lin;
+    p.n = n; p.rays_per_img = rays_per_img; p.steps = steps; p.H = H; p.W = W;
+    hipStream_t st = (hipStream_t)stream;
+    const hipError_t e = hipMemsetAsync(cells, 0, (size_t)(n * map_bytes), st);
+    if (e != hipSuccess) { set_error("plane_cells: hipMemsetAsync: %s", hipGetErrorString(e)); return IDE3D_ELAUNCH; }
+    const int lds_cells = (map_bytes % 4 == 0 && map_bytes <= 48 * 1024) ? (int)map_bytes : 0;
+    hipLaunchKernelGGL(plane_cells_kernel, dim3((unsigned)cdiv64(per_img, 256), (unsigned)n), dim3(256), (size_t)lds_cells, st, p, cells_h, cells_w, lds_cells, cells);
+    IDE3D_CHECK_LAUNCH("plane_cells");
+    return IDE3D_OK;
+}
+
+extern "C" int ide3d_plane_tile_list(const ide3d_plane_gate* gate, int32_t n, int32_t h, int32_t w, int32_t tile_h, int32_t tile_w, int32_t* list, void* stream) {
+    using namespace ide3d;
+    IDE3D_CHECK_ARG(gate && gate->cells && list, "plane_tile_list: null pointer");
+    IDE3D_CHECK_ARG(n > 0 && h > 0 && w > 0 && tile_h > 0 && tile_w > 0 && tile_h % 4 == 0 && tile_w % 4 == 0, "plane_tile_list: bad shape (tiles are multiples of the 4 x 4 cell)");
+    IDE3D_CHECK_ARG(4 * (int64_t)gate->cells_h >= h && 4 * (int64_t)gate->cells_w >= w, "plane_tile_list: the cell map does not cover the output");
+    const int tiles_y = cdiv(h, tile_h), tiles_x = cdiv(w, tile_w);
+    IDE3D_CHECK_ARG((int64_t)n * tiles_y * tiles_x < 0x7fffffffLL, "plane_tile_list: too many tiles");
+    hipLaunchKernelGGL(plane_tile_list_kernel, dim3(1), dim3(1024), 0, (hipStream_t)stream, *gate, n, tiles_y, tiles_x, tile_h, tile_w, list);
+    IDE3D_CHECK_LAUNCH("plane_tile_list");
+    return IDE3D_OK;
 }
 
 extern "C" int ide3d_sphere_points(const float* theta, const float* pitch, int32_t n, float r, int32_t pitch_is_v,
diff --git a/ide-3d_amd/csrc/common.h b/ide-3d_amd/csrc/common.h
--- a/ide-3d_amd/csrc/common.h
+++ b/ide-3d_amd/csrc/common.h
@@ -116,6 +116,22 @@
     return (int)g;
 }
 
+__device__ __forceinline__ bool plane_gate_live(const ide3d_plane_gate& g, int n, int pl0, int npl, int y0, int x0, int th, int tw) {
+    const int cy0 = max(y0 >> 2, 0), cx0 = max(x0 >> 2, 0);
+    const int cy1 = min((y0 + th - 1) >> 2, g.cells_h - 1), cx1 = min((x0 + tw - 1) >> 2, g.cells_w - 1);
+    const int nx = cx1 - cx0 + 1, ny = cy1 - cy0 + 1;
+    bool any = false;
+    if (nx > 0 && ny > 0) {
+        const int per = nx * ny, count = per * npl;
+        for (int i = (int)(threadIdx.x & 63u); i < count; i += 64) {
+            const int pl = pl0 + i / per, r = i % per;
+            any |= g.cells[(((int64_t)n * 3 + pl) * g.cells_h + cy0 + r / nx) * g.cells_w + cx0 + r % nx] != 0;
+        }
+    }
+    return __builtin_amdgcn_ballot_w64(any) != 0ull;
+}
+ide3d_plane_gate resolve_plane_gate(const ide3d_plane_gate* gate);
+
 __device__ __forceinline__ int xcd_remap(int bid, int nblocks) {
     const int xcd = bid % kNumXCD;
     const int idx = bid / kNumXCD;
diff --git a/ide-3d_amd/csrc/core.hip b/ide-3d_amd/csrc/core.hip
--- a/ide-3d_amd/csrc/core.hip
+++ b/ide-3d_amd/csrc/core.hip
@@ -1,4 +1,5 @@
 #include "common.h"
+#include "knobs.h"
 #include <string.h>
 #include <stdio.h>
 #include <map>
@@ -53,6 +54,11 @@
     return occ <= 1;
 }
 
+ide3d_plane_gate resolve_plane_gate(const ide3d_plane_gate* gate) {
+    if (!gate || !gate->cells || knob_live("IDE3D_NO_PLANE_GATE")) return ide3d_plane_gate{};
+    return *gate;
+}
+
 }
 
 extern "C" int ide3d_exclusive_violations(void) { return ide3d::g_excl_violations; }
diff --git a/ide-3d_amd/csrc/modconv.hip b/ide-3d_amd/csrc/modconv.hip
--- a/ide-3d_amd/csrc/modconv.hip
+++ b/ide-3d_amd/csrc/modconv.hip
@@ -601,6 +601,7 @@
     float clamp;
     int store_x;
     int bias_first;
+    ide3d_plane_gate gate;
 };
 template <int PH, int PW, int NWV, int MTW, int NTW, int BM, int MT, int PARTS, int SCRATCH>
 __device__ __forceinline__ void split_heads_finish(const ide3d_modconv_params& p, const HeadEpi& he, f32x16 (&acc)[1][MTW][NTW], float* smem,
@@ -1428,7 +1429,16 @@
     using K = SpCfg<MODE_CONV3, BIG, PH, 3, 2, 8>;
     if constexpr (kSpExclusive) asm volatile("" ::: "v255");
     __shared__ __attribute__((aligned(16))) unsigned char sp_smem[K::LDS_BYTES];
-    const BlockId b = decode_block(g);
+    BlockId b;
+    if (he.gate.tile_list) {
+        const int live = __builtin_amdgcn_readfirstlane(he.gate.tile_list[0]);
+        if ((int)blockIdx.x >= live) return;
+        const int id = __builtin_amdgcn_readfirstlane(he.gate.tile_list[1 + xcd_remap(blockIdx.x, live)]);
+        b.mb = 0; b.split = 0; b.tile = id % g.tile_base[4]; b.grp = id / g.tile_base[4];
+    } else {
+        b = decode_block(g);
+        if (he.gate.cells && !plane_gate_live(he.gate, b.grp, 0, 3, (b.tile / g.tiles_x[0]) * PH, (b.tile % g.tiles_x[0]) * K::PW, PH, K::PW)) return;
+    }
     modconv_split_tile<MODE_CONV3, BIG, PH, 3, 2, 8, 0, 1, -1, HEAD_MT>(p, wp, nullptr, g, sp_smem, b.mb, b.tile, b.grp, b.split, g.tiles_x[0], nullptr, nullptr, &he);
 }
 
@@ -1958,6 +1968,10 @@
 }
 
 extern "C" int ide3d_modconv2d_heads(const ide3d_modconv_params* pp, const ide3d_modconv_head_epilogue* hp, void* stream) {
+    return ide3d_modconv2d_heads_gated(pp, hp, nullptr, stream);
+}
+
+extern "C" int ide3d_modconv2d_heads_gated(const ide3d_modconv_params* pp, const ide3d_modconv_head_epilogue* hp, const ide3d_plane_gate* gate, void* stream) {
     using namespace ide3d;
     IDE3D_CHECK_ARG(pp != nullptr && hp != nullptr, "modconv2d_heads: null params");
     const ide3d_modconv_params& p = *pp;
@@ -1997,6 +2011,10 @@
     HeadEpi e;
     e.w = hw_packed; e.bias = h.bias; e.y = h.y; e.rows = h.rows; e.clamp = h.clamp; e.store_x = !h.no_activation_output;
     e.bias_first = head_resident_applies(q) ? 1 : 0;
+    e.gate = resolve_plane_gate(gate);
+    if (e.gate.cells)
+        IDE3D_CHECK_ARG(4 * (int64_t)e.gate.cells_h >= p.h && 4 * (int64_t)e.gate.cells_w >= p.w_, "modconv2d_heads: the plane gate's cell map does not cover the output");
+    if (!e.gate.cells || e.gate.tile_h != ph || e.gate.tile_w != 16) e.gate.tile_list = nullptr;
     const ConvGeom& g = pl.g;
     const unsigned nblocks = (unsigned)((int64_t)g.mblocks * g.tile_base[4] * g.img_groups * g.split_k);
     const u32x4* wu = reinterpret_cast<const u32x4*>(p.workspace);
diff --git a/ide-3d_amd/csrc/resample.hip b/ide-3d_amd/csrc/resample.hip
--- a/ide-3d_amd/csrc/resample.hip
+++ b/ide-3d_amd/csrc/resample.hip
@@ -12,6 +12,7 @@
     int64_t lo_s[4], add_s[4];
     int n, c, h, w;
     int tiles_x, tiles_y, cgroups;
+    ide3d_plane_gate gate;
 };
 
 __global__ void __launch_bounds__(256)
@@ -26,6 +27,7 @@
     const int n = b;
     const int c0 = cg * SK_CH, Y0 = ty * SK_ROWS, X0 = tx * SK_COLS;
     const int H = 2 * p.h, W = 2 * p.w;
+    if (p.gate.cells && !plane_gate_live(p.gate, n, cg % 3, 1, Y0, X0, SK_ROWS, SK_COLS)) return;
     const int m0 = Y0 / 2 - 1, q0 = X0 / 2 - 1;
     constexpr int NLO = (SK_CH * SK_LR * SK_LC + 255) / 256;
     float lo_v[NLO];
@@ -134,6 +136,11 @@
 
 extern "C" int ide3d_skip_upsample_add_cl(const float* lo, const int64_t lo_stride[4], const float* add, const int64_t add_stride[4],
                                           int32_t n, int32_t c, int32_t h, int32_t w, float* out, void* stream) {
+    return ide3d_skip_upsample_add_cl_gated(lo, lo_stride, add, add_stride, n, c, h, w, out, nullptr, stream);
+}
+
+extern "C" int ide3d_skip_upsample_add_cl_gated(const float* lo, const int64_t lo_stride[4], const float* add, const int64_t add_stride[4],
+                                                int32_t n, int32_t c, int32_t h, int32_t w, float* out, const ide3d_plane_gate* gate, void* stream) {
     using namespace ide3d;
     IDE3D_CHECK_ARG(lo && add && out && lo_stride && add_stride, "skip_upsample_add_cl: null pointer");
     IDE3D_CHECK_ARG(n > 0 && c > 0 && h > 0 && w > 0, "skip_upsample_add_cl: bad shape");
@@ -142,6 +149,10 @@
     a.lo = lo; a.add = add; a.out = out;
     for (int i = 0; i < 4; ++i) { a.lo_s[i] = lo_stride[i]; a.add_s[i] = add_stride[i]; }
     a.n = n; a.c = c; a.h = h; a.w = w;
+    a.gate = resolve_plane_gate(gate);
+    if (a.gate.cells)
+        IDE3D_CHECK_ARG(c % (3 * SK_CH) == 0 && 4 * (int64_t)a.gate.cells_h >= 2 * (int64_t)h && 4 * (int64_t)a.gate.cells_w >= 2 * (int64_t)w,
+                        "skip_upsample_add_cl: a plane gate needs 96-channel tri-planes and a cell map that covers the output");
     a.tiles_x = cdiv(2 * w, SK_COLS); a.tiles_y = cdiv(2 * h, SK_ROWS); a.cgroups = cdiv(c, SK_CH);
     const int64_t blocks = (int64_t)n * a.tiles_x * a.tiles_y * a.cgroups;
     IDE3D_CHECK_ARG(blocks < 0x7fffffffLL, "skip_upsample_add_cl: too many tiles");
diff --git a/ide-3d_amd/torch_utils/hip_plugin.py b/ide-3d_amd/torch_utils/hip_plugin.py
--- a/ide-3d_amd/torch_utils/hip_plugin.py
+++ b/ide-3d_amd/torch_utils/hip_plugin.py
@@ -376,6 +376,10 @@
             'ide3d_raster_shade': [vp, vp, i64, i32, i32, i32, vp, vp, vp, vp, i32, f32, f32, ctypes.POINTER(ctypes.c_float * 3), f32, vp, i64, vp, vp, vp, vp, vp],
             'ide3d_modconv2d': [ctypes.POINTER(_ModconvParams), vp],
             'ide3d_modconv2d_heads': [ctypes.POINTER(_ModconvParams), ctypes.POINTER(_ModconvHeadEpilogue), vp],
+            'ide3d_modconv2d_heads_gated': [ctypes.POINTER(_ModconvParams), ctypes.POINTER(_ModconvHeadEpilogue), ctypes.POINTER(_PlaneGate), vp],
+            'ide3d_plane_cells': [vp, vp, vp, i32, i32, i32, i32, i32, vp, vp],
+            'ide3d_plane_tile_list': [ctypes.POINTER(_PlaneGate), i32, i32, i32, i32, i32, vp, vp],
+            'ide3d_skip_upsample_add_cl_gated': [vp, ctypes.POINTER(i64 * 4), vp, ctypes.POINTER(i64 * 4), i32, i32, i32, i32, vp, ctypes.POINTER(_PlaneGate), vp],
             'ide3d_modconv_plan': [ctypes.POINTER(_ModconvParams), ctypes.POINTER(_ModconvPlanInfo)],
             'ide3d_modconv_workspace_bytes': [i32, i32, i32, i32, i32, i32, i32, i32],
             'ide3d_act_bwd_workspace_bytes': [i32, i32, i32, i32],
@@ -486,6 +490,7 @@
     'ide3d_render_ray_weights', 'ide3d_merge_depths', 'ide3d_render_rays_merged',
     'ide3d_render_merged_param_grad_workspace_bytes', 'ide3d_render_rays_merged_backward',
     'ide3d_raster_workspace_bytes', 'ide3d_raster_project', 'ide3d_raster_depth', 'ide3d_raster_shade',
+    'ide3d_plane_cells', 'ide3d_plane_tile_list', 'ide3d_modconv2d_heads_gated', 'ide3d_skip_upsample_add_cl_gated',
 )
 
 
@@ -1331,7 +1336,7 @@
 
     @staticmethod
     def modconv2d_heads(x, w, styles, dcoefs, noise, noise_strength, bias, act, alpha, gain, clamp, head_w, head_bias, head_clamp,
-                        want_x=True, arith=0):
+                        want_x=True, arith=0, gate=None, heads_out=None):
         for t in (x, w, head_w):
             _require(t.is_cuda and t.dtype == torch.float32 and t.is_contiguous(), 'modconv2d_heads: contiguous float32 CUDA tensors required')
         n, cin, h, wd = x.shape
@@ -1349,7 +1354,9 @@
         if knob_off or shape_key in ModconvPlugin._heads_declined:
             return None
         y = torch.empty([n, cout, h, wd], dtype=torch.float32, device=x.device) if want_x else None
-        heads = torch.empty([n, rows, h, wd], dtype=torch.float32, device=x.device)
+        heads = torch.empty([n, rows, h, wd], dtype=torch.float32, device=x.device) if heads_out is None else heads_out
+        _require(heads.dtype == torch.float32 and heads.device == x.device and tuple(heads.shape) == (n, rows, h, wd) and heads.is_contiguous(),
+                 'modconv2d_heads: heads_out must be a contiguous float32 [n, rows, h, w] tensor on the device of x')
         p, ent, keep = ModconvPlugin._params(lib, x, w, y, styles, dcoefs, noise, noise_strength, bias, act, alpha, gain, clamp, 0, arith, None, None)
         hent = ModconvPlugin._workspace(lib, heads, head_w, n, cout, rows, h, wd, 1, 0, True, arith)
         e = _ModconvHeadEpilogue()
@@ -1360,7 +1367,10 @@
             e.bias = head_bias.data_ptr()
         e.workspace, e.workspace_bytes = hent[0].data_ptr(), hent[0].numel() * 4
         with _dev_guard(x.device):
-            rc = lib.ide3d_modconv2d_heads(ctypes.byref(p), ctypes.byref(e), _stream(x))
+            if gate is not None:
+                rc = lib.ide3d_modconv2d_heads_gated(ctypes.byref(p), ctypes.byref(e), ctypes.byref(_plane_gate(gate, n, h, wd)), _stream(x))
+            else:
+                rc = lib.ide3d_modconv2d_heads(ctypes.byref(p), ctypes.byref(e), _stream(x))
         if rc == -2:
             ModconvPlugin._heads_declined.add(shape_key)
             return None
@@ -2643,18 +2653,68 @@
         return out
 
 
+class _PlaneGate(ctypes.Structure):
+    _fields_ = [('cells', ctypes.c_void_p), ('cells_h', ctypes.c_int32), ('cells_w', ctypes.c_int32),
+                ('tile_list', ctypes.c_void_p), ('tile_h', ctypes.c_int32), ('tile_w', ctypes.c_int32)]
+
+
+def _plane_gate(gate, n, h, w):
+    cells, tiles, tile_hw = gate if isinstance(gate, tuple) else (gate, None, None)
+    _require(cells.is_cuda and cells.dtype == torch.uint8 and cells.is_contiguous() and tuple(cells.shape) == (n, 3, (h + 3) // 4, (w + 3) // 4),
+             f'plane gate: cells must be a contiguous uint8 CUDA tensor [{n}, 3, {(h + 3) // 4}, {(w + 3) // 4}], got {list(cells.shape)} {cells.dtype}')
+    g = _PlaneGate()
+    g.cells, g.cells_h, g.cells_w = cells.data_ptr(), cells.shape[2], cells.shape[3]
+    if tiles is not None:
+        th, tw = tile_hw
+        _require(tiles.is_cuda and tiles.dtype == torch.int32 and tiles.is_contiguous() and tiles.device == cells.device
+                 and tiles.numel() == 1 + n * (-(-h // th)) * (-(-w // tw)), 'plane gate: the tile list must be plane_tile_list(cells, h, w, tile_h, tile_w)')
+        g.tile_list, g.tile_h, g.tile_w = tiles.data_ptr(), th, tw
+    return g
+
+
+def plane_tile_list(cells, h, w, tile_h, tile_w):
+    n = cells.shape[0]
+    g = _plane_gate(cells, n, h, w)
+    out = torch.empty([1 + n * (-(-h // tile_h)) * (-(-w // tile_w))], dtype=torch.int32, device=cells.device)
+    with _dev_guard(cells.device):
+        rc = load().ide3d_plane_tile_list(ctypes.byref(g), n, int(h), int(w), int(tile_h), int(tile_w), _ptr(out), _stream(cells))
+    _check(rc, 'plane_tile_list')
+    return out
+
+
+def plane_cells(rays_d_cam, z_lin, cam2world, H, W):
+    for t in (rays_d_cam, z_lin, cam2world):
+        _require(t.is_cuda and t.dtype == torch.float32 and t.is_contiguous(), 'plane_cells: contiguous float32 CUDA tensors required')
+    _require(rays_d_cam.ndim == 2 and rays_d_cam.shape[1] == 3 and z_lin.ndim == 1 and cam2world.ndim == 3 and tuple(cam2world.shape[1:]) == (4, 4),
+             'plane_cells: rays_d_cam [R, 3], z_lin [S], cam2world [n, 4, 4]')
+    n = cam2world.shape[0]
+    cells = torch.empty([n, 3, (H + 3) // 4, (W + 3) // 4], dtype=torch.uint8, device=cam2world.device)
+    with _dev_guard(cells.device):
+        rc = load().ide3d_plane_cells(_ptr(rays_d_cam), _ptr(z_lin), _ptr(cam2world), n, rays_d_cam.shape[0], z_lin.shape[0], int(H), int(W),
+                                      _ptr(cells), _stream(cells))
+    _check(rc, 'plane_cells')
+    return cells
+
+
 class ResamplePlugin:
     @staticmethod
-    def skip_upsample_add_cl(lo, add):
+    def skip_upsample_add_cl(lo, add, gate=None, out=None):
         _require(lo.is_cuda and lo.dtype == torch.float32 and add.dtype == torch.float32 and add.device == lo.device,
                  'skip_upsample_add_cl: float32 CUDA tensors on one device required')
         n, c, h, w = lo.shape
         _require(tuple(add.shape) == (n, c, 2 * h, 2 * w), 'skip_upsample_add_cl: add must be [n, c, 2h, 2w]')
         _require(c % 4 == 0, 'skip_upsample_add_cl: channel count must be a multiple of 4')
-        out = torch.empty([n, c, 2 * h, 2 * w], dtype=torch.float32, device=lo.device, memory_format=torch.channels_last)
+        if out is None:
+            out = torch.empty([n, c, 2 * h, 2 * w], dtype=torch.float32, device=lo.device, memory_format=torch.channels_last)
+        _require(out.dtype == torch.float32 and out.device == lo.device and tuple(out.shape) == (n, c, 2 * h, 2 * w)
+                 and out.is_contiguous(memory_format=torch.channels_last), 'skip_upsample_add_cl: out must be a channels_last float32 [n, c, 2h, 2w] tensor')
         with _dev_guard(lo.device):
-            rc = load().ide3d_skip_upsample_add_cl(_ptr(lo), ctypes.byref(_i64x4(lo.stride())), _ptr(add), ctypes.byref(_i64x4(add.stride())),
-                                                   n, c, h, w, _ptr(out), _stream(lo))
+            if gate is not None:
+                rc = load().ide3d_skip_upsample_add_cl_gated(_ptr(lo), ctypes.byref(_i64x4(lo.stride())), _ptr(add), ctypes.byref(_i64x4(add.stride())),
+                                                             n, c, h, w, _ptr(out), ctypes.byref(_plane_gate(gate, n, 2 * h, 2 * w)), _stream(lo))
+            else:
+                rc = load().ide3d_skip_upsample_add_cl(_ptr(lo), ctypes.byref(_i64x4(lo.stride())), _ptr(add), ctypes.byref(_i64x4(add.stride())),
+                                                       n, c, h, w, _ptr(out), _stream(lo))
         _check(rc, 'skip_upsample_add_cl')
         return out
 
diff --git a/ide-3d_amd/training/graph_cache.py b/ide-3d_amd/training/graph_cache.py
--- a/ide-3d_amd/training/graph_cache.py
+++ b/ide-3d_amd/training/graph_cache.py
@@ -15,7 +15,7 @@
 STATS = collections.Counter()
 
 
-_PASS_ENV = ('IDE3D_NO_SKIP_MERGE', 'IDE3D_NO_STYLE_PREFETCH', 'IDE3D_NO_STYLE_BATCH', 'IDE3D_NO_LOWRES_GROUP')
+_PASS_ENV = ('IDE3D_NO_SKIP_MERGE', 'IDE3D_NO_STYLE_PREFETCH', 'IDE3D_NO_STYLE_BATCH', 'IDE3D_NO_LOWRES_GROUP', 'IDE3D_NO_PLANE_GATE')
 
 
 def _env_int(name, default):
diff --git a/ide-3d_amd/training/networks.py b/ide-3d_amd/training/networks.py
--- a/ide-3d_amd/training/networks.py
+++ b/ide-3d_amd/training/networks.py
@@ -554,7 +554,21 @@
     return y[:, :co], y[:, co:]
 
 
-def _conv1_dual_head(block, x, w1, w_shared, want_x, noise_mode='random', gain=1, input_noise=None, **unused):
+class PlaneGate:
+
+    def __init__(self, cells):
+        self.cells, self.taken = cells, False
+        self._lists = {}
+
+    def with_tiles(self, h, w, tile_h, tile_w):
+        from torch_utils import hip_plugin
+        key = (h, w, tile_h, tile_w)
+        if key not in self._lists:
+            self._lists[key] = hip_plugin.plane_tile_list(self.cells, h, w, tile_h, tile_w)
+        return self.cells, self._lists[key], (tile_h, tile_w)
+
+
+def _conv1_dual_head(block, x, w1, w_shared, want_x, noise_mode='random', gain=1, input_noise=None, _plane_gate=None, **unused):
     c1, tr, ts = block.conv1, block.torgb, block.toseg
     if not (use_hip_modconv and type(c1) is SynthesisLayer and c1.up == 1 and c1.padding == 1 and c1.weight.shape[2:] == (3, 3)
             and c1.activation in ('linear', 'lrelu') and tr.weight.shape[2] == 1 and tr.conv_clamp == ts.conv_clamp
@@ -581,9 +595,14 @@
     hbias = _cat_cached(tr.bias, ts.bias)
     hclamp = -1.0 if tr.conv_clamp is None else tr.conv_clamp
     xc = x.contiguous()
+    gate = None
+    if _plane_gate is not None and not want_x:
+        gate = _plane_gate.with_tiles(x.shape[2], x.shape[3], 16 if c1.weight.shape[0] == 128 else 32, 16)
     out = _modconv_plugin.modconv2d_heads(xc, c1.weight.contiguous(), styles.contiguous(), dcoefs, noise, 1.0, bias,
                                           spec.cuda_idx, spec.def_alpha, act_gain, -1.0 if act_clamp is None else act_clamp,
-                                          wcat, hbias, hclamp, want_x=want_x)
+                                          wcat, hbias, hclamp, want_x=want_x, gate=gate)
+    if gate is not None and out is not None:
+        _plane_gate.taken = True
     if out is None:
         x = _modconv_bias_act(x, c1.weight, styles, True, noise, 1.0, bias, c1.activation, act_gain, act_clamp, dcoefs=dcoefs)
         return x, _dual_head(x, tr, ts, w_shared, wcat=wcat)
@@ -1133,11 +1152,11 @@
             return skip
         raise NotImplementedError
 
-    def _accumulate(self, lo, cur, y):
+    def _accumulate(self, lo, cur, y, gate=None):
         if lo is not None:
             if (getattr(self, 'skip_channels_last', False) and lo.shape[1] % 4 == 0 and self.resample_filter.shape == (4, 4)
                     and _inference_on_gpu(lo, y) and self._filter_is_1331() and _resample_init()):
-                return _resample_plugin.skip_upsample_add_cl(lo, y)
+                return _resample_plugin.skip_upsample_add_cl(lo, y, gate=(gate.cells if gate is not None and lo.shape[1] % 96 == 0 else None))
             f = self.resample_filter
             return _upfirdn_plugin().upfirdn2d_ex(lo, f, 2, 2, 1, 1, 2, 1, 2, 1, False, 4.0, add=y)
         return cur.add_(y) if cur is not None else y
@@ -1153,6 +1172,7 @@
         misc.assert_shape(ws, [None, self.num_conv + self.num_torgb, self.w_dim])
         resume_after_conv0 = bool(layer_kwargs.pop('_resume_after_conv0', False))
         x_unused = bool(layer_kwargs.pop('_x_unused', False))
+        plane_gate = layer_kwargs.pop('_plane_gate', None)
         ws_list = ws.unbind(dim=1)
         w_iter = iter(ws_list)
         dtype = torch.float16 if self.use_fp16 and not force_fp32 else torch.float32
@@ -1182,7 +1202,7 @@
                 layer_kwargs['input_noise'] = block_noise[:, 1:2] if block_noise is not None else None
                 w1 = next(w_iter)
                 if (self.is_last or self.architecture == 'skip') and not disable_rgb and dtype == torch.float32:
-                    fused = _conv1_dual_head(self, x, w1, ws_list[self.num_conv], not x_unused, **layer_kwargs)
+                    fused = _conv1_dual_head(self, x, w1, ws_list[self.num_conv], not x_unused, _plane_gate=plane_gate, **layer_kwargs)
                 if fused is not None:
                     x, fused_heads = fused
                 else:
@@ -1214,8 +1234,9 @@
                     both = self._accumulate(lo_both, None, y_both)
                     img, seg = both[:, :y.shape[1]], both[:, y.shape[1]:]
                 else:
-                    img = self._accumulate(img_lo, img, y)
-                    seg = self._accumulate(seg_lo, seg, y_seg)
+                    skip_gate = plane_gate if (plane_gate is not None and plane_gate.taken) else None
+                    img = self._accumulate(img_lo, img, y, gate=skip_gate)
+                    seg = self._accumulate(seg_lo, seg, y_seg, gate=skip_gate)
         assert x is None or x.dtype == dtype
         if x is not None and out_dtype != dtype:
             x = x.to(out_dtype)
diff --git a/ide-3d_amd/training/triplane.py b/ide-3d_amd/training/triplane.py
--- a/ide-3d_amd/training/triplane.py
+++ b/ide-3d_amd/training/triplane.py
@@ -186,15 +186,27 @@
             return False
         return not any(t is not None and t.requires_grad for t in (cam2world, jitter, sigma_noise, importance_u))
 
+    def resolve_camera_model(self, fov=None, num_steps=None, ray_start=None, ray_end=None, img_size=None):
+        sp = self.spec
+        return (sp.fov if fov is None else fov, sp.num_steps if num_steps is None else num_steps,
+                sp.ray_start if ray_start is None else ray_start, sp.ray_end if ray_end is None else ray_end,
+                sp.render_size if img_size is None else img_size)
+
+    def needed_cells(self, cam2world, plane_hw, fov=None, num_steps=None, ray_start=None, ray_end=None, img_size=None):
+        fov, steps, t0, t1, size = self.resolve_camera_model(fov, num_steps, ray_start, ray_end, img_size)
+        vr._init()
+        rays_d_cam, z_lin = vr._fused_ray_setup(cam2world.device, float(fov), (size, size), int(steps), float(t0), float(t1))
+        from torch_utils import hip_plugin
+        return hip_plugin.plane_cells(rays_d_cam, z_lin, cam2world.float().contiguous(), plane_hw[0], plane_hw[1])
+
+    def fused_kernel_exists(self):
+        return (self.spec.plane_channels, self.spec.decoder_hidden) in ((32, 64), (16, 32))
+
     def forward(self, img_v, seg_v, cam2world, fov=None, num_steps=None, ray_start=None, ray_end=None, img_size=None,
                 nerf_noise=0.0, jitter=None, sigma_noise=None, white_back=False, clamp_mode=None,
                 hierarchical=None, importance_u=None, sigma_noise_fine=None, **unused):
         sp = self.spec
-        fov = sp.fov if fov is None else fov
-        steps = sp.num_steps if num_steps is None else num_steps
-        t0 = sp.ray_start if ray_start is None else ray_start
-        t1 = sp.ray_end if ray_end is None else ray_end
-        size = sp.render_size if img_size is None else img_size
+        fov, steps, t0, t1, size = self.resolve_camera_model(fov, num_steps, ray_start, ray_end, img_size)
         clamp_mode = sp.clamp_mode if clamp_mode is None else clamp_mode
         n, device = img_v.shape[0], img_v.device
         rays = size * size
@@ -334,7 +346,7 @@
                 w_idx += block.num_conv
         return voxel_ws, block_ws
 
-    def backbone(self, voxel_ws, **block_kwargs):
+    def backbone(self, voxel_ws, _plane_gate=None, **block_kwargs):
         x_v = img_v = seg_v = None
         blocks = [getattr(self, f'vb{res}') for res in self.voxel_block_resolutions]
         start, resume = 0, False
@@ -347,6 +359,8 @@
             extra = dict(_resume_after_conv0=True) if (resume and i == start) else {}
             if i == len(blocks) - 1:
                 extra['_x_unused'] = True
+                if _plane_gate is not None:
+                    extra['_plane_gate'] = _plane_gate
             x_v, img_v, seg_v = block(x_v, img_v, cur_ws, condition_img=seg_v, **block_kwargs, **extra)
         return img_v, seg_v
 
@@ -410,16 +424,38 @@
             return graph_cache.run(self, impl, ws, c, render_params, noise_mode, flags, force_fp32, ray_jitter, cached_planes, unused)
         return impl(ws, c, ray_jitter, cached_planes)
 
+    def _plane_gate_ok(self, ws, cam2world, render_params):
+        if os.environ.get('IDE3D_NO_PLANE_GATE') is not None or not ws.is_cuda or torch.is_grad_enabled() or not networks.use_hip_modconv:
+            return False
+        hierarchical = render_params.get('hierarchical')
+        if (self.spec.hierarchical if hierarchical is None else hierarchical) or not self.renderer.fused_kernel_exists():
+            return False
+        if cam2world.device != ws.device or any(p.device != ws.device for p in self.renderer.decoder.parameters()):
+            return False
+        last = getattr(self, f'vb{self.voxel_block_resolutions[-1]}')
+        if not getattr(last, 'skip_channels_last', False) or networks._hooked(self, last, self.renderer):
+            return False
+        from torch_utils import hip_plugin
+        return last.out_channels in (64, 128) and hip_plugin.conv_arithmetic() == 'bf16x6'
+
     def _forward_impl(self, ws, c, render_params, noise_mode, flags, force_fp32, ray_jitter, cached_planes):
         return_seg, return_raw, return_dict = flags
         voxel_ws, block_ws = self.split_ws(ws)
         block_kwargs = dict(noise_mode=noise_mode, force_fp32=force_fp32)
         with self._pass_scope(ws, ([] if cached_planes is not None else list(zip(self.voxel_block_resolutions, voxel_ws)), list(zip(self.block_resolutions, block_ws)))):
+            cam2world = c[:, :16].reshape(-1, 4, 4).to(torch.float32)
             if cached_planes is not None:
                 img_v, seg_v = cached_planes
             else:
-                img_v, seg_v = self.backbone(voxel_ws, **block_kwargs)
-            cam2world = c[:, :16].reshape(-1, 4, 4).to(torch.float32)
+                gate = None
+                if not return_dict and self._plane_gate_ok(ws, cam2world, render_params):
+                    res = self.voxel_block_resolutions[-1]
+                    gate = networks.PlaneGate(self.renderer.needed_cells(
+                        cam2world, (res, res), fov=render_params.get('fov'), num_steps=render_params.get('num_steps'),
+                        ray_start=render_params.get('ray_start'), ray_end=render_params.get('ray_end')))
+                    last = getattr(self, f'vb{res}')
+                    gate.with_tiles(res, res, 16 if last.out_channels == 128 else 32, 16)
+                img_v, seg_v = self.backbone(voxel_ws, _plane_gate=gate, **block_kwargs)
             feat, depth, wsum = self.renderer(
                 img_v, seg_v, cam2world, fov=render_params.get('fov'), num_steps=render_params.get('num_steps'),
                 ray_start=render_params.get('ray_start'), ray_end=render_params.get('ray_end'),
diff --git a/include/ide3d_hip.h b/include/ide3d_hip.h
--- a/include/ide3d_hip.h
+++ b/include/ide3d_hip.h
@@ -296,6 +296,17 @@
     int64_t      workspace_bytes;
 } ide3d_modconv_head_epilogue;
 int ide3d_modconv2d_heads(const ide3d_modconv_params* p, const ide3d_modconv_head_epilogue* heads, void* stream);
+
+typedef struct ide3d_plane_gate {
+    const uint8_t* cells;
+    int32_t        cells_h, cells_w;
+    const int32_t* tile_list;
+    int32_t        tile_h, tile_w;
+} ide3d_plane_gate;
+int ide3d_plane_cells(const float* rays_d_cam, const float* z_lin, const float* cam2world, int32_t n, int32_t rays_per_img, int32_t steps,
+                      int32_t H, int32_t W, uint8_t* cells, void* stream);
+int ide3d_plane_tile_list(const ide3d_plane_gate* gate, int32_t n, int32_t h, int32_t w, int32_t tile_h, int32_t tile_w, int32_t* list, void* stream);
+int ide3d_modconv2d_heads_gated(const ide3d_modconv_params* p, const ide3d_modconv_head_epilogue* heads, const ide3d_plane_gate* gate, void* stream);
 
 typedef struct ide3d_act_bwd_params {
     const float* dy;
@@ -453,6 +464,8 @@
 
 int ide3d_skip_upsample_add_cl(const float* lo, const int64_t lo_stride[4], const float* add, const int64_t add_stride[4],
                                int32_t n, int32_t c, int32_t h, int32_t w, float* out, void* stream);
+int ide3d_skip_upsample_add_cl_gated(const float* lo, const int64_t lo_stride[4], const float* add, const int64_t add_stride[4],
+                                     int32_t n, int32_t c, int32_t h, int32_t w, float* out, const ide3d_plane_gate* gate, void* stream);
 
 int ide3d_bilinear_up2_split(const float* x, int32_t n, int32_t c, int32_t h, int32_t w,
                              float* const dst[3], const int32_t c_begin[3], const int32_t c_count[3], const int64_t* dst_batch_floats, void* stream);
```

After: 986.7 frames/s (median of 6 runs). 4.8% higher.
